# salute-developers/GigaAM

Measured on AMD Instinct MI355X. Metric: RTFx v2_ctc batch32x20s (log-mel + encoder + greedy decode), higher is better.
Workload: dtype f32 (GEMMs: 3-term split on fp16 MFMA, fp32 accumulate)

## Files before the change

### gigaam_amd/_lib.py

```python
from __future__ import annotations

import ctypes as C
import os
from typing import Optional

_HERE = os.path.dirname(os.path.abspath(__file__))
LIB_NAME = "libgigaam_hip.so"
LIB_PATH = os.path.join(_HERE, LIB_NAME)

SUBS_CONV2D, SUBS_CONV1D = 0, 1
ATT_ROTARY, ATT_REL_POS = 0, 1
NORM_BATCH, NORM_LAYER = 0, 1
HEAD_NONE, HEAD_CTC, HEAD_RNNT, HEAD_EMO = 0, 1, 2, 3
DTYPE_F32, DTYPE_F16, DTYPE_BF16, DTYPE_F64, DTYPE_I64 = 0, 1, 2, 3, 4
GEMM_F32, GEMM_F16X3, GEMM_F16 = 0, 1, 2
RS_U8, RS_I16, RS_I24, RS_I32, RS_F32, RS_MULAW, RS_ALAW = range(7)
RS_FORM_SINGLE, RS_FORM_TABLE, RS_FORM_ROWS = 0, 1, 2
PF_CLASSES = ["gemm", "conv2", "attn", "norm", "convmod", "stem", "frontend", "decode", "misc", "align_bt", "align_out"]


class GamConfig(C.Structure):
    _fields_ = [(n, C.c_int32) for n in (
        "sample_rate", "n_mels", "hop_length", "win_length", "n_fft", "center",
        "feat_in", "n_layers", "d_model", "subsampling", "subs_kernel_size", "subsampling_factor",
        "ff_expansion_factor", "self_attention_model", "n_heads", "pos_emb_max_len",
        "conv_norm_type", "conv_kernel_size",
        "head_type", "num_classes", "pred_hidden", "pred_rnn_layers", "joint_hidden",
    )]


_P = C.c_void_p


class GamLnOp(C.Structure):
    _fields_ = ([(n, _P) for n in ("x", "out1", "out2", "w1", "b1", "w2", "b2", "rcos", "rsin", "row_t", "rs", "part", "pbias", "presid",
                                   "xstore")]
                + [(n, C.c_int32) for n in ("mode", "rows", "d", "split1", "split2", "dk", "ta", "rope_rows", "nsplit")]
                + [("eps", C.c_float), ("palpha", C.c_float)])


SIGNATURES = {
    "gam_abi_version": (C.c_int, []),
    "gam_create": (C.c_int, [C.POINTER(GamConfig), C.c_int, C.POINTER(_P)]),
    "gam_destroy": (None, [_P]),
    "gam_set_weight": (C.c_int, [_P, C.c_char_p, _P, C.c_int, C.POINTER(C.c_int64), C.c_int]),
    "gam_finalize": (C.c_int, [_P]),
    "gam_feat_frames": (C.c_int64, [_P, C.c_int64]),
    "gam_enc_frames": (C.c_int64, [_P, C.c_int64]),
    "gam_frontend": (C.c_int, [_P, _P, _P, C.c_int, C.c_int64, _P, _P, _P]),
    "gam_encode": (C.c_int, [_P, _P, _P, C.c_int, C.c_int64, _P, _P, _P]),
    "gam_encode_ex": (C.c_int, [_P, _P, _P, C.c_int, C.c_int64, _P, _P, C.c_int, _P, _P]),
    "gam_encode_varlen": (C.c_int, [_P, _P, _P, C.POINTER(C.c_int64), C.c_int, C.c_int64, _P, _P, C.c_int, _P, _P]),
    "gam_last_encode_rows": (C.c_int, [_P, C.POINTER(C.c_int)]),
    "gam_ctc_head": (C.c_int, [_P, _P, C.c_int, C.c_int64, _P, _P]),
    "gam_ctc_greedy": (C.c_int, [_P, _P, _P, C.c_int, C.c_int64, _P, _P, _P, _P]),
    "gam_ctc_align": (C.c_int, [_P, _P, _P, C.c_int, C.c_int64, _P, _P, C.c_int, _P, _P, _P, _P, _P, _P, _P]),
    "gam_op_ctc_align": (C.c_int, [_P, _P, _P, C.c_int, C.c_int64, C.c_int, _P, _P, C.c_int, _P, _P, _P, _P, _P, _P, _P]),
    "gam_op_ctc_align_long": (C.c_int, [_P, _P, C.c_int64, C.c_int, _P, C.c_int, _P, _P, _P, _P, _P, _P, _P]),
    "gam_op_ctc_star_row": (C.c_int, [_P, _P, _P, C.c_int, C.c_int64, C.c_int, C.c_float, _P, _P]),
    "gam_ctc_align_star": (C.c_int, [_P, _P, _P, C.c_int, C.c_int64, _P, _P, C.c_int, C.c_float, _P, _P, _P, _P, _P, _P, _P]),
    "gam_op_ctc_align_star": (C.c_int, [_P, _P, _P, C.c_int, C.c_int64, C.c_int, _P, _P, _P, C.c_int, _P, _P, _P, _P, _P, _P, _P]),
    "gam_op_ctc_align_long_star": (C.c_int, [_P, _P, C.c_int64, C.c_int, _P, _P, C.c_int, _P, _P, _P, _P, _P, _P, _P]),
    "gam_op_ctc_stitch": (C.c_int, [_P, _P, _P, C.c_int, C.c_int64, C.c_int, _P, _P, _P, _P, C.c_int64, _P, _P]),
    "gam_op_ctc_greedy_long": (C.c_int, [_P, _P, C.c_int64, C.c_int, _P, _P, _P, _P]),
    "gam_set_ctc_align_workspace": (C.c_int, [_P, C.c_int64]),
    "gam_tune_ctc_align_long": (C.c_int, [C.c_int, C.c_int]),
    "gam_ctc_kws": (C.c_int, [_P, _P, _P, C.c_int, C.c_int64, C.c_int, _P, _P, _P, _P, _P, _P]),
    "gam_op_ctc_kws": (C.c_int, [_P, _P, _P, C.c_int, C.c_int64, C.c_int, C.c_int, _P, _P, _P, _P, _P, _P]),
    "gam_set_keywords": (C.c_int, [_P, _P, _P, C.c_int, _P]),
    "gam_ctc_beam": (C.c_int, [_P, _P, _P, C.c_int, C.c_int64, C.c_int, _P, _P, _P, _P, _P, _P]),
    "gam_op_ctc_beam": (C.c_int, [_P, _P, _P, C.c_int, C.c_int64, C.c_int, C.c_int, _P, _P, _P, _P, _P, _P]),
    "gam_set_hotwords": (C.c_int, [_P, _P, _P, C.c_int, C.c_float]),
    "gam_set_lm": (C.c_int, [_P, _P, C.c_int, _P, C.c_int64, C.c_int, _P, C.c_int64, C.c_int, C.c_int, C.c_int, C.c_int, C.c_int,
                             C.c_float, C.c_float, C.c_float]),
    "gam_rnnt_greedy": (C.c_int, [_P, _P, _P, C.c_int, C.c_int64, C.c_int, _P, _P, _P, _P, _P, C.c_int, _P]),
    "gam_ctc_beam_nbest": (C.c_int, [_P, _P, _P, C.c_int, C.c_int64, C.c_int, C.c_int, _P, _P, _P, _P, _P, _P, _P]),
    "gam_op_ctc_beam_nbest": (C.c_int, [_P, _P, _P, C.c_int, C.c_int64, C.c_int, C.c_int, C.c_int, _P, _P, _P, _P, _P, _P, _P]),
    "gam_rnnt_beam_nbest": (C.c_int, [_P, _P, _P, C.c_int, C.c_int64, C.c_int, C.c_int, C.c_int, _P, _P, _P, _P, _P, _P, _P]),
    "gam_op_rnnt_beam_nbest": (C.c_int, [_P, _P, _P, C.c_int, C.c_int64, C.c_int, C.c_int, C.c_int, _P, _P, _P, _P, _P, _P, _P]),
    "gam_rnnt_beam": (C.c_int, [_P, _P, _P, C.c_int, C.c_int64, C.c_int, C.c_int, _P, _P, _P, _P, _P, _P]),
    "gam_op_rnnt_beam": (C.c_int, [_P, _P, _P, C.c_int, C.c_int64, C.c_int, C.c_int, _P, _P, _P, _P, _P, _P]),
    "gam_rnnt_align": (C.c_int, [_P, _P, _P, C.c_int, C.c_int64, _P, _P, C.c_int, _P, _P, _P, _P, _P]),
    "gam_op_rnnt_align": (C.c_int, [_P, _P, _P, C.c_int, C.c_int64, _P, _P, C.c_int, _P, _P, _P, _P, _P, _P]),
    "gam_op_rnnt_lattice_align": (C.c_int, [_P, _P, _P, C.c_int, C.c_int64, C.c_int, _P, _P, C.c_int, _P, _P, _P, _P, _P]),
    "gam_set_rnnt_align_workspace": (C.c_int, [_P, C.c_int64]),
    "gam_ctc_confidence": (C.c_int, [_P, _P, _P, C.c_int, C.c_int64, _P, _P, _P, C.c_int, C.c_int, C.c_int, _P, _P, _P, _P]),
    "gam_op_ctc_confidence": (C.c_int, [_P, _P, _P, C.c_int, C.c_int64, C.c_int, _P, _P, _P, C.c_int, C.c_int, C.c_int, _P, _P, _P, _P]),
    "gam_rnnt_confidence": (C.c_int, [_P, _P, _P, C.c_int, C.c_int64, _P, _P, _P, C.c_int, C.c_int, _P, _P, _P]),
    "gam_op_rnnt_confidence": (C.c_int, [_P, _P, _P, C.c_int, C.c_int64, _P, _P, _P, C.c_int, C.c_int, _P, _P, _P]),
    "gam_emo_probs": (C.c_int, [_P, _P, _P, C.c_int, C.c_int64, _P, _P]),
    "gam_rnnt_predict": (C.c_int, [_P, _P, _P, _P, C.c_int, _P, _P, _P, _P]),
    "gam_rnnt_joint": (C.c_int, [_P, _P, _P, C.c_int, C.c_int, C.c_int, _P, _P]),
    "gam_set_gemm_mode": (C.c_int, [_P, C.c_int]),
    "gam_get_gemm_mode": (C.c_int, [_P]),
    "gam_set_rnnt_cluster": (C.c_int, [_P, C.c_int]),
    "gam_get_rnnt_cluster": (C.c_int, [_P]),
    "gam_rnnt_cluster_plan_info": (C.c_int, [C.c_int] * 8 + [C.POINTER(C.c_int32)]),
    "gam_rnnt_last_decode": (C.c_int, [_P, C.POINTER(C.c_int32)]),
    "gam_debug_buffer_hash": (C.c_int, [_P, C.c_int, C.POINTER(C.c_uint64), C.POINTER(C.c_int64)]),
    "gam_range_flag": (C.c_int, [_P, C.POINTER(C.c_int), _P]),
    "gam_range_flag_fetch": (C.c_int, [_P, _P, _P]),
    "gam_op_gemm": (C.c_int, [_P, _P, _P, _P, _P, C.c_int, C.c_int, C.c_int, C.c_int, _P]),
    "gam_op_gemm_ex": (C.c_int, [_P, _P, _P, _P, _P, C.c_float, _P, C.c_int, C.c_int, C.c_int, C.c_int, _P]),
    "gam_op_attention": (C.c_int, [_P, _P, _P, _P, _P, _P, C.c_int, C.c_int, C.c_int, _P]),
    "gam_op_attention_ex": (C.c_int, [_P, _P, _P, _P, C.c_int64, _P, _P, _P, C.c_int, C.c_int, C.c_int, C.c_int, _P, _P, _P, _P]),
    "gam_op_layernorm": (C.c_int, [_P, C.POINTER(GamLnOp), _P]),
    "gam_op_convmod": (C.c_int, [_P, _P, _P, _P, _P, _P, _P, _P, _P, C.c_int, C.c_int, C.c_int, C.c_int, C.c_int, C.c_int, C.c_int, _P]),
    "gam_tune_sp": (C.c_int, [C.c_int, C.c_int, C.c_int]),
    "gam_plan_sp": (C.c_int, [C.c_int, C.c_int, C.c_int, C.c_int, C.POINTER(C.c_int), C.POINTER(C.c_int), C.POINTER(C.c_int)]),
    "gam_plan_sp_ex": (C.c_int, [C.c_int, C.c_int, C.c_int, C.c_int, C.POINTER(C.c_int), C.POINTER(C.c_int), C.POINTER(C.c_int), C.POINTER(C.c_int)]),
    "gam_tune_sp_stages": (C.c_int, [C.c_int]),
    "gam_resample_plan": (C.c_int, [C.c_int, C.c_int, C.POINTER(C.c_int), C.POINTER(C.c_int), C.POINTER(C.c_int)]),
    "gam_resample_tile": (C.c_int, [C.c_int, C.c_int, C.POINTER(C.c_int), C.POINTER(C.c_int)]),
    "gam_resample_table": (C.c_int, [C.c_int, C.c_int, _P, _P]),
    "gam_resample_out_len": (C.c_int64, [C.c_int, C.c_int, C.c_int64]),
    "gam_op_resample": (C.c_int, [_P, C.c_int, C.c_int, C.c_int, _P, C.c_int, C.c_int64, C.c_int, C.c_int, _P, _P, _P, C.c_int64, _P, _P]),
    "gam_profile_enable": (C.c_int, [_P, C.c_int]),
    "gam_profile_pause": (C.c_int, [_P, C.c_int]),
    "gam_profile_read": (C.c_int, [_P, C.c_int, C.POINTER(C.c_double), C.POINTER(C.c_int64), C.POINTER(C.c_double)]),
    "gam_profile_read_bytes": (C.c_int, [_P, C.c_int, C.POINTER(C.c_double)]),
    "gam_last_error": (C.c_char_p, [_P]),
    "gam_comm_unique_id": (C.c_int, [C.c_char_p]),
    "gam_comm_create": (C.c_int, [C.c_char_p, C.c_int, C.c_int, C.c_int, C.POINTER(_P)]),
    "gam_comm_world": (C.c_int, [_P]),
    "gam_gather_ids": (C.c_int, [_P, _P, _P, _P, _P, C.c_int, C.c_int, _P, _P, _P, _P, _P]),
    "gam_comm_last_error": (C.c_char_p, [_P]),
    "gam_comm_destroy": (None, [_P]),
}

_lib: Optional[C.CDLL] = None


class GigaAMHipError(RuntimeError):
    pass


def load_library(path: Optional[str] = None) -> C.CDLL:
    global _lib
    if _lib is not None and path is None:
        return _lib
    p = path or os.environ.get("GIGAAM_HIP_LIB", LIB_PATH)
    if not os.path.exists(p):
        raise GigaAMHipError(
            f"{p} not found: the HIP extension is not built. Run `python -c 'import __graft_entry__ as g; g.build()'` "
            "(hipcc --offload-arch=gfx950). There is no CPU fallback.")
    lib = C.CDLL(p)
    for name, (res, args) in SIGNATURES.items():
        fn = getattr(lib, name)
        fn.restype = res
        fn.argtypes = args
    if lib.gam_abi_version() != 1:
        raise GigaAMHipError("libgigaam_hip.so ABI version mismatch")
    if path is None:
        _lib = lib
    return lib
```

### gigaam_amd/csrc/gam_api.hip

```cpp
#include <hip/hip_runtime.h>

#include <algorithm>
#include <cmath>
#include <cstdarg>
#include <cstdio>
#include <cstring>
#include <map>
#include <string>
#include <vector>

#include "../../include/gigaam_hip.h"
#include "gam_align.h"
#include "gam_align_long.h"
#include "gam_kws.h"
#include "gam_attn.h"
#include "gam_beam.h"
#include "gam_rnnt_beam.h"
#include "gam_attn16.h"
#include "gam_comm.h"
#include "gam_common.h"
#include "gam_convmod.h"
#include "gam_decode.h"
#include "gam_rnnt_align.h"
#include "gam_confidence.h"
#include "gam_decode_cluster.h"
#include "gam_frontend.h"
#include "gam_gemm.h"
#include "gam_gemm_sp.h"
#include "gam_norm.h"
#include "gam_pack.h"
#include "gam_resample.h"
#include "gam_stem.h"
#include "gam_stitch.h"

namespace {

struct HostTensor {
  std::vector<float> data;
  std::vector<int64_t> shape;
  int64_t numel() const {
    int64_t n = 1;
    for (auto s : shape) n *= s;
    return n;
  }
};

struct DevBuf {
  float* p = nullptr;
  size_t cap = 0;
  DevBuf() = default;
  DevBuf(DevBuf&& o) noexcept : p(o.p), cap(o.cap) { o.p = nullptr; o.cap = 0; }
  DevBuf& operator=(DevBuf&& o) noexcept { std::swap(p, o.p); std::swap(cap, o.cap); return *this; }
  ~DevBuf() { (void)release(); }
  hipError_t release() {
    const hipError_t e = p ? hipFree(p) : hipSuccess;
    p = nullptr; cap = 0;
    return e;
  }
  hipError_t alloc(size_t floats) {
    hipError_t e = release();
    if (e == hipSuccess) e = hipMalloc(&p, floats * sizeof(float));
    if (e == hipSuccess) cap = floats; else p = nullptr;
    return e;
  }
  template <class T> T* as() const { return reinterpret_cast<T*>(p); }
};

struct W16 {
  _Float16* sp = nullptr;
  _Float16* h16 = nullptr;
  float inv = 1.0f;
};

struct LayerW {
  float *ln_ff1_w, *ln_ff1_b, *ff1_w1, *ff1_b1, *ff1_w2, *ff1_b2;
  float *ln_att_w, *ln_att_b, *wqkv, *bqkv, *wo, *bo;
  float *wpos, *pos_u, *pos_v;
  float *ln_conv_w, *ln_conv_b, *pw1_w, *pw1_b, *dw_w, *dw_b, *cn_scale, *cn_shift, *pw2_w, *pw2_b;
  float *ln_ff2_w, *ln_ff2_b, *ff2_w1, *ff2_b1, *ff2_w2, *ff2_b2;
  float *ln_out_w, *ln_out_b;
  W16 s_ff1_w1, s_ff1_w2, s_wqkv, s_wo, s_wpos, s_pw1, s_pw2, s_ff2_w1, s_ff2_w2;
};

struct ProfEvent {
  hipEvent_t a, b;
  int cls;
};

}

struct gam_handle {
  gam_config cfg;
  int device = 0;
  bool finalized = false;
  bool has_encoder = false, has_head = false;
  std::map<std::string, HostTensor> staged;
  std::vector<DevBuf> owned;
  std::string err;

  float* dft_basis = nullptr;
  int* mel_band = nullptr;
  float* mel_wts = nullptr;
  int mel_nw = 0;
  int nf = 0, kpad = 0;
  float *c1_w = nullptr, *c1_b = nullptr, *c2_w = nullptr, *c2_b = nullptr, *lin_w = nullptr, *lin_b = nullptr;
  W16 s_c1, s_c2, s_lin;
  int gemm_mode = 1;
  int f1 = 0, f2 = 0;
  std::vector<LayerW> layers;
  float *rot_cos = nullptr, *rot_sin = nullptr;
  float* rel_pe = nullptr;
  float* rel_pe_sp = nullptr;
  float *ctc_w = nullptr, *ctc_b = nullptr;
  float *emo_w = nullptr, *emo_b = nullptr;
  float *jn_enc_w = nullptr, *jn_enc_b = nullptr, *jn_pred_t = nullptr, *jn_pred_b = nullptr;
  float *jn_out_w = nullptr, *jn_out_b = nullptr, *lstm_whh_t = nullptr, *lstm_tab = nullptr;
  float *lstm_whh_q = nullptr, *jn_pred_q = nullptr;
  float* jn_pred_w = nullptr;
  DevBuf jz, jp, jl;
  float *lstm_wih_x = nullptr, *lstm_whh_x = nullptr, *lstm_bias_x = nullptr;
  int use_rowscale = 1;
  int use_range = 1;
  int ncu = 256;
  int rnnt_cluster = -1;
  int rnnt_coop = 1;
  int rnnt_force_timeout = 0;
  int rnnt_no_repair = 0;
  int rnnt_exclusive = 0;
  int last_rnnt_c = 0, last_rnnt_kern = -1, last_rnnt_refused = 0;
  DevBuf rnnt_x;
  DevBuf rnnt_audit;
  bool audit_pending = false; int audit_last_c = 0; long audit_decodes = 0, audit_hit_decodes = 0;
  hipEvent_t dec_evt = nullptr;
  hipStream_t dec_stream = nullptr;
  bool dec_evt_set = false;

  DevBuf wavp, spec, img, c2, xin, y1, x, y, yr, hbuf, qkv, ctx, ubuf, zbuf, tok, logits, encp, pbuf, aplanes;
  DevBuf op_planes, op_sp, splitk_ws;
  DevBuf align_star;
  DevBuf align_bp;
  DevBuf align_long_ws;
  DevBuf greedy_long_ws;
  size_t al_ws_limit = GAM_AL_WS_DEFAULT;
  DevBuf beam_nodes;
  DevBuf rb_ws, rb_nodes;
  DevBuf ra_g, ra_pp, ra_lat, ra_bp;
  DevBuf cf_stats;
  size_t ra_ws_limit = GAM_RA_WS_DEFAULT;
  DevBuf hw_trie;
  int hw_nodes = 0, hw_words = 0, hw_max_tok = -1;
  float hw_boost = 0.f;
  DevBuf kw_dev;
  int kw_K = 0, kw_ntok = 0, kw_max_tok = -1;
  DevBuf kws_mb;
  DevBuf lm_cls, lm_wt, lm_ng;
  int lm_V = 0, lm_wslots = 0, lm_wprobe = 0, lm_nslots = 0, lm_nprobe = 0, lm_order = 0, lm_bos = 0, lm_eos = 0, lm_unk = 0;
  float lm_unk_logp = 0.f, lm_alpha = 0.f, lm_beta = 0.f;
  DevBuf dec_splitk_ws;
  int last_rows = 0, last_rows_padded = 0;
  DevBuf pack_idx;
  int use_pack = 1;
  int use_splitk = 1;
  int fuse_reduce = 1;
  int use_graph = 1;
  int graph_max_rows = 2048;
  uint64_t ws_generation = 0;
  struct GraphEntry {
    enum Seen { UNSEEN, SEEN_ONCE, PLAIN_ONLY };
    uint64_t gen = 0; Seen seen = UNSEEN; hipGraphExec_t exec = nullptr;
  };
  std::map<std::vector<int>, GraphEntry> graphs;
  long graph_replays = 0, graph_captures_failed = 0;
  int graph_count = 0;
  hipStream_t cap_stream = nullptr;
  DevBuf lens;
  DevBuf rsbuf, op_rs;
  int* range_flag = nullptr;

  int prof_on = 0;
  std::vector<ProfEvent> prof_events;
  size_t prof_used = 0;
  double prof_work[GAM_PF_NCLASS] = {0};
  double prof_bytes[GAM_PF_NCLASS] = {0};
  int64_t prof_launches[GAM_PF_NCLASS] = {0};
};

namespace {

int fail(gam_handle* h, int code, const char* fmt, ...) {
  char buf[512];
  va_list ap;
  va_start(ap, fmt);
  vsnprintf(buf, sizeof buf, fmt, ap);
  va_end(ap);
  if (h) h->err = buf;
  return code;
}

#define HIPCHK(h, expr)                                                                        \
  do {                                                                                         \
    hipError_t e_ = (expr);                                                                    \
    if (e_ != hipSuccess) return fail(h, -2, "%s failed: %s (%s:%d)", #expr, hipGetErrorString(e_), __FILE__, __LINE__); \
  } while (0)

void* dev_upload(gam_handle* h, const void* src, size_t bytes, size_t alloc_bytes) {
  h->owned.emplace_back();
  DevBuf& b = h->owned.back();
  if (b.alloc((alloc_bytes + 3) / 4) != hipSuccess) return nullptr;
  if (src && bytes && hipMemcpy(b.p, src, bytes, hipMemcpyHostToDevice) != hipSuccess) return nullptr;
  return b.p;
}

float* upload(gam_handle* h, const std::vector<float>& v) {
  return (float*)dev_upload(h, v.data(), v.size() * sizeof(float), std::max<size_t>(v.size(), 4) * sizeof(float));
}

int ensure_table(gam_handle* h, DevBuf& b, size_t floats) {
  if (floats <= b.cap) return 0;
  HIPCHK(h, b.alloc(floats));
  return 0;
}
// ... 59 lines not shown
    hi[i] = hb;
    lo[i] = float_to_half_bits(v - half_to_float(hb));
  }
  out.inv = ldexpf(1.0f, -shift);
  std::vector<uint16_t> hp(hi);
  if (conv_taps > 0 && K > 0 && (K / conv_taps) % 64 == 0 && w.size() % (size_t)K == 0) {
    const size_t C = (size_t)K / conv_taps, cb64 = C / 64;
    for (size_t n = 0; n < w.size() / K; ++n)
      for (size_t cb = 0; cb < cb64; ++cb)
        for (size_t t = 0; t < (size_t)conv_taps; ++t)
          for (size_t j = 0; j < 64; ++j)
            hp[n * K + (cb * conv_taps + t) * 64 + j] = hi[n * K + t * C + cb * 64 + j];
  }
  out.h16 = (_Float16*)dev_upload(h, hp.data(), w.size() * 2, std::max<size_t>(w.size(), 8) * 2 + 64);
  if (!out.h16) return -2;
  if (K > 0 && K % 32 == 0 && w.size() % (size_t)K == 0) {
    std::vector<uint16_t> sp(w.size() * 2);
    for (size_t i = 0; i < w.size(); ++i) {
      const size_t n = i / K, k = i % K;
      size_t kb = k / 32;
      if (conv_taps > 0) {
        const size_t cblocks = (size_t)K / conv_taps / 32, t = kb / cblocks, cb = kb % cblocks;
        kb = cb * conv_taps + t;
      }
      const size_t o = n * 2 * (size_t)K + kb * 64 + (k % 32);
      sp[o] = hi[i];
      sp[o + 32] = lo[i];
    }
    out.sp = (_Float16*)dev_upload(h, sp.data(), sp.size() * 2, sp.size() * 2 + 64);
    if (!out.sp) return -2;
  }
  return 0;
}

const HostTensor* find(gam_handle* h, const std::string& key) {
  auto it = h->staged.find(key);
  return it == h->staged.end() ? nullptr : &it->second;
}

struct ProfScope {
  gam_handle* h;
  hipStream_t s;
  ProfEvent* ev = nullptr;
  ProfScope(gam_handle* h_, hipStream_t s_, int cls, double work) : h(h_), s(s_) {
    if (!h->prof_on || (h->prof_on == 2 && cls != GAM_PF_GEMM && cls != GAM_PF_CONV2)) return;
    if (h->prof_used == h->prof_events.size()) {
      ProfEvent e;
      if (hipEventCreate(&e.a) != hipSuccess || hipEventCreate(&e.b) != hipSuccess) return;
      h->prof_events.push_back(e);
    }
    ev = &h->prof_events[h->prof_used++];
    ev->cls = cls;
    h->prof_work[cls] += work;
    h->prof_launches[cls] += 1;
    hipEventRecord(ev->a, s);
  }
  ~ProfScope() {
    if (ev) hipEventRecord(ev->b, s);
  }
};

struct PendingReduce {
  const float* part = nullptr;
  int nsplit = 0;
  const float* bias = nullptr;
  const float* resid = nullptr;
  float alpha = 1.0f;
  GamGemmArgs full;
  int act = 0;
  void clear() { part = nullptr; nsplit = 0; }
};

int flush_pending(gam_handle* h, hipStream_t s, PendingReduce* p) {
  if (p == nullptr || p->part == nullptr) return 0;
  const hipError_t e = gam_launch_splitk_reduce(p->full, p->act, p->nsplit, s);
  const int M = p->full.M, N = p->full.N;
  p->clear();
  if (e != hipSuccess) return fail(h, -2, "split-K reduce launch (M=%d N=%d): %s", M, N, hipGetErrorString(e));
  return 0;
}

static inline bool split_mode(const gam_handle* h) { return h->gemm_mode != GAM_GEMM_F32; }

int gemm(gam_handle* h, hipStream_t s, const GamGemmArgs& a_in, int act, int cls = GAM_PF_GEMM, const W16* w16 = nullptr,
         PendingReduce* defer = nullptr) {
  GamGemmArgs a = a_in;
  if (int r = flush_pending(h, s, defer)) return r;
  a.range_flag = h->use_range ? h->range_flag : nullptr;
  if (!split_mode(h)) a.c_guard = 0;
  ProfScope ps(h, s, cls, 2.0 * (double)a.M * (double)a.N * (double)a.K);
  if (ps.ev) {
    const double abytes = a.a_mode == 0 ? ((double)(a.M - 1) * (double)std::min<long>(a.lda, a.K) + a.K) * 4.0
                                        : (double)a.M / a.conv_f2 * 2.0 * a.conv_fp * a.conv_c * 4.0;
    h->prof_bytes[cls] += abytes * (a.n_switch > 0 ? 2.0 : 1.0) + 4.0 * a.N * a.K + 4.0 * a.M * a.N * (a.R ? 2.0 : 1.0);
  }
  hipError_t e;
  if (a.Asp != nullptr) {
    if (!split_mode(h)) return fail(h, -2, "sp32 A operand outside the split-fp16 GEMM mode");
    if (w16 == nullptr || w16->sp == nullptr) return fail(h, -2, "sp32 A without sp32 W planes");
    a.wscale_inv = w16->inv;
    a.Wsp = w16->sp;
    a.h16 = 0;
    if (a.a_fmt == 2) {
      if (a.K % 64 != 0 || (a.a_mode == 0 ? a.lda % 64 != 0 : a.conv_c % 64 != 0) || w16->h16 == nullptr)
        return fail(h, -2, "GAM_GEMM_F16: K / row pitch of a GEMM operand is not a multiple of 64 (M=%d N=%d K=%d)", a.M, a.N, a.K);
      a.h16 = 1; a.K /= 2; a.lda /= 2; a.conv_c /= 2;
      a.Wsp = w16->h16;
    }
    GamSpPlan plan = gam_gemm_sp_plan(a.M, a.N, a.K, a.a_mode, h->ncu);
    if (!h->use_splitk) plan.s = 1;
    a.sp_mt = plan.mt; a.sp_nw = plan.nw; a.sp_ns = plan.ns;
    GamGemmArgs full = a;
    if (plan.s > 1) {
      if (int r = ensure(h, h->splitk_ws, (size_t)plan.s * a.M * a.N + 64)) return r;
      a.splitk = plan.s; a.partial = h->splitk_ws.p;
    }
    e = gam_launch_gemm_sp(a, act, s);
    if (e != hipSuccess) return fail(h, -2, "sp gemm launch (M=%d N=%d K=%d): %s", a.M, a.N, a.K, hipGetErrorString(e));
    if (plan.s > 1 && defer != nullptr && h->fuse_reduce && act == GAM_ACT_NONE && !a.c_split && !a.c_guard && a.lens == nullptr &&
        !a.remap && a.ldc == a.N && a.bias != nullptr && a.R != nullptr && a.ldr == a.N) {
      defer->part = a.partial; defer->nsplit = plan.s; defer->bias = a.bias; defer->resid = a.R; defer->alpha = a.alpha;
      defer->full = full; defer->full.partial = a.partial; defer->act = act;
    } else if (plan.s > 1) {
      full.partial = a.partial;
      e = gam_launch_splitk_reduce(full, act, plan.s, s);
      if (e != hipSuccess) return fail(h, -2, "split-K reduce launch (M=%d N=%d): %s", a.M, a.N, hipGetErrorString(e));
    }
    return 0;
  }
  if (a.a_rs != nullptr || a.c_split) return fail(h, -2, "row-scaled A or split C without sp32 operands (M=%d N=%d K=%d)", a.M, a.N, a.K);
  int S = 1;
  if (h->use_splitk && a.a_mode == 0 && a.K % 32 == 0) {
    const int tiles = gam_cdiv(a.M, 128) * gam_cdiv(a.N, 128), nk = a.K / 32, ncu = 256;
    if (tiles * 2 <= ncu && nk >= 4) {
      S = std::min(16, std::min(ncu / tiles, nk / 2));
      while (S > 1 && nk % S != 0) --S;
    }
  }
  GamGemmArgs full = a;
  if (S > 1) {
    DevBuf& ws = cls == GAM_PF_DECODE ? h->dec_splitk_ws : h->splitk_ws;
    if (int r = ensure(h, ws, (size_t)S * a.M * a.N + 64)) return r;
    a.splitk = S; a.ldw = a.K; a.K = a.K / S; a.partial = ws.p;
  }
  e = gam_launch_gemm(a, act, s);
  if (e != hipSuccess) return fail(h, -2, "gemm launch (M=%d N=%d K=%d): %s", a.M, a.N, a.K, hipGetErrorString(e));
  if (S > 1) {
    full.partial = a.partial;
    e = gam_launch_splitk_reduce(full, act, S, s);
    if (e != hipSuccess) return fail(h, -2, "split-K reduce launch (M=%d N=%d): %s", a.M, a.N, hipGetErrorString(e));
  }
  return 0;
}

GamGemmArgs gemm_args(const float* A, long lda, const float* W, const float* bias, float* C, long ldc, int M, int N, int K) {
  GamGemmArgs g;
  memset(&g, 0, sizeof g);
  g.A = A; g.W = W; g.bias = bias; g.C = C; g.R = nullptr;
  g.M = M; g.N = N; g.K = K; g.lda = lda; g.ldc = ldc; g.ldr = ldc; g.alpha = 1.0f;
  g.rpb = 1; g.fdiv = 1;
  return g;
}

int layernorm(gam_handle* h, hipStream_t s, GamLnArgs a, int mode, PendingReduce* pend = nullptr) {
  if (pend != nullptr && pend->part != nullptr) {
    const GamGemmArgs& g = pend->full;
    if (a.x == g.C && a.rows == g.M && a.d == g.N && g.ldc == g.N) {
      a.part = pend->part; a.nsplit = pend->nsplit; a.pbias = pend->bias; a.presid = pend->resid; a.palpha = pend->alpha;
      a.xstore = const_cast<float*>(a.x);
      pend->clear();
    } else if (int r = flush_pending(h, s, pend)) {
      return r;
    }
  }
  const double bytes = (double)a.rows * a.d * 4.0 * (mode == 0 ? 2.0 : 3.0);
  ProfScope ps(h, s, GAM_PF_NORM, bytes);
  hipError_t e = gam_launch_layernorm(a, mode, s);
  if (e != hipSuccess) return fail(h, -2, "layernorm launch: %s", hipGetErrorString(e));
  return 0;
}

int64_t half_up(int64_t l) { return l <= 0 ? 0 : (l + 1) / 2; }

struct DecodeScope {
  gam_handle* h;
  hipStream_t s;
  DecodeScope(gam_handle* h_, hipStream_t s_) : h(h_), s(s_) {
    if (h->dec_evt == nullptr && hipEventCreateWithFlags(&h->dec_evt, hipEventDisableTiming) != hipSuccess) { h->dec_evt = nullptr; (void)hipGetLastError(); }
    if (h->dec_evt != nullptr && h->dec_evt_set && h->dec_stream != s) (void)hipStreamWaitEvent(s, h->dec_evt, 0);
  }
  ~DecodeScope() {
    if (h->dec_evt != nullptr && hipEventRecord(h->dec_evt, s) == hipSuccess) { h->dec_stream = s; h->dec_evt_set = true; }
  }
};

#define GAM_DECODE_ENTRY(h, stream)      \
  hipStream_t s = (hipStream_t)(stream); \
  if (!(h)) return -1;                   \
  HIPCHK(h, hipSetDevice((h)->device));  \
  DecodeScope ds(h, s)

int head_check(gam_handle* h, int want, const char* who) {
  if (!h) return -1;
  if (who && !h->finalized) return fail(h, -1, "%s before gam_finalize", who);
  if (h->cfg.head_type != want || !h->has_head)
    return fail(h, -1, "model has no %s head", want == GAM_HEAD_CTC ? "CTC" : want == GAM_HEAD_RNNT ? "RNN-T" : "emotion");
  return 0;
}

template <class Args> void rnnt_pred_weights(const gam_handle* h, Args& a) {
  a.gate_tab = h->lstm_tab; a.whh_t = h->lstm_whh_t; a.wih_x = h->lstm_wih_x; a.whh_x = h->lstm_whh_x; a.bias_x = h->lstm_bias_x;
}
template <class Args> void rnnt_joint_weights(const gam_handle* h, Args& a) {
  a.wpred_t = h->jn_pred_t; a.bpred = h->jn_pred_b; a.wout = h->jn_out_w; a.bout = h->jn_out_b;
}

}

extern "C" {

int gam_abi_version(void) { return GAM_ABI_VERSION; }

const char* gam_last_error(const gam_handle* h) { return h ? h->err.c_str() : "null handle"; }

int gam_create(const gam_config* cfg, int device_id, gam_handle** out) {
  if (!cfg || !out) return -1;
  gam_handle* h = new gam_handle();
  h->cfg = *cfg;
  h->device = device_id;
  *out = h;
  if (const char* e = getenv("GAM_SPLITK")) h->use_splitk = atoi(e);
  if (const char* e = getenv("GAM_PACK")) h->use_pack = atoi(e);
  if (const char* e = getenv("GAM_FUSE_REDUCE")) h->fuse_reduce = atoi(e);
  if (const char* e = getenv("GAM_GRAPH")) h->use_graph = atoi(e);
  if (const char* e = getenv("GAM_GRAPH_MAX_ROWS")) h->graph_max_rows = atoi(e);
  if (const char* e = getenv("GAM_RNNT_CLUSTER")) h->rnnt_cluster = std::max(-1, std::min(8, atoi(e)));
  if (const char* e = getenv("GAM_RNNT_ALIGN_WS")) h->ra_ws_limit = (size_t)std::max(1ll, atoll(e));
  if (const char* e = getenv("GAM_CTC_ALIGN_WS")) h->al_ws_limit = (size_t)std::max(1ll, atoll(e));
  if (const char* e = getenv("GAM_RNNT_EXCLUSIVE")) h->rnnt_exclusive = atoi(e);
  if (const char* e = getenv("GAM_RNNT_COOP")) h->rnnt_coop = atoi(e);
  if (const char* e = getenv("GAM_RNNT_FORCE_TIMEOUT")) h->rnnt_force_timeout = atoi(e);
  if (const char* e = getenv("GAM_RNNT_NO_REPAIR")) h->rnnt_no_repair = atoi(e);
  {
    int n = 0;
    if (hipDeviceGetAttribute(&n, hipDeviceAttributeMultiprocessorCount, device_id) == hipSuccess && n > 0) h->ncu = n;
    int co = 0;
    if (hipDeviceGetAttribute(&co, hipDeviceAttributeCooperativeLaunch, device_id) != hipSuccess || co == 0) h->rnnt_coop = 0;
  }
  if (const char* e = getenv("GAM_ROWSCALE")) h->use_rowscale = atoi(e);
  if (const char* e = getenv("GAM_RANGE")) h->use_range = atoi(e);
  if (const char* e = getenv("GAM_GEMM_MODE"))
    h->gemm_mode = strcmp(e, "f32") == 0 ? GAM_GEMM_F32 : (strcmp(e, "f16") == 0 ? GAM_GEMM_F16 : GAM_GEMM_F16X3);
  const gam_config& c = h->cfg;
  if (c.d_model <= 0 || c.n_heads <= 0 || c.d_model % c.n_heads != 0)
    return fail(h, -1, "bad d_model/n_heads %d/%d", c.d_model, c.n_heads);
  if (c.d_model / c.n_heads != GAM_ATT_DK) return fail(h, -1, "head dim %d unsupported (kernels are built for %d)", c.d_model / c.n_heads, GAM_ATT_DK);
  if (c.d_model % 64 != 0 || c.d_model > 1024) return fail(h, -1, "d_model %d unsupported", c.d_model);
  if (c.subsampling_factor != 4) return fail(h, -1, "subsampling_factor %d unsupported", c.subsampling_factor);
  if (c.subsampling == GAM_SUBS_CONV2D && c.subs_kernel_size != 3) return fail(h, -1, "conv2d stem needs kernel 3");
  if (c.subsampling == GAM_SUBS_CONV1D && c.subs_kernel_size != 5) return fail(h, -1, "conv1d stem needs kernel 5");
  if (c.win_length != c.n_fft) return fail(h, -1, "win_length != n_fft unsupported");
  if (c.n_mels > 64 || c.n_mels != c.feat_in) return fail(h, -1, "n_mels %d / feat_in %d unsupported", c.n_mels, c.feat_in);
  if (c.head_type == GAM_HEAD_RNNT && (c.pred_rnn_layers < 1 || c.pred_rnn_layers > 4 || c.pred_hidden > GAM_RNNT_MAXH || c.joint_hidden > GAM_RNNT_MAXH || c.num_classes > GAM_RNNT_MAXV || c.joint_hidden % 16 != 0 || c.pred_hidden % 16 != 0))
    return fail(h, -1, "RNN-T head shape unsupported");
  if (hipSetDevice(device_id) != hipSuccess) return fail(h, -2, "hipSetDevice(%d) failed", device_id);
  return 0;
}

#if GAM_RC_AUDIT
static int audit_dump(gam_handle* h);
#endif
void gam_destroy(gam_handle* h) {
  if (!h) return;
  hipSetDevice(h->device);
#if GAM_RC_AUDIT
  audit_dump(h);
  fprintf(stderr, "[gam-audit] total: %ld of %ld cluster decodes logged at least one entry\n", h->audit_hit_decodes, h->audit_decodes);
#endif
  for (auto& e : h->prof_events) { hipEventDestroy(e.a); hipEventDestroy(e.b); }
  for (auto& g : h->graphs)
    if (g.second.exec) hipGraphExecDestroy(g.second.exec);
  if (h->cap_stream) hipStreamDestroy(h->cap_stream);
  if (h->dec_evt) hipEventDestroy(h->dec_evt);
  if (getenv("GAM_GRAPH_DEBUG")) fprintf(stderr, "[gam] graph replays %ld, failed captures %ld\n", h->graph_replays, h->graph_captures_failed);
  delete h;
}

int gam_set_weight(gam_handle* h, const char* key, const void* host_ptr, int dtype, const int64_t* shape, int ndim) {
  if (!h || !key || !host_ptr) return -1;
  if (h->finalized) return fail(h, -1, "gam_set_weight after gam_finalize");
  HostTensor t;
  for (int i = 0; i < ndim; ++i) t.shape.push_back(shape[i]);
  const int64_t n = t.numel();
  t.data.resize((size_t)n);
  switch (dtype) {
    case GAM_DTYPE_F32: memcpy(t.data.data(), host_ptr, (size_t)n * 4); break;
    case GAM_DTYPE_F16: for (int64_t i = 0; i < n; ++i) t.data[i] = half_to_float(((const uint16_t*)host_ptr)[i]); break;
    case GAM_DTYPE_BF16: for (int64_t i = 0; i < n; ++i) { uint32_t u = (uint32_t)((const uint16_t*)host_ptr)[i] << 16; memcpy(&t.data[i], &u, 4); } break;
    case GAM_DTYPE_F64: for (int64_t i = 0; i < n; ++i) t.data[i] = (float)((const double*)host_ptr)[i]; break;
    case GAM_DTYPE_I64: for (int64_t i = 0; i < n; ++i) t.data[i] = (float)((const int64_t*)host_ptr)[i]; break;
    default: return fail(h, -1, "unknown dtype %d for %s", dtype, key);
  }
  h->staged[key] = std::move(t);
  return 0;
}

struct Dst {
  float** p;
  const char* name;
};
#define DST(member) Dst{&(member), #member}

static int need(gam_handle* h, const std::string& key, int64_t n, const HostTensor** t) {
  *t = find(h, key);
  if (!*t) return fail(h, -3, "missing weight %s", key.c_str());
  if ((*t)->numel() != n) return fail(h, -3, "weight %s has %lld elements, expected %lld", key.c_str(), (long long)(*t)->numel(), (long long)n);
  return 0;
}

static int upload_to(gam_handle* h, Dst dst, const std::vector<float>& v) {
  *dst.p = upload(h, v);
  return *dst.p ? 0 : fail(h, -2, "device upload failed (%s)", dst.name);
}

static int up_split(gam_handle* h, const std::vector<float>& w, W16* out, int K, int conv_taps = 0) {
  return make_split(h, w, *out, K, conv_taps) ? fail(h, -2, "split upload failed") : 0;
}

static int upload_linear(gam_handle* h, const std::string& prefix, int64_t nout, int64_t nin, Dst w, Dst b, W16* split) {
  const HostTensor *wt, *bt;
  if (int r = need(h, prefix + ".weight", nout * nin, &wt)) return r;
  if (int r = need(h, prefix + ".bias", nout, &bt)) return r;
// ... 79 lines not shown

static int fin_stem_conv2d(gam_handle* h) {
  const int C = h->cfg.d_model, D = h->cfg.d_model, F = h->cfg.feat_in;
  const std::string pe = "encoder.pre_encode.";
  h->f1 = (F + 1) / 2;
  h->f2 = (h->f1 + 1) / 2;
  const HostTensor *w0, *b0, *w2, *b2, *wl, *bl;
  if (int r = need(h, pe + "conv.0.weight", (int64_t)C * 9, &w0)) return r;
  if (int r = need(h, pe + "conv.0.bias", C, &b0)) return r;
  if (int r = need(h, pe + "conv.2.weight", (int64_t)C * C * 9, &w2)) return r;
  if (int r = need(h, pe + "conv.2.bias", C, &b2)) return r;
  if (int r = need(h, pe + "out.weight", (int64_t)D * C * h->f2, &wl)) return r;
  if (int r = need(h, pe + "out.bias", D, &bl)) return r;
  if (int r = upload_to(h, DST(h->c1_w), w0->data)) return r;
  if (int r = upload_to(h, DST(h->c1_b), b0->data)) return r;
  const std::vector<float> t2 = swap_inner(w2->data, C, C, 9);
  if (int r = upload_to(h, DST(h->c2_w), t2)) return r;
  if (int r = up_split(h, t2, &h->s_c2, 9 * C, C % 32 == 0 ? 9 : 0)) return r;
  if (int r = upload_to(h, DST(h->c2_b), b2->data)) return r;
  const std::vector<float> l = swap_inner(wl->data, D, C, h->f2);
  if (int r = upload_to(h, DST(h->lin_w), l)) return r;
  if (int r = up_split(h, l, &h->s_lin, C * h->f2)) return r;
  return upload_to(h, DST(h->lin_b), bl->data);
}

static int fin_stem_conv1d(gam_handle* h) {
  const int C = h->cfg.d_model, F = h->cfg.feat_in, ks = h->cfg.subs_kernel_size;
  const std::string pe = "encoder.pre_encode.";
  const HostTensor *w0, *b0, *w2, *b2;
  if (int r = need(h, pe + "conv.0.weight", (int64_t)C * F * ks, &w0)) return r;
  if (int r = need(h, pe + "conv.0.bias", C, &b0)) return r;
  if (int r = need(h, pe + "conv.2.weight", (int64_t)C * C * ks, &w2)) return r;
  if (int r = need(h, pe + "conv.2.bias", C, &b2)) return r;
  const std::vector<float> r0 = swap_inner(w0->data, C, F, ks), r2 = swap_inner(w2->data, C, C, ks);
  if (int r = upload_to(h, DST(h->c1_w), r0)) return r;
  if (int r = up_split(h, r0, &h->s_c1, ks * F)) return r;
  if (int r = upload_to(h, DST(h->c1_b), b0->data)) return r;
  if (int r = upload_to(h, DST(h->c2_w), r2)) return r;
  if (int r = up_split(h, r2, &h->s_c2, ks * C)) return r;
  return upload_to(h, DST(h->c2_b), b2->data);
}

static int fin_qkv(gam_handle* h, const std::string& p, LayerW& L) {
  const int D = h->cfg.d_model;
  const HostTensor *wq, *bq, *wk, *bk, *wv, *bv;
  if (int r = need(h, p + "self_attn.linear_q.weight", (int64_t)D * D, &wq)) return r;
  if (int r = need(h, p + "self_attn.linear_q.bias", D, &bq)) return r;
  if (int r = need(h, p + "self_attn.linear_k.weight", (int64_t)D * D, &wk)) return r;
  if (int r = need(h, p + "self_attn.linear_k.bias", D, &bk)) return r;
  if (int r = need(h, p + "self_attn.linear_v.weight", (int64_t)D * D, &wv)) return r;
  if (int r = need(h, p + "self_attn.linear_v.bias", D, &bv)) return r;
  std::vector<float> w(wq->data), b(bq->data);
  w.insert(w.end(), wk->data.begin(), wk->data.end());
  w.insert(w.end(), wv->data.begin(), wv->data.end());
  b.insert(b.end(), bk->data.begin(), bk->data.end());
  b.insert(b.end(), bv->data.begin(), bv->data.end());
  if (int r = upload_to(h, DST(L.wqkv), w)) return r;
  if (int r = upload_to(h, DST(L.bqkv), b)) return r;
  return up_split(h, w, &L.s_wqkv, D);
}

static int fin_conv_norm(gam_handle* h, const std::string& p, LayerW& L) {
  const int D = h->cfg.d_model;
  const HostTensor *g, *be;
  if (int r = need(h, p + "conv.batch_norm.weight", D, &g)) return r;
  if (int r = need(h, p + "conv.batch_norm.bias", D, &be)) return r;
  if (h->cfg.conv_norm_type != GAM_NORM_BATCH) {
    if (int r = upload_to(h, DST(L.cn_scale), g->data)) return r;
    return upload_to(h, DST(L.cn_shift), be->data);
  }
  const HostTensor *rm, *rv;
  if (int r = need(h, p + "conv.batch_norm.running_mean", D, &rm)) return r;
  if (int r = need(h, p + "conv.batch_norm.running_var", D, &rv)) return r;
  std::vector<float> sc(D), sh(D);
  for (int i = 0; i < D; ++i) {
    const float inv = 1.0f / sqrtf(rv->data[i] + 1e-5f);
    sc[i] = g->data[i] * inv;
    sh[i] = be->data[i] - rm->data[i] * sc[i];
  }
  if (int r = upload_to(h, DST(L.cn_scale), sc)) return r;
  return upload_to(h, DST(L.cn_shift), sh);
}

static int fin_layer(gam_handle* h, int li, LayerW& L) {
  const gam_config& c = h->cfg;
  const int D = c.d_model, DFF = D * c.ff_expansion_factor;
  const std::string p = "encoder.layers." + std::to_string(li) + ".";
  memset(&L, 0, sizeof L);
  if (int r = upload_ln(h, p + "norm_feed_forward1", D, DST(L.ln_ff1_w), DST(L.ln_ff1_b))) return r;
  if (int r = upload_linear(h, p + "feed_forward1.linear1", DFF, D, DST(L.ff1_w1), DST(L.ff1_b1), &L.s_ff1_w1)) return r;
  if (int r = upload_linear(h, p + "feed_forward1.linear2", D, DFF, DST(L.ff1_w2), DST(L.ff1_b2), &L.s_ff1_w2)) return r;
  if (int r = upload_ln(h, p + "norm_self_att", D, DST(L.ln_att_w), DST(L.ln_att_b))) return r;
  if (int r = fin_qkv(h, p, L)) return r;
  if (int r = upload_linear(h, p + "self_attn.linear_out", D, D, DST(L.wo), DST(L.bo), &L.s_wo)) return r;
  if (c.self_attention_model == GAM_ATT_REL_POS) {
    const HostTensor *wp, *pu, *pv;
    if (int r = need(h, p + "self_attn.linear_pos.weight", (int64_t)D * D, &wp)) return r;
    if (int r = need(h, p + "self_attn.pos_bias_u", D, &pu)) return r;
    if (int r = need(h, p + "self_attn.pos_bias_v", D, &pv)) return r;
    if (int r = upload_to(h, DST(L.wpos), wp->data)) return r;
    if (int r = up_split(h, wp->data, &L.s_wpos, D)) return r;
    if (int r = upload_to(h, DST(L.pos_u), pu->data)) return r;
    if (int r = upload_to(h, DST(L.pos_v), pv->data)) return r;
  }
  if (int r = upload_ln(h, p + "norm_conv", D, DST(L.ln_conv_w), DST(L.ln_conv_b))) return r;
  if (int r = upload_linear(h, p + "conv.pointwise_conv1", 2 * D, D, DST(L.pw1_w), DST(L.pw1_b), &L.s_pw1)) return r;
  if (int r = upload_linear(h, p + "conv.depthwise_conv", D, c.conv_kernel_size, DST(L.dw_w), DST(L.dw_b), nullptr)) return r;
  if (int r = fin_conv_norm(h, p, L)) return r;
  if (int r = upload_linear(h, p + "conv.pointwise_conv2", D, D, DST(L.pw2_w), DST(L.pw2_b), &L.s_pw2)) return r;
  if (int r = upload_ln(h, p + "norm_feed_forward2", D, DST(L.ln_ff2_w), DST(L.ln_ff2_b))) return r;
  if (int r = upload_linear(h, p + "feed_forward2.linear1", DFF, D, DST(L.ff2_w1), DST(L.ff2_b1), &L.s_ff2_w1)) return r;
  if (int r = upload_linear(h, p + "feed_forward2.linear2", D, DFF, DST(L.ff2_w2), DST(L.ff2_b2), &L.s_ff2_w2)) return r;
  return upload_ln(h, p + "norm_out", D, DST(L.ln_out_w), DST(L.ln_out_b));
}

static int fin_rotary(gam_handle* h) {
  const int dk = h->cfg.d_model / h->cfg.n_heads, half = dk / 2, n = h->cfg.pos_emb_max_len;
  std::vector<float> cs((size_t)n * half), sn((size_t)n * half);
  for (int i = 0; i < half; ++i) {
    const float inv_freq = 1.0f / powf((float)n, (float)(2 * i) / (float)dk);
    for (int t = 0; t < n; ++t) {
      const float fr = (float)t * inv_freq;
      cs[(size_t)t * half + i] = (float)cos((double)fr);
      sn[(size_t)t * half + i] = (float)sin((double)fr);
    }
  }
  if (int r = upload_to(h, DST(h->rot_cos), cs)) return r;
  return upload_to(h, DST(h->rot_sin), sn);
}

static int fin_rel_pos(gam_handle* h) {
  const int D = h->cfg.d_model, n = h->cfg.pos_emb_max_len;
  std::vector<float> pe((size_t)(2 * n - 1) * D);
  for (int i = 0; i < D / 2; ++i) {
    const float w = expf((float)(2 * i) * (float)(-(log(10000.0) / D)));
    for (int r = -(n - 1); r <= n - 1; ++r) {
      const float ang = (float)r * w;
      pe[(size_t)(r + n - 1) * D + 2 * i] = (float)sin((double)ang);
      pe[(size_t)(r + n - 1) * D + 2 * i + 1] = (float)cos((double)ang);
    }
  }
  if (int r = upload_to(h, DST(h->rel_pe), pe)) return r;
  h->rel_pe_sp = (float*)dev_upload(h, nullptr, 0, pe.size() * sizeof(float));
  if (!h->rel_pe_sp) return fail(h, -2, "device upload failed (h->rel_pe_sp)");
  hipLaunchKernelGGL(gam_to_sp32_kernel, dim3((int)std::min<size_t>((pe.size() / 4 + 255) / 256, 4096)), dim3(256), 0, nullptr, h->rel_pe,
                     reinterpret_cast<_Float16*>(h->rel_pe_sp), pe.size() / 4, (const float*)nullptr, D);
  HIPCHK(h, hipGetLastError());
  HIPCHK(h, hipStreamSynchronize(nullptr));
  return 0;
}

static int fin_rnnt_upper(gam_handle* h) {
  const int PH = h->cfg.pred_hidden, LX = h->cfg.pred_rnn_layers - 1;
  const size_t G = (size_t)4 * PH;
  std::vector<float> wih_x(LX * PH * G), whh_x(LX * PH * G), bias_x(LX * G);
  for (int l = 1; l <= LX; ++l) {
    const std::string sfx = "_l" + std::to_string(l);
    const HostTensor *wi, *wh, *bi, *bh;
    if (int r = need(h, "head.decoder.lstm.weight_ih" + sfx, (int64_t)4 * PH * PH, &wi)) return r;
    if (int r = need(h, "head.decoder.lstm.weight_hh" + sfx, (int64_t)4 * PH * PH, &wh)) return r;
    if (int r = need(h, "head.decoder.lstm.bias_ih" + sfx, 4 * PH, &bi)) return r;
    if (int r = need(h, "head.decoder.lstm.bias_hh" + sfx, 4 * PH, &bh)) return r;
    transpose_rk(wi->data.data(), G, PH, &wih_x[(l - 1) * PH * G]);
    transpose_rk(wh->data.data(), G, PH, &whh_x[(l - 1) * PH * G]);
    for (size_t r = 0; r < G; ++r) bias_x[(l - 1) * G + r] = bi->data[r] + bh->data[r];
  }
  if (int r = upload_to(h, DST(h->lstm_wih_x), wih_x)) return r;
  if (int r = upload_to(h, DST(h->lstm_whh_x), whh_x)) return r;
  return upload_to(h, DST(h->lstm_bias_x), bias_x);
}

static std::vector<float> lstm_input_table(const HostTensor* emb, const HostTensor* wih, const HostTensor* bih, const HostTensor* bhh, int V, int PH) {
  std::vector<float> tab((size_t)(V + 1) * 4 * PH);
  for (int v = 0; v <= V; ++v)
    for (int r = 0; r < 4 * PH; ++r) {
      float acc = 0.f;
      if (v < V) {
        const float* wr = &wih->data[(size_t)r * PH];
        const float* e = &emb->data[(size_t)v * PH];
        for (int k = 0; k < PH; ++k) acc = fmaf(wr[k], e[k], acc);
      }
      tab[(size_t)v * 4 * PH + r] = (acc + bih->data[r]) + bhh->data[r];
    }
  return tab;
}

static int fin_rnnt_head(gam_handle* h) {
  const gam_config& c = h->cfg;
  const int D = c.d_model, V = c.num_classes, PH = c.pred_hidden, JH = c.joint_hidden;
  const HostTensor *emb, *wih, *whh, *bih, *bhh, *wp, *bp, *we, *bee, *wo, *bo;
  if (int r = need(h, "head.decoder.embed.weight", (int64_t)V * PH, &emb)) return r;
  if (int r = need(h, "head.decoder.lstm.weight_ih_l0", (int64_t)4 * PH * PH, &wih)) return r;
  if (int r = need(h, "head.decoder.lstm.weight_hh_l0", (int64_t)4 * PH * PH, &whh)) return r;
  if (int r = need(h, "head.decoder.lstm.bias_ih_l0", 4 * PH, &bih)) return r;
  if (int r = need(h, "head.decoder.lstm.bias_hh_l0", 4 * PH, &bhh)) return r;
  if (int r = need(h, "head.joint.pred.weight", (int64_t)JH * PH, &wp)) return r;
  if (int r = need(h, "head.joint.pred.bias", JH, &bp)) return r;
  if (int r = need(h, "head.joint.enc.weight", (int64_t)JH * D, &we)) return r;
  if (int r = need(h, "head.joint.enc.bias", JH, &bee)) return r;
  if (int r = need(h, "head.joint.joint_net.1.weight", (int64_t)V * JH, &wo)) return r;
  if (int r = need(h, "head.joint.joint_net.1.bias", V, &bo)) return r;
  if (c.pred_rnn_layers > 1)
    if (int r = fin_rnnt_upper(h)) return r;
  if (int r = upload_to(h, DST(h->lstm_whh_q), quad_rk(whh->data, 4 * PH, PH))) return r;
  if (int r = upload_to(h, DST(h->jn_pred_q), quad_rk(wp->data, JH, PH))) return r;
  if (int r = upload_to(h, DST(h->lstm_tab), lstm_input_table(emb, wih, bih, bhh, V, PH))) return r;
  if (int r = upload_to(h, DST(h->lstm_whh_t), swap_inner(whh->data, 1, 4 * PH, PH))) return r;
  if (int r = upload_to(h, DST(h->jn_pred_t), swap_inner(wp->data, 1, JH, PH))) return r;
  if (int r = upload_to(h, DST(h->jn_pred_b), bp->data)) return r;
  if (int r = upload_to(h, DST(h->jn_pred_w), wp->data)) return r;
  if (int r = upload_to(h, DST(h->jn_enc_w), we->data)) return r;
  if (int r = upload_to(h, DST(h->jn_enc_b), bee->data)) return r;
  if (int r = upload_to(h, DST(h->jn_out_w), wo->data)) return r;
  return upload_to(h, DST(h->jn_out_b), bo->data);
}

static int fin_head(gam_handle* h) {
  const gam_config& c = h->cfg;
  if (c.head_type == GAM_HEAD_CTC) return upload_linear(h, "head.decoder_layers.0", c.num_classes, c.d_model, DST(h->ctc_w), DST(h->ctc_b), nullptr);
  if (c.head_type == GAM_HEAD_EMO) return upload_linear(h, "head", c.num_classes, c.d_model, DST(h->emo_w), DST(h->emo_b), nullptr);
  return c.head_type == GAM_HEAD_RNNT ? fin_rnnt_head(h) : 0;
}

int gam_finalize(gam_handle* h) {
  if (!h) return -1;
  if (h->finalized) return 0;
  HIPCHK(h, hipSetDevice(h->device));
  const gam_config& c = h->cfg;
  if (int r = fin_frontend(h)) return r;
  const bool build_encoder = find(h, "encoder.pre_encode.conv.0.weight") != nullptr;
  if (build_encoder) {
    if (int r = c.subsampling == GAM_SUBS_CONV2D ? fin_stem_conv2d(h) : fin_stem_conv1d(h)) return r;
    h->layers.resize(c.n_layers);
    for (int li = 0; li < c.n_layers; ++li)
      if (int r = fin_layer(h, li, h->layers[li])) return r;
    if (int r = c.self_attention_model == GAM_ATT_ROTARY ? fin_rotary(h) : fin_rel_pos(h)) return r;
  }
  h->has_encoder = build_encoder;
  h->has_head = find(h, "head.decoder_layers.0.weight") != nullptr || find(h, "head.joint.enc.weight") != nullptr ||
                (c.head_type == GAM_HEAD_EMO && find(h, "head.weight") != nullptr);
  if (h->has_head)
    if (int r = fin_head(h)) return r;
  const std::vector<int> zeros(16, 0);
  h->range_flag = (int*)dev_upload(h, zeros.data(), 64, 64);
  if (!h->range_flag) return fail(h, -2, "device upload failed (h->range_flag)");
  h->staged.clear();
  h->finalized = true;
  return 0;
}

int64_t gam_feat_frames(const gam_handle* h, int64_t n) {
  const gam_config& c = h->cfg;
  if (c.center) return n / c.hop_length + 1;
  return n < c.win_length ? 0 : (n - c.win_length) / c.hop_length + 1;
}

int64_t gam_enc_frames(const gam_handle* h, int64_t t) {
  (void)h;
  return half_up(half_up(t));
}

int gam_frontend(gam_handle* h, const float* wav, const int64_t* wav_len, int B, int64_t L, float* feat,
                 int64_t* feat_len, void* stream) {
  if (!h || !h->finalized) return fail(h, -1, "gam_frontend before gam_finalize");
  if (B <= 0 || L <= 0) return fail(h, -1, "bad shape B=%d L=%lld", B, (long long)L);
  const gam_config& c = h->cfg;
  hipStream_t s = (hipStream_t)stream;
  HIPCHK(h, hipSetDevice(h->device));
  const int hop = c.hop_length, n = c.n_fft, half = n / 2;
  if (c.center && L <= half) return fail(h, -1, "input of %lld samples is too short for reflect padding (%d)", (long long)L, half);
  const int64_t Tf = gam_feat_frames(h, L);
  if (Tf <= 0) return fail(h, -1, "input of %lld samples yields no frames", (long long)L);
  const int64_t need = (Tf - 1) * hop + h->kpad;
  const int64_t Tfa = (need + hop - 1) / hop;
  const int64_t Lp = Tfa * hop;
  const int lds = (2 * h->nf + 3) / 4 * 4;
  if (int r = ensure(h, h->wavp, (size_t)B * Lp + h->kpad + 64)) return r;
  if (int r = ensure(h, h->spec, (size_t)B * Tfa * lds)) return r;
  {
    ProfScope ps(h, s, GAM_PF_FRONTEND, (double)B * (L + Lp) * 4.0);
    dim3 grid(gam_cdiv(Lp, 256), B);
    hipLaunchKernelGGL(gam_pad_wav_kernel, grid, dim3(256), 0, s, wav, h->wavp.p, B, (long)L, (long)Lp, half, c.center);
    HIPCHK(h, hipGetLastError());
    HIPCHK(h, hipMemsetAsync(h->wavp.p + (size_t)B * Lp, 0, (h->kpad + 64) * sizeof(float), s));
  }
  GamGemmArgs g = gemm_args(h->wavp.p, hop, h->dft_basis, nullptr, h->spec.p, lds, (int)(B * Tfa), 2 * h->nf, h->kpad);
  if (int r = gemm(h, s, g, GAM_ACT_NONE, GAM_PF_FRONTEND, nullptr)) return r;
  {
    GamPowMelArgs a;
    a.spec = h->spec.p; a.wts = h->mel_wts; a.nw = h->mel_nw; a.band = h->mel_band; a.feat = feat; a.wav_len = (const long long*)wav_len; a.feat_len = (long long*)feat_len;
    a.B = B; a.Tfa = (int)Tfa; a.Tf = (int)Tf; a.nf = h->nf; a.n_mels = c.n_mels; a.lds = lds;
    a.hop = hop; a.win = c.win_length; a.center = c.center;
    ProfScope ps(h, s, GAM_PF_FRONTEND, (double)B * Tf * (2.0 * h->nf + c.n_mels) * 4.0);
    dim3 grid(gam_cdiv(Tf, 64), B);
    const size_t pm_lds = (size_t)(64 * (h->nf + 1) + h->mel_nw) * sizeof(float);
    if (pm_lds > 160 * 1024) return fail(h, -1, "n_fft %d: the power / mel kernel's LDS image (%zu bytes) does not fit", c.n_fft, pm_lds);
    if (pm_lds > 64 * 1024) {
      static std::atomic<unsigned long long> attr_devs{0};
      HIPCHK(h, gam_set_max_lds(reinterpret_cast<const void*>(gam_powmel_kernel), (int)pm_lds, attr_devs));
    }
    hipLaunchKernelGGL(gam_powmel_kernel, grid, dim3(256), pm_lds, s, a);
    HIPCHK(h, hipGetLastError());
  }
  return 0;
}

struct EncPlan {
  int B;
  int64_t T;
  int T1, Tv;
  int Ta, N;
  int NR, Tmax;
  int T1a;
  int D, DFF, F, H, dk, nl;
  bool conv2d, rel, packed;
  bool sp;
  int spf;
  bool sp_stem;
  bool graph;
};

struct EncBufs {
  int *len0, *len1, *len2, *elen;
  int *cu, *row_t, *row_src;
  float* rs;
};

struct EncCtx {
  EncPlan p;
  EncBufs w;
  GamLnArgs ln;
};

static int enc_plan(gam_handle* h, int B, int64_t T, int n_layers_run, const int64_t* feat_len_host, EncPlan& p) {
  const gam_config& c = h->cfg;
  if (B <= 0 || T <= 0) return fail(h, -1, "bad shape B=%d T=%lld", B, (long long)T);
  p.B = B; p.T = T;
  p.D = c.d_model; p.F = c.feat_in; p.H = c.n_heads; p.dk = p.D / p.H; p.DFF = p.D * c.ff_expansion_factor;
  p.T1 = (int)half_up(T); p.Tv = (int)half_up(p.T1);
  if (p.Tv > c.pos_emb_max_len) return fail(h, -1, "%d encoder frames exceed pos_emb_max_len %d", p.Tv, c.pos_emb_max_len);
  if (p.Tv <= 0) return fail(h, -1, "no encoder frames");
  p.conv2d = c.subsampling == GAM_SUBS_CONV2D;
  p.rel = c.self_attention_model == GAM_ATT_REL_POS;
  p.nl = n_layers_run < 0 ? c.n_layers : std::min(n_layers_run, c.n_layers);
  p.Ta = p.conv2d ? std::max(p.Tv + 1, (p.T1 + 3) / 2) : std::max(p.Tv, (p.T1 + 5) / 2);
  p.N = B * p.Ta;
  const int pad = (c.subs_kernel_size - 1) / 2;
  p.T1a = p.conv2d ? 0 : std::max(p.T1, (int)((T + 2 * pad + 1) / 2));
  p.packed = false;
  p.NR = p.N; p.Tmax = p.Ta;
  const bool pack_regime = h->use_pack >= 2 || !h->use_graph || p.N >= h->graph_max_rows;
  if (feat_len_host != nullptr && h->use_pack && pack_regime && B > 1 && B <= 1024) {
    long long sum = 0;
    int mx = 0;
    for (int b = 0; b < B; ++b) {
      const int64_t l = std::min<int64_t>(std::max<int64_t>(feat_len_host[b], 0), T);
      const int l2 = (int)half_up(half_up(l));
      sum += l2;
      mx = std::max(mx, l2);
    }
    if (sum > 0 && sum * 100 <= (long long)p.N * 97) { p.packed = true; p.NR = (int)sum; p.Tmax = mx; }
  }
  p.sp = split_mode(h) && p.D % 32 == 0 && p.DFF % 32 == 0;
  const bool f16_fmt_ok = p.D % 64 == 0 && p.DFF % 64 == 0;
  p.spf = p.sp ? (h->gemm_mode == GAM_GEMM_F16 && f16_fmt_ok ? 2 : 1) : 0;
  p.sp_stem = p.sp && p.F % 32 == 0;
  p.graph = h->use_graph && !h->prof_on && p.nl > 0 && p.N < h->graph_max_rows && !p.packed;
  return 0;
}

static int enc_workspace(gam_handle* h, const EncPlan& p, EncBufs& w) {
  const size_t B = p.B, N = p.N, D = p.D, Ta = p.Ta;
  if (int r = ensure(h, h->lens, 4 * B)) return r;
  const size_t maxB = h->lens.cap / 4;
  w.len0 = h->lens.as<int>(); w.len1 = w.len0 + maxB; w.len2 = w.len0 + 2 * maxB; w.elen = w.len0 + 3 * maxB;
  if (int r = ensure(h, h->x, N * D)) return r;
  if (int r = ensure(h, h->y, N * D)) return r;
  if (int r = ensure(h, h->yr, N * D)) return r;
  if (int r = ensure(h, h->hbuf, N * p.DFF)) return r;
  if (int r = ensure(h, h->qkv, N * 3 * D)) return r;
  if (int r = ensure(h, h->ctx, N * D)) return r;
  if (int r = ensure(h, h->ubuf, N * 2 * D)) return r;
  if (int r = ensure(h, h->zbuf, N * D)) return r;
  if (int r = ensure(h, h->rsbuf, N + 64)) return r;
  if (p.packed)
    if (int r = ensure(h, h->pack_idx, (size_t)1032 + 2 * N)) return r;
  w.cu = p.packed ? reinterpret_cast<int*>(h->pack_idx.p) : nullptr;
  w.row_t = p.packed ? w.cu + 1032 : nullptr;
  w.row_src = p.packed ? w.row_t + N : nullptr;
  w.rs = p.sp && h->use_rowscale ? h->rsbuf.p : nullptr;
  if (p.conv2d) {
    if (int r = ensure(h, h->img, (B * 2 * Ta + 2) * (h->f1 + 1) * D)) return r;
    if (int r = ensure(h, h->c2, N * h->f2 * D)) return r;
  } else {
    if (int r = ensure(h, h->xin, (B * 2 * p.T1a + 8) * p.F)) return r;
    if (int r = ensure(h, h->y1, (B * 2 * Ta + 8) * D)) return r;
  }
  if (p.rel)
    if (int r = ensure(h, h->pbuf, (size_t)(2 * p.Tv - 1) * D)) return r;
  if (p.graph)
    if (int r = ensure(h, h->splitk_ws, (size_t)16 * N * std::max(p.DFF, 2 * p.D) + 64)) return r;
  return 0;
}

static GamLnArgs enc_ln_args(const gam_handle* h, const EncPlan& p, const EncBufs& w) {
  GamLnArgs ln;
  memset(&ln, 0, sizeof ln);
  ln.rows = p.NR; ln.d = p.D; ln.ta = p.Ta; ln.row_t = w.row_t; ln.dk = p.dk; ln.eps = 1e-5f; ln.rcos = h->rot_cos; ln.rsin = h->rot_sin;
  ln.rope_rows = h->cfg.pos_emb_max_len;
  ln.rs = w.rs;
  return ln;
}

static int enc_lengths(gam_handle* h, hipStream_t s, const EncPlan& p, const EncBufs& w, const int64_t* feat_len) {
  ProfScope ps(h, s, GAM_PF_MISC, 0.0);
  hipLaunchKernelGGL(gam_lengths_kernel, dim3(gam_cdiv(p.B, 64)), dim3(64), 0, s, (const long long*)feat_len, p.B, (int)p.T, 2,
                     w.len0, w.len1, w.len2, w.elen);
  HIPCHK(h, hipGetLastError());
  if (p.packed) {
    hipLaunchKernelGGL(gam_pack_index_kernel, dim3(1), dim3(256), 0, s, w.len2, p.B, p.Ta, p.NR, w.cu, w.row_t, w.row_src, h->range_flag);
    HIPCHK(h, hipGetLastError());
  }
  return 0;
}

static inline void gemm_formats(GamGemmArgs& g, int a_fmt, const float* a_rs, int c_split, int c_guard) {
  if (a_fmt) { g.Asp = reinterpret_cast<const _Float16*>(g.A); g.a_fmt = a_fmt; }
  g.a_rs = a_rs; g.c_split = c_split; g.c_guard = c_guard;
}

static int stem_conv2d(gam_handle* h, hipStream_t s, const EncPlan& p, const EncBufs& w, const float* feat) {
  const int B = p.B, Ta = p.Ta, N = p.N, C = p.D, D = p.D, FP = h->f1 + 1, F2 = h->f2;
  {
    GamConv1Args a;
    a.feat = feat; a.img = h->img.p; a.w = h->c1_w; a.bias = h->c1_b; a.len0 = w.len0; a.len1 = w.len1;
    a.B = B; a.T = (int)p.T; a.F = p.F; a.Ta = Ta; a.FP = FP; a.C = C; a.T1 = p.T1;
    a.img_split = p.spf;
    a.range_flag = h->use_range ? h->range_flag : nullptr;
    ProfScope ps(h, s, GAM_PF_STEM, (double)B * 2 * Ta * FP * C * 4.0);
    if (a.img_split == 2) hipLaunchKernelGGL(gam_conv2d1_kernel<2>, dim3(2 * Ta, B), dim3(256), 0, s, a);
    else if (a.img_split == 1) hipLaunchKernelGGL(gam_conv2d1_kernel<1>, dim3(2 * Ta, B), dim3(256), 0, s, a);
    else hipLaunchKernelGGL(gam_conv2d1_kernel<0>, dim3(2 * Ta, B), dim3(256), 0, s, a);
    HIPCHK(h, hipGetLastError());
    const size_t img_end = (size_t)B * 2 * Ta * FP * C;
    HIPCHK(h, hipMemsetAsync(a.img_split == 2 ? reinterpret_cast<float*>(reinterpret_cast<_Float16*>(h->img.p) + img_end) : h->img.p + img_end, 0,
                             (size_t)2 * FP * C * sizeof(float), s));
  }
  GamGemmArgs g = gemm_args(h->img.p, 0, h->c2_w, h->c2_b, h->c2.p, C, N * F2, C, 9 * C);
  g.a_mode = 1; g.conv_fp = FP; g.conv_c = C; g.conv_f2 = F2;
  g.lens = w.len2; g.rpb = Ta * F2; g.fdiv = F2;
  g.skip_pad = p.packed ? 1 : 0;
  gemm_formats(g, p.spf, nullptr, p.spf, 1);
  if (int r = gemm(h, s, g, GAM_ACT_RELU, GAM_PF_CONV2, &h->s_c2)) return r;
  GamGemmArgs l = gemm_args(h->c2.p, (long)F2 * C, h->lin_w, h->lin_b, p.packed ? h->y.p : h->x.p, D, N, D, F2 * C);
  gemm_formats(l, p.spf, nullptr, 0, 0);
  return gemm(h, s, l, GAM_ACT_NONE, GAM_PF_GEMM, &h->s_lin);
}

static int stem_conv1d(gam_handle* h, hipStream_t s, const EncPlan& p, const EncBufs& w, const float* feat) {
  const int B = p.B, Ta = p.Ta, T1a = p.T1a, N = p.N, C = p.D, D = p.D, F = p.F;
  const int64_t T = p.T;
  const int ks = h->cfg.subs_kernel_size, pad = (ks - 1) / 2;
  const int fmt = p.sp_stem ? 1 : 0;
  {
    ProfScope ps(h, s, GAM_PF_STEM, (double)B * T * F * 8.0);
    HIPCHK(h, hipMemsetAsync(h->xin.p, 0, ((size_t)B * 2 * T1a + 8) * F * sizeof(float), s));
    HIPCHK(h, hipMemsetAsync(h->y1.p, 0, ((size_t)B * 2 * Ta + 8) * C * sizeof(float), s));
    dim3 grid(gam_cdiv(T, 32), gam_cdiv(F, 32), B);
    int* const rf = h->use_range ? h->range_flag : nullptr;
    if (p.sp_stem) hipLaunchKernelGGL(gam_feat_to_rows_kernel<1>, grid, dim3(256), 0, s, feat, h->xin.p, w.len0, B, F, (int)T, 2 * T1a, pad, rf);
    else hipLaunchKernelGGL(gam_feat_to_rows_kernel<0>, grid, dim3(256), 0, s, feat, h->xin.p, w.len0, B, F, (int)T, 2 * T1a, pad, rf);
    HIPCHK(h, hipGetLastError());
  }
  GamGemmArgs g1 = gemm_args(h->xin.p, 2L * F, h->c1_w, h->c1_b, h->y1.p, C, B * T1a, C, ks * F);
  g1.lens = w.len1; g1.rpb = T1a; g1.fdiv = 1;
  g1.remap = 1; g1.out_rpb = 2 * Ta; g1.out_shift = pad; g1.rows_valid = std::min(T1a, 2 * Ta - pad);
  gemm_formats(g1, fmt, nullptr, fmt, 1);
  if (int r = gemm(h, s, g1, GAM_ACT_RELU, GAM_PF_CONV2, &h->s_c1)) return r;
  GamGemmArgs g2 = gemm_args(h->y1.p, 2L * C, h->c2_w, h->c2_b, p.packed ? h->y.p : h->x.p, D, N, D, ks * C);
  g2.lens = w.len2; g2.rpb = Ta; g2.fdiv = 1;
  gemm_formats(g2, fmt, nullptr, 0, 0);
  return gemm(h, s, g2, GAM_ACT_RELU, GAM_PF_CONV2, &h->s_c2);
}

static int enc_stem(gam_handle* h, hipStream_t s, const EncPlan& p, const EncBufs& w, const float* feat) {
  if (int r = p.conv2d ? stem_conv2d(h, s, p, w, feat) : stem_conv1d(h, s, p, w, feat)) return r;
  if (p.packed) {
    ProfScope ps(h, s, GAM_PF_STEM, (double)p.NR * p.D * 8.0);
    hipLaunchKernelGGL(gam_gather_rows_kernel, dim3(std::min(4096, gam_cdiv(p.NR * (p.D / 4), 256))), dim3(256), 0, s, h->y.p, w.row_src, h->x.p, p.NR, p.D);
    HIPCHK(h, hipGetLastError());
  }
  return 0;
}

static int launch_attention(gam_handle* h, hipStream_t s, const float* q, const float* k, const float* v, long ldq, float* ctx, int ctx_split,
                            const int* lens, const int* cu, int B, int Ta, int Tv, int H, const float* pbuf, const float* pos_u,
                            const float* pos_v) {
  const int D = H * GAM_ATT_DK;
  GamAttnArgs at;
  memset(&at, 0, sizeof at);
  at.q = q; at.k = k; at.v = v; at.ctx = ctx; at.ctx_split = ctx_split; at.lens = lens; at.cu = cu;
  at.B = B; at.Ta = Ta; at.Tv = Tv; at.H = H; at.ldq = ldq; at.ldv = ldq; at.ldo = D;
  at.scale = 1.0f / sqrtf((float)GAM_ATT_DK);
  at.pbuf = pbuf; at.pos_u = pos_u; at.pos_v = pos_v; at.ldp = D;
  hipError_t e = gam_launch_attn_mode(at, GAM_ATT_DK, split_mode(h), s, h->gemm_mode == GAM_GEMM_F16 ? 1 : 3, h->ncu);
  if (e != hipSuccess) return fail(h, -2, "attention launch: %s", hipGetErrorString(e));
  return 0;
}

static hipError_t launch_convmod(gam_handle* h, hipStream_t s, const float* u, float* z, const float* dw_w, const float* dw_b, const float* n_scale,
                                 const float* n_shift, const int* lens, const int* cu, int B, int Ta, int Tv, int d, int ks, bool layer_norm,
                                 int z_split) {
  GamConvModArgs cm;
  memset(&cm, 0, sizeof cm);
  cm.u = u; cm.z = z; cm.dw_w = dw_w; cm.dw_b = dw_b; cm.n_scale = n_scale; cm.n_shift = n_shift;
  cm.lens = lens; cm.cu = cu; cm.B = B; cm.Ta = Ta; cm.Tv = Tv; cm.d = d; cm.ks = ks; cm.eps = 1e-5f;
  cm.z_split = z_split; cm.range_flag = h->use_range ? h->range_flag : nullptr;
  return gam_launch_convmod(cm, layer_norm, s);
}

static int norm_to_y(gam_handle* h, hipStream_t s, const EncCtx& c, const float* w, const float* b, PendingReduce* pend) {
  GamLnArgs a = c.ln;
  a.x = h->x.p; a.out1 = h->y.p; a.w1 = w; a.b1 = b;
  a.split1 = c.p.spf;
  return layernorm(h, s, a, 0, pend);
}

static int ffn_block(gam_handle* h, hipStream_t s, const EncCtx& c, const float* w1, const float* b1, const W16& s_w1, const float* w2,
                     const float* b2, const W16& s_w2, PendingReduce* pend) {
  const int D = c.p.D, DFF = c.p.DFF, NR = c.p.NR, spf = c.p.spf;
  GamGemmArgs g = gemm_args(h->y.p, D, w1, b1, h->hbuf.p, DFF, NR, DFF, D);
  gemm_formats(g, spf, c.w.rs, spf, 1);
  if (int r = gemm(h, s, g, GAM_ACT_SILU, GAM_PF_GEMM, &s_w1)) return r;
  GamGemmArgs g2 = gemm_args(h->hbuf.p, DFF, w2, b2, h->x.p, D, NR, D, DFF);
  g2.R = h->x.p; g2.ldr = D; g2.alpha = 0.5f;
  gemm_formats(g2, spf, nullptr, 0, 0);
  return gemm(h, s, g2, GAM_ACT_NONE, GAM_PF_GEMM, &s_w2, pend);
}

static int attn_block(gam_handle* h, hipStream_t s, const EncCtx& c, const LayerW& L, PendingReduce* pend) {
  const EncPlan& p = c.p;
  const int D = p.D, NR = p.NR, Tv = p.Tv, spf = p.spf;
  float* const rs = c.w.rs;
  GamLnArgs a = c.ln;
  a.x = h->x.p; a.out1 = h->y.p; a.out2 = h->yr.p; a.w1 = L.ln_att_w; a.b1 = L.ln_att_b;
  a.split1 = spf; a.split2 = spf;
  if (int r = layernorm(h, s, a, p.rel ? 0 : 1, pend)) return r;
  const bool one_launch = p.rel || (p.sp && (2 * D) % 256 == 0);
  if (one_launch) {
    GamGemmArgs gq = gemm_args(p.rel ? h->y.p : h->yr.p, D, L.wqkv, L.bqkv, h->qkv.p, 3 * D, NR, 3 * D, D);
    gemm_formats(gq, spf, rs, 0, 1);
    if (!p.rel) { gq.Asp2 = reinterpret_cast<const _Float16*>(h->y.p); gq.n_switch = 2 * D; }
    if (int r = gemm(h, s, gq, GAM_ACT_NONE, GAM_PF_GEMM, &L.s_wqkv)) return r;
  } else {
    GamGemmArgs gq = gemm_args(h->yr.p, D, L.wqkv, L.bqkv, h->qkv.p, 3 * D, NR, 2 * D, D);
    gemm_formats(gq, spf, rs, 0, 1);
    if (int r = gemm(h, s, gq, GAM_ACT_NONE, GAM_PF_GEMM, &L.s_wqkv)) return r;
    W16 wv16 = L.s_wqkv;
    const size_t off = (size_t)2 * D * D;
    wv16.h16 += off;
    if (wv16.sp) wv16.sp += 2 * off;
    GamGemmArgs gv = gemm_args(h->y.p, D, L.wqkv + off, L.bqkv + 2 * D, h->qkv.p + 2 * D, 3 * D, NR, D, D);
    gemm_formats(gv, spf, rs, 0, 1);
    if (int r = gemm(h, s, gv, GAM_ACT_NONE, GAM_PF_GEMM, &wv16)) return r;
  }
  if (p.rel) {
    const size_t pe0 = (size_t)(h->cfg.pos_emb_max_len - 1 - (Tv - 1)) * D;
    GamGemmArgs gp = gemm_args(h->rel_pe + pe0, D, L.wpos, nullptr, h->pbuf.p, D, 2 * Tv - 1, D, D);
    if (p.sp) { gp.Asp = reinterpret_cast<const _Float16*>(h->rel_pe_sp + pe0); gp.a_fmt = 1; }
    if (int r = gemm(h, s, gp, GAM_ACT_NONE, GAM_PF_GEMM, &L.s_wpos)) return r;
  }
  {
    ProfScope ps(h, s, GAM_PF_ATTN, 4.0 * (double)p.B * p.H * (double)Tv * Tv * p.dk);
    if (int r = launch_attention(h, s, h->qkv.p, h->qkv.p + D, h->qkv.p + 2 * D, 3 * D, h->ctx.p, spf, p.B > 1 ? c.w.len2 : nullptr, c.w.cu, p.B,
                                 p.packed ? p.Tmax : p.Ta, Tv, p.H, p.rel ? h->pbuf.p : nullptr, L.pos_u, L.pos_v))
      return r;
  }
  GamGemmArgs go = gemm_args(h->ctx.p, D, L.wo, L.bo, h->x.p, D, NR, D, D);
  go.R = h->x.p; go.ldr = D;
  gemm_formats(go, spf, nullptr, 0, 0);
  return gemm(h, s, go, GAM_ACT_NONE, GAM_PF_GEMM, &L.s_wo, pend);
}

static int conv_block(gam_handle* h, hipStream_t s, const EncCtx& c, const LayerW& L, PendingReduce* pend) {
  const EncPlan& p = c.p;
  const int D = p.D, NR = p.NR, ks = h->cfg.conv_kernel_size;
  if (int r = norm_to_y(h, s, c, L.ln_conv_w, L.ln_conv_b, pend)) return r;
  GamGemmArgs g1 = gemm_args(h->y.p, D, L.pw1_w, L.pw1_b, h->ubuf.p, 2 * D, NR, 2 * D, D);
  gemm_formats(g1, p.spf, c.w.rs, 0, 0);
  if (int r = gemm(h, s, g1, GAM_ACT_NONE, GAM_PF_GEMM, &L.s_pw1)) return r;
  {
    ProfScope ps(h, s, GAM_PF_CONVMOD, (double)NR * D * 3 * 4.0);
    hipError_t e = launch_convmod(h, s, h->ubuf.p, h->zbuf.p, L.dw_w, L.dw_b, L.cn_scale, L.cn_shift, c.w.len2, c.w.cu, p.B,
                                  p.packed ? p.Tmax : p.Ta, p.Tv, D, ks, h->cfg.conv_norm_type == GAM_NORM_LAYER, p.spf);
    if (e != hipSuccess) return fail(h, -2, "conv-module launch (k=%d): %s", ks, hipGetErrorString(e));
  }
  GamGemmArgs g2 = gemm_args(h->zbuf.p, D, L.pw2_w, L.pw2_b, h->x.p, D, NR, D, D);
  g2.R = h->x.p; g2.ldr = D;
  gemm_formats(g2, p.spf, nullptr, 0, 0);
  return gemm(h, s, g2, GAM_ACT_NONE, GAM_PF_GEMM, &L.s_pw2, pend);
}

static int norm_out_block(gam_handle* h, hipStream_t s, const EncCtx& c, const LayerW& L, const LayerW* next, PendingReduce* pend) {
  GamLnArgs a = c.ln;
  a.x = h->x.p; a.out1 = h->x.p; a.w1 = L.ln_out_w; a.b1 = L.ln_out_b;
  if (next != nullptr) {
    a.out2 = h->y.p; a.w2 = next->ln_ff1_w; a.b2 = next->ln_ff1_b;
    a.split2 = c.p.spf;
    return layernorm(h, s, a, 2, pend);
  }
  a.rs = nullptr;
  return layernorm(h, s, a, 0, pend);
}

static int run_layers(gam_handle* h, hipStream_t s, const EncCtx& c) {
  const int nl = c.p.nl;
  if (nl > 0)
    if (int r = norm_to_y(h, s, c, h->layers[0].ln_ff1_w, h->layers[0].ln_ff1_b, nullptr)) return r;
  PendingReduce pend;
  for (int li = 0; li < nl; ++li) {
    const LayerW& L = h->layers[li];
    if (int r = ffn_block(h, s, c, L.ff1_w1, L.ff1_b1, L.s_ff1_w1, L.ff1_w2, L.ff1_b2, L.s_ff1_w2, &pend)) return r;
    if (int r = attn_block(h, s, c, L, &pend)) return r;
    if (int r = conv_block(h, s, c, L, &pend)) return r;
    if (int r = norm_to_y(h, s, c, L.ln_ff2_w, L.ln_ff2_b, &pend)) return r;
    if (int r = ffn_block(h, s, c, L.ff2_w1, L.ff2_b1, L.s_ff2_w1, L.ff2_w2, L.ff2_b2, L.s_ff2_w2, &pend)) return r;
    if (int r = norm_out_block(h, s, c, L, li + 1 < nl ? &h->layers[li + 1] : nullptr, &pend)) return r;
  }
  return flush_pending(h, s, &pend);
}

static int replay_layers(gam_handle* h, hipStream_t s, const EncCtx& c, bool* replayed) {
  typedef gam_handle::GraphEntry Entry;
  const EncPlan& p = c.p;
  *replayed = false;
  if (!p.graph) return 0;
  const GamSpForce& frc = gam_sp_force();
  const std::vector<int> key = {p.B, p.Ta, p.Tv, p.nl, h->gemm_mode, (int)p.sp, h->use_splitk, h->fuse_reduce, frc.mt.load(), frc.nw.load(), frc.s.load(), frc.ns.load()};
  Entry& ge = h->graphs[key];
  if (ge.gen != h->ws_generation) {
    if (ge.exec) { hipGraphExecDestroy(ge.exec); --h->graph_count; }
    ge = Entry();
    ge.gen = h->ws_generation;
  }
  if (ge.exec == nullptr && ge.seen == Entry::SEEN_ONCE && h->graph_count >= 32) ge.seen = Entry::PLAIN_ONLY;
  if (ge.exec == nullptr && ge.seen == Entry::SEEN_ONCE) {
    hipGraph_t graph = nullptr;
    if (h->cap_stream == nullptr && hipStreamCreateWithFlags(&h->cap_stream, hipStreamNonBlocking) != hipSuccess)
      h->cap_stream = nullptr;
    if (h->cap_stream != nullptr && hipStreamBeginCapture(h->cap_stream, hipStreamCaptureModeRelaxed) == hipSuccess) {
      const int r = run_layers(h, h->cap_stream, c);
      const hipError_t e = hipStreamEndCapture(h->cap_stream, &graph);
      if (r == 0 && e == hipSuccess && graph != nullptr && h->ws_generation == ge.gen &&
          hipGraphInstantiate(&ge.exec, graph, nullptr, nullptr, 0) != hipSuccess)
        ge.exec = nullptr;
      if (graph) hipGraphDestroy(graph);
    }
    (void)hipGetLastError();
    if (ge.exec == nullptr) { ge.seen = Entry::PLAIN_ONLY; ++h->graph_captures_failed; }
    else ++h->graph_count;
  }
  if (ge.exec != nullptr) {
    HIPCHK(h, hipGraphLaunch(ge.exec, s));
    *replayed = true;
    ++h->graph_replays;
  } else if (ge.seen == Entry::UNSEEN) {
    ge.seen = Entry::SEEN_ONCE;
  }
  return 0;
}

static int enc_outputs(gam_handle* h, hipStream_t s, const EncPlan& p, const EncBufs& w, float* encoded, float* tokens_out, int32_t* enc_len) {
  const int B = p.B, Ta = p.Ta, Tv = p.Tv, D = p.D;
  ProfScope ps(h, s, GAM_PF_MISC, (double)B * Tv * D * 8.0);
  if (encoded && p.packed) {
    hipLaunchKernelGGL(gam_unpack_transpose_kernel, dim3(gam_cdiv(D, 32), gam_cdiv(Tv, 32), B), dim3(256), 0, s, h->x.p, w.cu, w.len2, encoded, Tv, D);
    HIPCHK(h, hipGetLastError());
  } else if (encoded) {
    hipError_t e = gam_launch_transpose(h->x.p, encoded, B, Tv, D, (size_t)Ta * D, D, (size_t)D * Tv, Tv, s);
    if (e != hipSuccess) return fail(h, -2, "transpose launch: %s", hipGetErrorString(e));
  }
  if (tokens_out && p.packed) {
    hipLaunchKernelGGL(gam_unpack_rows_kernel, dim3(std::min(4096, gam_cdiv(B * Tv * (D / 4), 256))), dim3(256), 0, s, h->x.p, w.cu, w.len2, tokens_out, B, Tv, D);
    HIPCHK(h, hipGetLastError());
  } else if (tokens_out)
    HIPCHK(h, hipMemcpy2DAsync(tokens_out, (size_t)Tv * D * 4, h->x.p, (size_t)Ta * D * 4, (size_t)Tv * D * 4, B, hipMemcpyDeviceToDevice, s));
  if (enc_len) HIPCHK(h, hipMemcpyAsync(enc_len, w.elen, (size_t)B * sizeof(int), hipMemcpyDeviceToDevice, s));
  return 0;
}

static int encode_impl(gam_handle* h, const float* feat, const int64_t* feat_len, int B, int64_t T, float* encoded,
                       int32_t* enc_len, int n_layers_run, float* tokens_out, hipStream_t s, const int64_t* feat_len_host = nullptr) {
  if (!h || !h->finalized) return fail(h, -1, "gam_encode before gam_finalize");
  if (!h->has_encoder) return fail(h, -1, "this handle was finalized without encoder weights");
  EncCtx c;
  if (int r = enc_plan(h, B, T, n_layers_run, feat_len_host, c.p)) return r;
  HIPCHK(h, hipSetDevice(h->device));
  h->last_rows = c.p.NR;
  h->last_rows_padded = c.p.N;
  if (int r = enc_workspace(h, c.p, c.w)) return r;
  c.ln = enc_ln_args(h, c.p, c.w);
  if (int r = enc_lengths(h, s, c.p, c.w, feat_len)) return r;
  if (int r = enc_stem(h, s, c.p, c.w, feat)) return r;
  bool replayed = false;
  if (int r = replay_layers(h, s, c, &replayed)) return r;
  if (!replayed)
    if (int r = run_layers(h, s, c)) return r;
  return enc_outputs(h, s, c.p, c.w, encoded, tokens_out, enc_len);
}

int gam_encode(gam_handle* h, const float* feat, const int64_t* feat_len, int B, int64_t T, float* encoded, int32_t* enc_len,
               void* stream) {
  return encode_impl(h, feat, feat_len, B, T, encoded, enc_len, -1, nullptr, (hipStream_t)stream);
}

int gam_encode_ex(gam_handle* h, const float* feat, const int64_t* feat_len, int B, int64_t T, float* encoded, int32_t* enc_len,
                  int n_layers_run, float* tokens_out, void* stream) {
  return encode_impl(h, feat, feat_len, B, T, encoded, enc_len, n_layers_run, tokens_out, (hipStream_t)stream);
}

int gam_encode_varlen(gam_handle* h, const float* feat, const int64_t* feat_len, const int64_t* feat_len_host, int B, int64_t T,
// ... 1106 lines not shown

int gam_op_rnnt_confidence(gam_handle* h, const float* encp, const int32_t* enc_len, int B, int64_t Tp, const int32_t* ids,
                           const int32_t* frames, const int32_t* counts, int cap, int measure, float* conf, int32_t* status, void* stream) {
  if (int r = head_check(h, GAM_HEAD_RNNT, "RNN-T head")) return r;
  GAM_DECODE_ENTRY(h, stream);
  return rnnt_conf_launch(h, encp, enc_len, B, Tp, ids, frames, counts, cap, measure, conf, status, s);
}

int gam_rnnt_predict(gam_handle* h, const int32_t* labels, const float* h_in, const float* c_in, int B, float* g_out,
                     float* h_out, float* c_out, void* stream) {
  if (int r = head_check(h, GAM_HEAD_RNNT, "gam_rnnt_predict")) return r;
  if (B <= 0 || !g_out || !h_out || !c_out || (h_in == nullptr) != (c_in == nullptr)) return fail(h, -1, "bad gam_rnnt_predict arguments");
  HIPCHK(h, hipSetDevice(h->device));
  const gam_config& c = h->cfg;
  GamPredictArgs a;
  rnnt_pred_weights(h, a);
  a.label = labels; a.h_in = h_in; a.c_in = c_in; a.g_out = g_out; a.h_out = h_out; a.c_out = c_out;
  a.B = B; a.PH = c.pred_hidden; a.V = c.num_classes; a.L = c.pred_rnn_layers;
  hipStream_t s = (hipStream_t)stream;
  ProfScope ps(h, s, GAM_PF_DECODE, 0.0);
  hipLaunchKernelGGL(gam_rnnt_predict_kernel, dim3(B), dim3(256), (size_t)6 * c.pred_hidden * sizeof(float), s, a);
  HIPCHK(h, hipGetLastError());
  return 0;
}

int gam_rnnt_joint(gam_handle* h, const float* enc, const float* dec, int B, int T, int U, float* log_probs, void* stream) {
  if (int r = head_check(h, GAM_HEAD_RNNT, "gam_rnnt_joint")) return r;
  if (B <= 0 || T <= 0 || U <= 0 || !enc || !dec || !log_probs) return fail(h, -1, "bad gam_rnnt_joint arguments");
  HIPCHK(h, hipSetDevice(h->device));
  const gam_config& c = h->cfg;
  const int D = c.d_model, PH = c.pred_hidden, JH = c.joint_hidden, V = c.num_classes;
  const size_t rows = (size_t)B * T * U;
  if (rows * std::max(JH, V) > ((size_t)1 << 31)) return fail(h, -1, "gam_rnnt_joint: B x T x U = %zu rows is too large for one call", rows);
  hipStream_t s = (hipStream_t)stream;
  DecodeScope ds(h, s);
  if (int r = ensure(h, h->encp, (size_t)B * T * JH)) return r;
  if (int r = ensure(h, h->jp, (size_t)B * U * JH)) return r;
  if (int r = ensure(h, h->jz, rows * JH)) return r;
  if (int r = ensure(h, h->jl, rows * V)) return r;
  GamGemmArgs ge = gemm_args(enc, D, h->jn_enc_w, h->jn_enc_b, h->encp.p, JH, B * T, JH, D);
  if (int r = gemm(h, s, ge, GAM_ACT_NONE, GAM_PF_DECODE)) return r;
  GamGemmArgs gp = gemm_args(dec, PH, h->jn_pred_w, h->jn_pred_b, h->jp.p, JH, B * U, JH, PH);
  if (int r = gemm(h, s, gp, GAM_ACT_NONE, GAM_PF_DECODE)) return r;
  {
    ProfScope ps(h, s, GAM_PF_DECODE, (double)rows * JH * 4.0);
    const int grid = (int)std::min<size_t>((rows * JH + 255) / 256, 8192);
    hipLaunchKernelGGL(gam_joint_hidden_kernel, dim3(grid), dim3(256), 0, s, h->encp.p, h->jp.p, h->jz.p, B, T, U, JH);
    HIPCHK(h, hipGetLastError());
  }
  GamGemmArgs go = gemm_args(h->jz.p, JH, h->jn_out_w, h->jn_out_b, h->jl.p, V, (int)rows, V, JH);
  if (int r = gemm(h, s, go, GAM_ACT_NONE, GAM_PF_DECODE)) return r;
  ProfScope ps(h, s, GAM_PF_DECODE, (double)rows * V * 8.0);
  hipLaunchKernelGGL(gam_log_softmax_kernel, dim3(gam_cdiv((long)rows, 4)), dim3(256), 0, s, h->jl.p, log_probs, (int)rows, V);
  HIPCHK(h, hipGetLastError());
  return 0;
}

int gam_emo_probs(gam_handle* h, const float* encoded, const int32_t* enc_len, int B, int64_t Tp, float* probs,
                  void* stream) {
  if (int r = head_check(h, GAM_HEAD_EMO, nullptr)) return r;
  if (B <= 0 || Tp <= 0 || !encoded || !probs) return fail(h, -1, "bad emotion-head arguments");
  HIPCHK(h, hipSetDevice(h->device));
  hipStream_t s = (hipStream_t)stream;
  const int D = h->cfg.d_model, NC = h->cfg.num_classes;
  ProfScope ps(h, s, GAM_PF_DECODE, (double)B * D * Tp * 4.0);
  hipLaunchKernelGGL(gam_emo_head_kernel, dim3(B), dim3(256), (size_t)(D + NC) * sizeof(float), s, encoded, enc_len,
                     h->emo_w, h->emo_b, probs, D, (int)Tp, NC);
  HIPCHK(h, hipGetLastError());
  return 0;
}

int gam_op_gemm(gam_handle* h, const float* A, const float* W, const float* bias, float* C, int M, int N, int K, int act,
                void* stream) {
  return gam_op_gemm_ex(h, A, W, bias, nullptr, 1.0f, C, M, N, K, act, stream);
}

int gam_op_gemm_ex(gam_handle* h, const float* A, const float* W, const float* bias, const float* R, float alpha, float* C, int M,
                   int N, int K, int act, void* stream) {
  if (!h) return -1;
  HIPCHK(h, hipSetDevice(h->device));
  GamGemmArgs g = gemm_args(A, K, W, bias, C, N, M, N, K);
  g.R = R; g.ldr = N; g.alpha = alpha;
  hipStream_t s = (hipStream_t)stream;
  if (!split_mode(h) || K % 32 != 0 || N % 4 != 0) return gemm(h, s, g, act);
  const size_t wn = (size_t)N * K, an = (size_t)M * K;
  W16 w16;
  if (int r = ensure(h, h->op_sp, wn + 64)) return r;
  hipLaunchKernelGGL(gam_to_sp32_kernel, dim3((int)std::min<size_t>((wn / 4 + 255) / 256, 4096)), dim3(256), 0, s, W,
                     (_Float16*)h->op_sp.p, wn / 4, (const float*)nullptr, K);
  w16.sp = (_Float16*)h->op_sp.p;
  if (int r = ensure(h, h->op_rs, (size_t)M + 64)) return r;
  hipLaunchKernelGGL(gam_rowscale_kernel, dim3(gam_cdiv(M, 4)), dim3(256), 0, s, A, h->op_rs.p, M, K, (long)K);
  g.a_rs = h->op_rs.p;
  if (int r = ensure(h, h->aplanes, an + 64)) return r;
  g.Asp = (const _Float16*)h->aplanes.p;
  g.a_fmt = (h->gemm_mode == GAM_GEMM_F16 && K % 64 == 0) ? 2 : 1;
  if (g.a_fmt == 2) {
    if (int r = ensure(h, h->op_planes, wn / 2 + 64)) return r;
    w16.h16 = (_Float16*)h->op_planes.p;
    hipLaunchKernelGGL(gam_to_h16_kernel, dim3((int)std::min<size_t>((wn / 4 + 255) / 256, 4096)), dim3(256), 0, s, W, w16.h16,
                       wn / 4, (const float*)nullptr, K);
    hipLaunchKernelGGL(gam_to_h16_kernel, dim3((int)std::min<size_t>((an / 4 + 255) / 256, 8192)), dim3(256), 0, s, A,
                       (_Float16*)h->aplanes.p, an / 4, (const float*)h->op_rs.p, K);
  } else {
    hipLaunchKernelGGL(gam_to_sp32_kernel, dim3((int)std::min<size_t>((an / 4 + 255) / 256, 8192)), dim3(256), 0, s, A,
                       (_Float16*)h->aplanes.p, an / 4, (const float*)h->op_rs.p, K);
  }
  return gemm(h, s, g, act, GAM_PF_GEMM, &w16);
}

int gam_op_attention(gam_handle* h, const float* q, const float* k, const float* v, float* ctx, const int32_t* lens, int B,
                     int T, int H, void* stream) {
  if (!h) return -1;
  if (B <= 0 || T <= 0 || H <= 0) return fail(h, -1, "bad attention shape");
  HIPCHK(h, hipSetDevice(h->device));
  return launch_attention(h, (hipStream_t)stream, q, k, v, H * GAM_ATT_DK, ctx, 0, lens, nullptr, B, T, T, H, nullptr, nullptr, nullptr);
}

int gam_op_attention_ex(gam_handle* h, const float* q, const float* k, const float* v, int64_t ldq, float* ctx, const int32_t* lens,
                        const int32_t* cu, int B, int Ta, int Tv, int H, const float* pbuf, const float* pos_u, const float* pos_v,
                        void* stream) {
  if (!h) return -1;
  const int D = H * GAM_ATT_DK;
  if (B <= 0 || Ta <= 0 || Tv <= 0 || H <= 0) return fail(h, -1, "bad attention shape");
  if (cu == nullptr && Tv > Ta) return fail(h, -1, "attention: Tv %d > Ta %d in the padded layout", Tv, Ta);
  if (ldq < D || ldq % 4 != 0) return fail(h, -1, "attention: row stride %ld (H*48 = %d, multiple of 4)", (long)ldq, D);
  if (pbuf != nullptr && (pos_u == nullptr || pos_v == nullptr)) return fail(h, -1, "attention: pbuf without pos_u / pos_v");
  auto al16 = [](const void* p) { return (reinterpret_cast<uintptr_t>(p) & 15) == 0; };
  if (!al16(q) || !al16(k) || !al16(v) || !al16(ctx) || (pbuf && (!al16(pbuf) || !al16(pos_u) || !al16(pos_v))))
    return fail(h, -1, "attention: operands must be 16-byte aligned");
  HIPCHK(h, hipSetDevice(h->device));
  return launch_attention(h, (hipStream_t)stream, q, k, v, (long)ldq, ctx, 0, lens, cu, B, Ta, Tv, H, pbuf, pos_u, pos_v);
}

int gam_op_layernorm(gam_handle* h, const gam_ln_op* op, void* stream) {
  if (!h) return -1;
  if (!op) return fail(h, -1, "layernorm: null argument block");
  const gam_ln_op& o = *op;
  if (o.mode < 0 || o.mode > 2) return fail(h, -1, "layernorm: mode %d outside 0..2", o.mode);
  if (o.rows <= 0 || o.d <= 0) return fail(h, -1, "layernorm: bad shape rows %d d %d", o.rows, o.d);
  if (o.split1 < 0 || o.split1 > 2 || o.split2 < 0 || o.split2 > 2)
    return fail(h, -1, "layernorm: store format %d / %d outside 0..2", o.split1, o.split2);
  if (!o.out1 || !o.w1 || !o.b1) return fail(h, -1, "layernorm: out1 / w1 / b1 are mandatory");
  if (!o.part && !o.x) return fail(h, -1, "layernorm: x is mandatory without part");
  if (o.part && o.mode != 2 && !o.xstore) return fail(h, -1, "layernorm: part without xstore");
  if (o.mode != 0 && !o.out2) return fail(h, -1, "layernorm: mode %d needs out2", o.mode);
  if (o.mode == 2 && (!o.w2 || !o.b2)) return fail(h, -1, "layernorm: mode 2 needs w2 / b2");
  if (o.mode == 1) {
    if (!o.rcos || !o.rsin || o.rope_rows <= 0) return fail(h, -1, "layernorm: mode 1 needs rcos / rsin of rope_rows > 0 rows");
    if (o.dk <= 0) return fail(h, -1, "layernorm: mode 1 needs dk > 0");
    if (!o.row_t && o.ta <= 0) return fail(h, -1, "layernorm: mode 1 needs row_t or ta > 0");
  }
  auto al16 = [](const void* p) { return (reinterpret_cast<uintptr_t>(p) & 15) == 0; };
  if (!al16(o.x) || !al16(o.out1) || !al16(o.out2) || !al16(o.w1) || !al16(o.b1) || !al16(o.w2) || !al16(o.b2) || !al16(o.rcos) ||
      !al16(o.rsin) || !al16(o.part) || !al16(o.pbias) || !al16(o.presid) || !al16(o.xstore))
    return fail(h, -1, "layernorm: operands must be 16-byte aligned");
  HIPCHK(h, hipSetDevice(h->device));
  GamLnArgs a;
  memset(&a, 0, sizeof a);
  a.x = o.x; a.out1 = o.out1; a.out2 = o.out2; a.w1 = o.w1; a.b1 = o.b1; a.w2 = o.w2; a.b2 = o.b2;
  a.rcos = o.rcos; a.rsin = o.rsin; a.rows = o.rows; a.d = o.d; a.ta = o.ta; a.dk = o.dk; a.eps = o.eps;
  a.split1 = o.split1; a.split2 = o.split2; a.rs = o.rs; a.rope_rows = o.rope_rows;
  a.part = o.part; a.nsplit = o.nsplit; a.pbias = o.pbias; a.presid = o.presid; a.palpha = o.palpha; a.xstore = o.xstore;
  a.row_t = o.row_t;
  hipError_t e = gam_launch_layernorm(a, o.mode, (hipStream_t)stream);
  if (e != hipSuccess)
    return fail(h, -2, "layernorm launch (mode %d, rows %d, d %d, dk %d, split %d/%d, nsplit %d): %s", o.mode, o.rows, o.d, o.dk,
                o.split1, o.split2, o.part ? o.nsplit : 0, hipGetErrorString(e));
  return 0;
}

int gam_op_convmod(gam_handle* h, const float* u, float* z, const float* dw_w, const float* dw_b, const float* n_scale,
                   const float* n_shift, const int32_t* lens, const int32_t* cu, int B, int Ta, int Tv, int d, int ks, int layer_norm,
                   int z_split, void* stream) {
  if (!h) return -1;
  if (!h->finalized) return fail(h, -1, "gam_op_convmod before gam_finalize");
  if (!u || !z || !dw_w || !dw_b || !n_scale || !n_shift || !lens) return fail(h, -1, "conv module: null operand");
  if (B <= 0 || Ta <= 0 || Tv <= 0 || d <= 0) return fail(h, -1, "conv module: bad shape B %d Ta %d Tv %d d %d", B, Ta, Tv, d);
  if (cu == nullptr && Tv > Ta) return fail(h, -1, "conv module: Tv %d > Ta %d in the padded layout", Tv, Ta);
  if (z_split < 0 || z_split > 2) return fail(h, -1, "conv module: store format %d outside 0..2", z_split);
  if (z_split && d % 32 != 0) return fail(h, -1, "conv module: a split-fp16 z needs d %% 32 == 0 (d = %d)", d);
  auto al16 = [](const void* p) { return (reinterpret_cast<uintptr_t>(p) & 15) == 0; };
  if (d % 4 == 0 && (!al16(u) || !al16(z) || !al16(dw_b) || !al16(n_scale) || !al16(n_shift)))
    return fail(h, -1, "conv module: operands must be 16-byte aligned");
  HIPCHK(h, hipSetDevice(h->device));
  hipError_t e = launch_convmod(h, (hipStream_t)stream, u, z, dw_w, dw_b, n_scale, n_shift, lens, cu, B, Ta, Tv, d, ks, layer_norm != 0, z_split);
  if (e != hipSuccess) return fail(h, -2, "conv-module launch (k=%d, d=%d, %s): %s", ks, d, layer_norm ? "LayerNorm" : "BatchNorm", hipGetErrorString(e));
  return 0;
}

int gam_set_gemm_mode(gam_handle* h, int mode) {
  if (!h || (mode != GAM_GEMM_F32 && mode != GAM_GEMM_F16X3 && mode != GAM_GEMM_F16)) return fail(h, -1, "unknown GEMM mode %d", mode);
  h->gemm_mode = mode;
  return 0;
}

int gam_get_gemm_mode(const gam_handle* h) { return h ? h->gemm_mode : -1; }

int gam_debug_buffer_hash(gam_handle* h, int which, uint64_t* hash_out, int64_t* floats_out) {
  if (!h || !hash_out) return -1;
  const DevBuf* b = which == 0 ? &h->tok : which == 1 ? &h->encp : which == 2 ? &h->rnnt_x : which == 3 ? &h->logits : nullptr;
  if (!b) return fail(h, -1, "no such buffer %d", which);
  HIPCHK(h, hipSetDevice(h->device));
  HIPCHK(h, hipDeviceSynchronize());
  std::vector<uint32_t> host(b->cap);
  if (b->cap) HIPCHK(h, hipMemcpy(host.data(), b->p, b->cap * sizeof(float), hipMemcpyDeviceToHost));
  uint64_t x = 1469598103934665603ull;
  for (uint32_t v : host) { x ^= v; x *= 1099511628211ull; }
  *hash_out = x;
  if (floats_out) *floats_out = (int64_t)b->cap;
  return 0;
}

int gam_set_rnnt_cluster(gam_handle* h, int workgroups_per_utterance) {
  if (!h) return -1;
  if (workgroups_per_utterance < -1 || workgroups_per_utterance > 8) return fail(h, -1, "cluster size %d outside -1 (auto) .. 8", workgroups_per_utterance);
  h->rnnt_cluster = workgroups_per_utterance;
  return 0;
}

int gam_get_rnnt_cluster(gam_handle* h) { return h ? h->rnnt_cluster : -2; }

int gam_rnnt_cluster_plan_info(int ncu, int cluster, int exclusive, int B, int H, int JH, int V, int L, int32_t* out) {
  if (!out || B <= 0 || H <= 0 || JH <= 0 || V <= 0 || L <= 0) return -1;
  const RnntClusterPlan p = rnnt_cluster_plan(ncu, cluster, exclusive, B, H, JH, V, L);
  memset(out, 0, 8 * sizeof(int32_t));
  if (p.C == 0) return 0;
  out[0] = p.C; out[1] = p.nr; out[2] = p.kern; out[3] = p.resident ? 1 : 0;
  out[4] = p.wout_slice_in_lds; out[5] = p.wpred_slice_in_lds; out[6] = (int32_t)p.lds; out[7] = (int32_t)p.grid;
  return 0;
}

int gam_rnnt_last_decode(gam_handle* h, int32_t* out) {
  if (!h || !out) return -1;
  out[0] = h->last_rnnt_c; out[1] = h->last_rnnt_kern; out[2] = h->last_rnnt_refused;
  return 0;
}

int gam_last_encode_rows(gam_handle* h, int* rows_padded) {
  if (!h) return -1;
  if (rows_padded) *rows_padded = h->last_rows_padded;
  return h->last_rows;
}

int gam_range_flag(gam_handle* h, int* flag_host, void* stream) {
  if (!h || !flag_host) return -1;
  if (!h->finalized) return fail(h, -1, "gam_range_flag before gam_finalize");
  HIPCHK(h, hipSetDevice(h->device));
  hipStream_t s = (hipStream_t)stream;
  HIPCHK(h, hipMemcpyAsync(flag_host, h->range_flag, sizeof(int), hipMemcpyDeviceToHost, s));
  HIPCHK(h, hipMemsetAsync(h->range_flag, 0, sizeof(int), s));
  HIPCHK(h, hipStreamSynchronize(s));
  return 0;
}

int gam_range_flag_fetch(gam_handle* h, int32_t* flag_dev, void* stream) {
  if (!h || !flag_dev) return -1;
  if (!h->finalized) return fail(h, -1, "gam_range_flag_fetch before gam_finalize");
  HIPCHK(h, hipSetDevice(h->device));
  hipStream_t s = (hipStream_t)stream;
  HIPCHK(h, hipMemcpyAsync(flag_dev, h->range_flag, sizeof(int), hipMemcpyDeviceToDevice, s));
  HIPCHK(h, hipMemsetAsync(h->range_flag, 0, sizeof(int), s));
  return 0;
}

int gam_plan_sp(int M, int N, int K, int n_cu, int* mt, int* nw, int* splitk) {
  if (M <= 0 || N <= 0 || K <= 0 || K % 32 != 0 || !mt || !nw || !splitk) return -1;
  const GamSpPlan p = gam_gemm_sp_plan(M, N, K, 0, n_cu > 0 ? n_cu : 256);
  *mt = p.mt; *nw = p.nw; *splitk = p.s;
// ... 100 lines not shown
```

### gigaam_amd/csrc/gam_common.h

```cpp
#pragma once
#include <hip/hip_runtime.h>
#include <stdint.h>
#include <math.h>

#define GAM_WAVE 64

typedef float f32x4 __attribute__((ext_vector_type(4)));
typedef float f32x2 __attribute__((ext_vector_type(2)));
typedef float f32x16 __attribute__((ext_vector_type(16)));

static inline int gam_cdiv(long a, long b) { return (int)((a + b - 1) / b); }

#include <atomic>
static inline hipError_t gam_set_max_lds(const void* kern, int bytes, std::atomic<unsigned long long>& mask) {
  int dev = 0;
  hipError_t e = hipGetDevice(&dev);
  if (e != hipSuccess) return e;
  const unsigned long long bit = 1ull << (dev & 63);
  if (mask.load(std::memory_order_acquire) & bit) return hipSuccess;
  e = hipFuncSetAttribute(kern, hipFuncAttributeMaxDynamicSharedMemorySize, bytes);
  if (e == hipSuccess) mask.fetch_or(bit, std::memory_order_release);
  return e;
}

// ... 97 lines not shown
    e = e < -40 ? -40 : (e > 40 ? 40 : e);
  }
  s = __builtin_ldexpf(1.0f, e);
  inv = __builtin_ldexpf(1.0f, -e);
}

#define GAM_F16_SAFE_MAX 60000.0f
__device__ __forceinline__ void gam_range_note(int* flag, float a, float b, float c, float d) {
  if (flag != nullptr && fmaxf(fmaxf(fabsf(a), fabsf(b)), fmaxf(fabsf(c), fabsf(d))) > GAM_F16_SAFE_MAX) atomicOr(flag, 1);
}

__device__ __forceinline__ void gam_store4(float* base, size_t row_off, int c, float x0, float x1, float x2, float x3,
                                           int split) {
  if (!split) {
    *reinterpret_cast<f32x4*>(base + row_off + c) = (f32x4){x0, x1, x2, x3};
  } else if (split == 2) {
    *reinterpret_cast<gam_half4*>(reinterpret_cast<_Float16*>(base) + row_off + c) = __builtin_convertvector((f32x4){x0, x1, x2, x3}, gam_half4);
  } else {
    _Float16* p = reinterpret_cast<_Float16*>(base) + row_off * 2 + (c >> 5) * 64 + (c & 31);
    gam_half4 hi, lo;
    gam_split4((f32x4){x0, x1, x2, x3}, hi, lo);
    *reinterpret_cast<gam_half4*>(p) = hi;
    *reinterpret_cast<gam_half4*>(p + 32) = lo;
  }
}
__device__ __forceinline__ void gam_store2(float* base, size_t row_off, int c, float x0, float x1, int split) {
  if (!split) {
    *reinterpret_cast<float2*>(base + row_off + c) = make_float2(x0, x1);
  } else if (split == 2) {
    *reinterpret_cast<gam_half2*>(reinterpret_cast<_Float16*>(base) + row_off + c) = __builtin_convertvector((f32x2){x0, x1}, gam_half2);
  } else {
    _Float16* p = reinterpret_cast<_Float16*>(base) + row_off * 2 + (c >> 5) * 64 + (c & 31);
    unsigned h, l;
    gam_split2(x0, x1, h, l);
    *reinterpret_cast<unsigned*>(p) = h;
    *reinterpret_cast<unsigned*>(p + 32) = l;
  }
}
__device__ __forceinline__ void gam_store1(float* base, size_t row_off, int c, float x, int split) {
  if (!split) {
    base[row_off + c] = x;
  } else if (split == 2) {
    reinterpret_cast<_Float16*>(base)[row_off + c] = (_Float16)x;
  } else {
    _Float16* p = reinterpret_cast<_Float16*>(base) + row_off * 2 + (c >> 5) * 64 + (c & 31);
    const _Float16 h = (_Float16)x;
    p[0] = h;
    p[32] = (_Float16)(x - (float)h);
  }
}

template <int NS>
__device__ __forceinline__ f32x4 gam_sum_slices_n(const float* __restrict__ p, size_t slice) {
  f32x4 t[NS];
#pragma unroll
  for (int s_ = 0; s_ < NS; ++s_) t[s_] = *reinterpret_cast<const f32x4*>(p + s_ * slice);
  f32x4 acc = (f32x4){0.f, 0.f, 0.f, 0.f};
#pragma unroll
  for (int s_ = 0; s_ < NS; ++s_) acc += t[s_];
  return acc;
}
template <int SMAX = 16>
__device__ __forceinline__ f32x4 gam_sum_slices(const float* __restrict__ p, size_t slice, int ns) {
  switch (ns) {
    case 1: return gam_sum_slices_n<1>(p, slice);
    case 2: return gam_sum_slices_n<2>(p, slice);
    case 3: return gam_sum_slices_n<3>(p, slice);
    case 4: return gam_sum_slices_n<4>(p, slice);
    default: break;
  }
  if (SMAX >= 8) {
    if (ns == 6) return gam_sum_slices_n<6>(p, slice);
    if (ns == 8) return gam_sum_slices_n<8>(p, slice);
  }
  if (SMAX >= 16) {
    if (ns == 12) return gam_sum_slices_n<12>(p, slice);
    if (ns == 16) return gam_sum_slices_n<16>(p, slice);
  }
  f32x4 acc = (f32x4){0.f, 0.f, 0.f, 0.f};
  for (int s_ = 0; s_ < ns; ++s_) acc += *reinterpret_cast<const f32x4*>(p + s_ * slice);
  return acc;
}

enum { GAM_ACT_NONE = 0, GAM_ACT_SILU = 1, GAM_ACT_RELU = 2 };
```

### gigaam_amd/csrc/gam_convmod.h

```cpp
#pragma once
#include "gam_common.h"
#include "gam_pack.h"
#include <type_traits>

struct GamConvModArgs {
  const float* u;
  float* z;
  const float* dw_w;
  const float* dw_b;
  const float* n_scale;
  const float* n_shift;
  const int* lens;
  const int* cu;
  int B, Ta, Tv, d, ks;
  float eps;
  int z_split;
  int* range_flag;
};

template <int KS>
__global__ __launch_bounds__(512, 4) void gam_convmod_bn_kernel(GamConvModArgs a) {
  constexpr int NRG = 32, TT = 128, PAD = (KS - 1) / 2, ROWS = (TT + KS - 1 + NRG - 1) / NRG * NRG, OUT = TT / NRG;
  __shared__ f32x4 tile[ROWS * 16];
  __shared__ f32x4 wl[KS * 16];
  const int tid = threadIdx.x;
  const int q = tid & 15, rg = tid >> 4;
  const int b = blockIdx.z, c = blockIdx.y * 64 + q * 4, t0 = blockIdx.x * TT;
  int klen = a.lens[b];
  klen = klen < a.Tv ? klen : a.Tv;
  const GamRows ur = gam_rows(a.cu, b, a.Ta, klen);
  if (t0 >= ur.lim) return;
  const size_t rowbase = ur.base;
  const int rlim = ur.lim;
  constexpr int NLD = ROWS / NRG;
  f32x4 ua[NLD], ub[NLD];
#pragma unroll
  for (int u = 0; u < NLD; ++u) {
    const int t = t0 - PAD + rg + NRG * u;
    const int tc = t < 0 ? 0 : (t < rlim ? t : rlim - 1);
    const float* up = a.u + (rowbase + tc) * (size_t)(2 * a.d);
    ua[u] = *reinterpret_cast<const f32x4*>(up + c);
    ub[u] = *reinterpret_cast<const f32x4*>(up + a.d + c);
  }
  {
#pragma unroll
    for (int i = 0; i < (KS + NRG - 1) / NRG; ++i) {
      const int k = rg + NRG * i;
      if (k < KS) wl[k * 16 + q] = (f32x4){a.dw_w[(size_t)c * KS + k], a.dw_w[(size_t)(c + 1) * KS + k],
                                           a.dw_w[(size_t)(c + 2) * KS + k], a.dw_w[(size_t)(c + 3) * KS + k]};
    }
  }
#pragma unroll
  for (int u = 0; u < NLD; ++u) {
    const int rr = rg + NRG * u;
    const int t = t0 - PAD + rr;
    const bool live = t >= 0 && t < klen;
    const f32x4 glu = (f32x4){ua[u].x * gam_sigmoid(ub[u].x), ua[u].y * gam_sigmoid(ub[u].y),
                              ua[u].z * gam_sigmoid(ub[u].z), ua[u].w * gam_sigmoid(ub[u].w)};
    tile[rr * 16 + q] = live ? glu : (f32x4){0.f, 0.f, 0.f, 0.f};
  }
  __syncthreads();
  const f32x4* trow = tile + (rg * OUT) * 16 + q;
  const f32x4* wq = wl + q;
  int lofs = 0;
  f32x4 win[OUT + KS - 1];
#pragma unroll
  for (int r = 0; r < OUT + 1; ++r) win[r] = trow[r * 16];
  f32x4 acc[OUT];
#pragma unroll
  for (int i = 0; i < OUT; ++i) acc[i] = (f32x4){0.f, 0.f, 0.f, 0.f};
  f32x4 w_cur = wq[0], w_nxt = wq[16];
#pragma unroll
  for (int k = 0; k < KS; ++k) {
    const f32x4 w = w_cur;
    w_cur = w_nxt;
#pragma unroll
    for (int i = 0; i < OUT; ++i) {
      acc[i].x = fmaf(w.x, win[i + k].x, acc[i].x);
      acc[i].y = fmaf(w.y, win[i + k].y, acc[i].y);
      acc[i].z = fmaf(w.z, win[i + k].z, acc[i].z);
      acc[i].w = fmaf(w.w, win[i + k].w, acc[i].w);
    }
    static_assert(OUT == 4, "the pin below names the 16 accumulator components of a tap");
    asm volatile("" : "+v"(lofs), "+v"(acc[0].x), "+v"(acc[0].y), "+v"(acc[0].z), "+v"(acc[0].w), "+v"(acc[1].x), "+v"(acc[1].y),
                 "+v"(acc[1].z), "+v"(acc[1].w), "+v"(acc[2].x), "+v"(acc[2].y), "+v"(acc[2].z), "+v"(acc[2].w), "+v"(acc[3].x),
                 "+v"(acc[3].y), "+v"(acc[3].z), "+v"(acc[3].w));
    if (k + 2 < KS) w_nxt = wq[(k + 2) * 16 + lofs];
    if (k + OUT + 1 < OUT + KS - 1) win[k + OUT + 1] = trow[(k + OUT + 1) * 16 + lofs];
  }
  const f32x4 bias = *reinterpret_cast<const f32x4*>(a.dw_b + c);
  const f32x4 sc = *reinterpret_cast<const f32x4*>(a.n_scale + c);
  const f32x4 sh = *reinterpret_cast<const f32x4*>(a.n_shift + c);
#pragma unroll
  for (int i = 0; i < OUT; ++i) {
    const int t = t0 + rg * OUT + i;
    const f32x4 y = (acc[i] + bias) * sc + sh;
    const float v0 = gam_silu(y.x), v1 = gam_silu(y.y), v2 = gam_silu(y.z), v3 = gam_silu(y.w);
    if (t < rlim) {
      gam_range_note(a.range_flag, v0, v1, v2, v3);
      gam_store4(a.z, (rowbase + t) * (size_t)a.d, c, v0, v1, v2, v3, a.z_split);
    }
  }
}

template <int KS>
__global__ __launch_bounds__(256) void gam_convmod_ln_kernel(GamConvModArgs a) {
  constexpr int TT = 8, PAD = (KS - 1) / 2, ROWS = TT + KS - 1, MAXC = 4;
  extern __shared__ __attribute__((aligned(16))) float gam_smem_cm[];
  float* tile = gam_smem_cm;
  float* red = gam_smem_cm + ROWS * a.d;
  const int tid = threadIdx.x, lane = tid & 63, wave = tid >> 6;
  const int b = blockIdx.y, t0 = blockIdx.x * TT;
  int klen = a.lens[b];
  klen = klen < a.Tv ? klen : a.Tv;
  const GamRows ur = gam_rows(a.cu, b, a.Ta, klen);
  if (t0 >= ur.lim) return;
  const size_t rowbase = ur.base;
  const int rlim = ur.lim;
  for (int r0 = 0; r0 < ROWS; r0 += 4) {
    float ua[4][MAXC], ub[4][MAXC];
#pragma unroll
    for (int q = 0; q < 4; ++q) {
      const int t = t0 - PAD + r0 + q;
      const int tc = t < 0 ? 0 : (t < rlim ? t : rlim - 1);
      const float* up = a.u + (rowbase + tc) * (size_t)(2 * a.d);
#pragma unroll
      for (int ci = 0; ci < MAXC; ++ci) {
        const int c = tid + ci * 256 < a.d ? tid + ci * 256 : a.d - 1;
        ua[q][ci] = up[c];
        ub[q][ci] = up[a.d + c];
      }
    }
#pragma unroll
    for (int q = 0; q < 4; ++q) {
      const int rr = r0 + q, t = t0 - PAD + rr;
      const bool ok = t >= 0 && t < klen;
#pragma unroll
      for (int ci = 0; ci < MAXC; ++ci) {
        const int c = tid + ci * 256;
        if (rr < ROWS && c < a.d) tile[rr * a.d + c] = ok ? ua[q][ci] * gam_sigmoid(ub[q][ci]) : 0.f;
      }
// ... 77 lines not shown
  const int c = live ? tid * 4 : 0;
  int klen = a.lens[b];
  klen = klen < a.Tv ? klen : a.Tv;
  const GamRows ur = gam_rows(a.cu, b, a.Ta, klen);
  if (t0 >= ur.lim) return;
  const size_t rowbase = ur.base;
  const int rlim = ur.lim;
  f32x4 ua[ROWS], ub[ROWS];
#pragma unroll
  for (int r = 0; r < ROWS; ++r) {
    const int t = t0 - PAD + r;
    const int tc = t < 0 ? 0 : (t < rlim ? t : rlim - 1);
    const float* up = a.u + (rowbase + tc) * (size_t)(2 * a.d);
    ua[r] = *reinterpret_cast<const f32x4*>(up + c);
    ub[r] = *reinterpret_cast<const f32x4*>(up + a.d + c);
  }
  f32x4 w[KS];
#pragma unroll
  for (int k = 0; k < KS; ++k)
    w[k] = (f32x4){a.dw_w[(size_t)c * KS + k], a.dw_w[(size_t)(c + 1) * KS + k], a.dw_w[(size_t)(c + 2) * KS + k],
                   a.dw_w[(size_t)(c + 3) * KS + k]};
  const f32x4 bias = *reinterpret_cast<const f32x4*>(a.dw_b + c);
#pragma unroll
  for (int r = 0; r < ROWS; ++r) {
    const int t = t0 - PAD + r;
    const bool live = t >= 0 && t < klen;
    const f32x4 glu = (f32x4){ua[r].x * gam_sigmoid(ub[r].x), ua[r].y * gam_sigmoid(ub[r].y), ua[r].z * gam_sigmoid(ub[r].z),
                              ua[r].w * gam_sigmoid(ub[r].w)};
    ua[r] = live ? glu : (f32x4){0.f, 0.f, 0.f, 0.f};
  }
  f32x4 y[TT];
#pragma unroll
  for (int i = 0; i < TT; ++i) {
    f32x4 acc = (f32x4){0.f, 0.f, 0.f, 0.f};
#pragma unroll
    for (int k = 0; k < KS; ++k) {
      acc.x = fmaf(w[k].x, ua[i + k].x, acc.x);
      acc.y = fmaf(w[k].y, ua[i + k].y, acc.y);
      acc.z = fmaf(w[k].z, ua[i + k].z, acc.z);
      acc.w = fmaf(w[k].w, ua[i + k].w, acc.w);
    }
    y[i] = acc + bias;
  }
  float mean[TT], rstd[TT];
#pragma unroll
  for (int i = 0; i < TT; ++i) {
    float s = live ? (y[i].x + y[i].y) + (y[i].z + y[i].w) : 0.f;
    s = gam_wave_sum(s);
    if (lane == 0) red[wave][i] = s;
  }
  __syncthreads();
#pragma unroll
  for (int i = 0; i < TT; ++i) mean[i] = (red[0][i] + red[1][i] + red[2][i] + red[3][i]) / (float)a.d;
  __syncthreads();
#pragma unroll
  for (int i = 0; i < TT; ++i) {
    const float d0 = y[i].x - mean[i], d1 = y[i].y - mean[i], d2 = y[i].z - mean[i], d3 = y[i].w - mean[i];
    float s = live ? (d0 * d0 + d1 * d1) + (d2 * d2 + d3 * d3) : 0.f;
    s = gam_wave_sum(s);
    if (lane == 0) red[wave][i] = s;
  }
  __syncthreads();
#pragma unroll
  for (int i = 0; i < TT; ++i) rstd[i] = 1.0f / sqrtf((red[0][i] + red[1][i] + red[2][i] + red[3][i]) / (float)a.d + a.eps);
  if (!live) return;
  const f32x4 gm = *reinterpret_cast<const f32x4*>(a.n_scale + c);
  const f32x4 be = *reinterpret_cast<const f32x4*>(a.n_shift + c);
#pragma unroll
  for (int i = 0; i < TT; ++i) {
    const int t = t0 + i;
    if (t < rlim) {
      const float v0 = gam_silu((y[i].x - mean[i]) * rstd[i] * gm.x + be.x), v1 = gam_silu((y[i].y - mean[i]) * rstd[i] * gm.y + be.y);
      const float v2 = gam_silu((y[i].z - mean[i]) * rstd[i] * gm.z + be.z), v3 = gam_silu((y[i].w - mean[i]) * rstd[i] * gm.w + be.w);
      gam_range_note(a.range_flag, v0, v1, v2, v3);
      gam_store4(a.z, (rowbase + t) * (size_t)a.d, c, v0, v1, v2, v3, a.z_split);
    }
  }
}

static inline hipError_t gam_launch_convmod(const GamConvModArgs& a, int layer_norm, hipStream_t s) {
  if (!layer_norm) {
    if (a.d % 64 != 0) return hipErrorInvalidValue;
    dim3 grid(gam_cdiv(a.Ta, 128), a.d / 64, a.B);
    if (a.ks == 31) hipLaunchKernelGGL(gam_convmod_bn_kernel<31>, grid, dim3(512), 0, s, a);
    else if (a.ks == 5) hipLaunchKernelGGL(gam_convmod_bn_kernel<5>, grid, dim3(512), 0, s, a);
    else if (a.ks == 9) hipLaunchKernelGGL(gam_convmod_bn_kernel<9>, grid, dim3(512), 0, s, a);
    else return hipErrorInvalidValue;
  } else {
    if (a.d > 1024) return hipErrorInvalidValue;
    dim3 grid(gam_cdiv(a.Ta, 8), a.B);
    if ((a.ks == 5 || a.ks == 9) && a.d % 4 == 0) {
      dim3 g4(gam_cdiv(a.Ta, 16), a.B);
      if (a.ks == 5) hipLaunchKernelGGL(gam_convmod_ln4_kernel<5>, g4, dim3(256), 0, s, a);
      else hipLaunchKernelGGL(gam_convmod_ln4_kernel<9>, g4, dim3(256), 0, s, a);
    } else if (a.ks == 5) {
      const size_t sm = ((8 + 4) * a.d + 32) * sizeof(float);
      hipLaunchKernelGGL(gam_convmod_ln_kernel<5>, grid, dim3(256), sm, s, a);
    } else if (a.ks == 31) {
      const size_t sm = ((8 + 30) * a.d + 32) * sizeof(float);
      static std::atomic<unsigned long long> attr_devs{0};
      if (hipError_t e = gam_set_max_lds(reinterpret_cast<const void*>(gam_convmod_ln_kernel<31>), 160 * 1024, attr_devs)) return e;
      hipLaunchKernelGGL(gam_convmod_ln_kernel<31>, grid, dim3(256), sm, s, a);
    } else if (a.ks == 9) {
      const size_t sm = ((8 + 8) * a.d + 32) * sizeof(float);
      if (sm > 64 * 1024) {
        static std::atomic<unsigned long long> attr_devs9{0};
        if (hipError_t e = gam_set_max_lds(reinterpret_cast<const void*>(gam_convmod_ln_kernel<9>), 160 * 1024, attr_devs9)) return e;
      }
      hipLaunchKernelGGL(gam_convmod_ln_kernel<9>, grid, dim3(256), sm, s, a);
    } else return hipErrorInvalidValue;
  }
  return hipGetLastError();
}
```

### gigaam_amd/csrc/gam_gemm_sp.h

```cpp
#pragma once
#include "gam_gemm.h"
#include <type_traits>
#if defined(GAM_SP_INSTRUMENT) && GAM_SP_INSTRUMENT
#include <algorithm>
#include <vector>
#endif

#ifndef GAM_SP_INSTRUMENT
#define GAM_SP_INSTRUMENT 0
#endif
#define GAM_SP_DBG(g) (GAM_SP_INSTRUMENT ? (g).dbg : 0)
#if GAM_SP_INSTRUMENT
#define GAM_SP_TL(i)                                                                  \
  if ((GAM_SP_DBG(g) & 16) && g.tlog != nullptr && threadIdx.x == 0) {                        \
    g.tlog[(size_t)lid * 8 + (i)] = wall_clock64();                                   \
    if ((i) == 1 || (i) == 2) g.tlog[(size_t)lid * 8 + 4 + (i)] = clock64();          \
    if ((i) == 0) g.tlog[(size_t)lid * 8 + 7] = blockIdx.x;                            \
  }
#else
#define GAM_SP_TL(i)
#endif

template <int MT, int NW, int NS = 2>
struct GamGemmSpCfg {
// ... 251 lines not shown
  const int mw = m0 + wm * (BM / 2), nw = n0 + wn * 64;
  if ((GAM_SP_DBG(g) & 1) && acc[0][0][0] != 123.456f) return;

  const int lrow = lane & 15, lq8 = (lane >> 4) * 8;
  const float accscale = g.wscale_inv;
  f32x4 bv[2][2];
#pragma unroll
  for (int pp = 0; pp < 2; ++pp)
#pragma unroll
    for (int hf = 0; hf < 2; ++hf) {
      const int col = nw + 32 * pp + lq8 + 4 * hf;
      bv[pp][hf] = (g.bias != nullptr && col < g.N) ? *reinterpret_cast<const f32x4*>(g.bias + col) : (f32x4){0.f, 0.f, 0.f, 0.f};
    }
  const bool part = g.partial != nullptr;
  const bool need_bt = !part && (g.lens != nullptr || g.remap);
  bool r_ok[2 * MT], r_masked[2 * MT];
  long r_orow[2 * MT];
  float r_rsc[2 * MT];
  int bb = 0, tt = 0;
  if (need_bt) { bb = (mw + lrow) / g.rpb; tt = (mw + lrow) - bb * g.rpb; }
#pragma unroll
  for (int i = 0; i < 2 * MT; ++i) {
    const int row = mw + 16 * i + lrow;
    bool ok = row < g.M, masked = false;
    long orow = row;
    if (need_bt) {
      if (i > 0) {
        tt += 16;
        if (g.rpb < 16) { bb = row / g.rpb; tt = row - bb * g.rpb; }
        else if (tt >= g.rpb) { tt -= g.rpb; ++bb; }
      }
      if (ok) {
        if (g.lens != nullptr) masked = tt >= g.lens[bb] * g.fdiv;
        if (g.remap) {
          if (tt >= g.rows_valid) ok = false;
          orow = (long)bb * g.out_rpb + tt + g.out_shift;
        }
      }
    }
    r_rsc[i] = accscale * ((ok && g.a_rs != nullptr) ? g.a_rs[row] : 1.0f);
    r_ok[i] = ok; r_masked[i] = masked; r_orow[i] = orow;
  }
  if (part) {
#pragma unroll
    for (int i = 0; i < 2 * MT; ++i) {
      if (!r_ok[i]) continue;
      float* P = g.partial + ((size_t)blockIdx.y * (size_t)g.M + (size_t)(mw + 16 * i + lrow)) * (size_t)g.N;
#pragma unroll
      for (int pp = 0; pp < 2; ++pp)
#pragma unroll
        for (int hf = 0; hf < 2; ++hf) {
          const int ecol = nw + 32 * pp + lq8 + 4 * hf;
          if (ecol < g.N) *reinterpret_cast<f32x4*>(P + ecol) = acc[i][2 * pp + hf] * r_rsc[i];
        }
    }
  }
#define GAM_SP_LDR(I, D)                                                                          \
  _Pragma("unroll") for (int pp = 0; pp < 2; ++pp) _Pragma("unroll") for (int hf = 0; hf < 2; ++hf) { \
    const int col = nw + 32 * pp + lq8 + 4 * hf;                                                  \
    D[pp][hf] = (r_ok[I] && col < g.N) ? *reinterpret_cast<const f32x4*>(g.R + r_orow[I] * g.ldr + col) : (f32x4){0.f, 0.f, 0.f, 0.f}; \
  }
  f32x4 rv[2][2], rn[2][2];
  const bool resid = g.R != nullptr && !part;
  if (resid) GAM_SP_LDR(0, rv);
#pragma unroll
  for (int i = 0; i < 2 * MT; ++i) {
    if (resid && i + 1 < 2 * MT) GAM_SP_LDR(i + 1, rn);
    const bool masked = r_masked[i];
    const long orow = r_orow[i];
    const float rsc = r_rsc[i];
    if (r_ok[i] && !part) {
#pragma unroll
      for (int pp = 0; pp < 2; ++pp) {
        const int ecol = nw + 32 * pp + lq8;
        if (ecol >= g.N) continue;
        const bool both = ecol + 4 < g.N;
        f32x4 v[2];
#pragma unroll
        for (int hf = 0; hf < 2; ++hf) {
          f32x4 t = acc[i][2 * pp + hf];
          t = t * rsc + bv[pp][hf];
          if (ACT == GAM_ACT_SILU) { t.x = gam_silu(t.x); t.y = gam_silu(t.y); t.z = gam_silu(t.z); t.w = gam_silu(t.w); }
          if (ACT == GAM_ACT_RELU) { t.x = fmaxf(t.x, 0.f); t.y = fmaxf(t.y, 0.f); t.z = fmaxf(t.z, 0.f); t.w = fmaxf(t.w, 0.f); }
          if (masked) t = (f32x4){0.f, 0.f, 0.f, 0.f};
          t = t * g.alpha;
          if (resid) t += rv[pp][hf];
          if (!both && hf == 1) t = (f32x4){0.f, 0.f, 0.f, 0.f};
          v[hf] = t;
        }
        if (g.c_guard) { gam_range_note(g.range_flag, v[0].x, v[0].y, v[0].z, v[0].w); gam_range_note(g.range_flag, v[1].x, v[1].y, v[1].z, v[1].w); }
        if ((GAM_SP_DBG(g) & 32) && v[0].x != 123.456f) continue;
        if (g.c_split == 2) {
          _Float16* cp = reinterpret_cast<_Float16*>(g.C) + orow * g.ldc + ecol;
          const gam_half4 h0 = __builtin_convertvector(v[0], gam_half4), h1 = __builtin_convertvector(v[1], gam_half4);
          if (both) *reinterpret_cast<gam_half8*>(cp) = (gam_half8){h0[0], h0[1], h0[2], h0[3], h1[0], h1[1], h1[2], h1[3]};
          else *reinterpret_cast<gam_half4*>(cp) = h0;
        } else if (g.c_split) {
          _Float16* cp = reinterpret_cast<_Float16*>(g.C) + orow * (2 * g.ldc) + (ecol >> 5) * 64 + (ecol & 31);
          gam_half4 hi0, lo0, hi1, lo1;
          gam_split4(v[0], hi0, lo0);
          gam_split4(v[1], hi1, lo1);
          if (both) {
            *reinterpret_cast<gam_half8*>(cp) = (gam_half8){hi0[0], hi0[1], hi0[2], hi0[3], hi1[0], hi1[1], hi1[2], hi1[3]};
            *reinterpret_cast<gam_half8*>(cp + 32) = (gam_half8){lo0[0], lo0[1], lo0[2], lo0[3], lo1[0], lo1[1], lo1[2], lo1[3]};
          } else {
            *reinterpret_cast<gam_half4*>(cp) = hi0;
            *reinterpret_cast<gam_half4*>(cp + 32) = lo0;
          }
        } else {
          *reinterpret_cast<f32x4*>(g.C + orow * g.ldc + ecol) = v[0];
          if (both) *reinterpret_cast<f32x4*>(g.C + orow * g.ldc + ecol + 4) = v[1];
        }
      }
    }
    if (resid && i + 1 < 2 * MT) {
#pragma unroll
      for (int pp = 0; pp < 2; ++pp)
#pragma unroll
        for (int hf = 0; hf < 2; ++hf) rv[pp][hf] = rn[pp][hf];
    }
  }
#undef GAM_SP_LDR
#if GAM_SP_INSTRUMENT
  if (GAM_SP_DBG(g) & 16) { __builtin_amdgcn_s_waitcnt(0x0070); __syncthreads(); }
  GAM_SP_TL(3);
#endif
}

static inline bool gam_gemm_sp_epilogue_ok(const GamGemmArgs& a) {
  auto al16 = [](const void* p) { return (reinterpret_cast<uintptr_t>(p) & 15) == 0; };
  return a.N % 4 == 0 && a.ldc % 4 == 0 && al16(a.C) && (a.bias == nullptr || al16(a.bias)) &&
         (a.R == nullptr || (a.ldr % 4 == 0 && al16(a.R)));
}

template <int ACT, int MT, int NW, int NS = 2, bool H16 = false>
static inline void gam_launch_gemm_sp_t(const GamGemmArgs& a, int grid, hipStream_t stream) {
  static std::atomic<unsigned long long> attr_devs{0};
  constexpr int smem = GamGemmSpCfg<MT, NW, NS>::SMEM;
  static_assert(smem <= 160 * 1024, "LDS stages do not fit a CU");
  auto kern = gam_gemm_sp_kernel<ACT, MT, NW, NS, H16>;
  if (gam_set_max_lds(reinterpret_cast<const void*>(kern), smem, attr_devs) != hipSuccess) return;
  hipLaunchKernelGGL(kern, dim3(grid, a.splitk > 1 ? a.splitk : 1), dim3(128 * NW), smem, stream, a);
}

struct GamSpPlan { int mt, nw, s, ns; };
struct GamSpForce {
  std::atomic<int> mt{0}, nw{0}, s{0}, ns{0};
  GamSpForce() {
    const char* e0 = getenv("GAM_SP_MT"); const char* e1 = getenv("GAM_SP_NW"); const char* e2 = getenv("GAM_SP_SPLITK");
    const char* e3 = getenv("GAM_SP_STAGES");
    mt = e0 ? atoi(e0) : 0; nw = e1 ? atoi(e1) : 0; s = e2 ? atoi(e2) : 0; ns = e3 ? atoi(e3) : 0;
  }
};
static inline bool gam_sp_has_ns3(int mt, int nw) { return (nw == 2 && (mt == 2 || mt == 3)) || (nw == 4 && mt == 2); }
static inline GamSpForce& gam_sp_force() { static GamSpForce f; return f; }
static inline int gam_env_int_once(const char* name) { const char* e = getenv(name); return e ? atoi(e) : 0; }
static inline double gam_gemm_sp_model(int M, int N, int K, int a_mode, int t, int w, int S, int ncu, int ns = 2) {
  const long wgs = (long)gam_cdiv(M, 64 * t) * gam_cdiv(N, 64 * w) * S;
  const int nkt = K / 32 / S;
  double t_kt, t_fix, rounds;
  if (ns == 3) {
    if (w == 4) { t_kt = 0.953; t_fix = S > 1 ? 6.62 : 12.8; }
    else { t_kt = 0.229 * t + 0.115; t_fix = S > 1 ? 4.76 : 12.0; }
    rounds = (double)((wgs + ncu - 1) / ncu);
  } else if (w == 4) {
    t_kt = 0.335 * t + 0.425;
    t_fix = S > 1 ? 6.2 : 13.2;
    rounds = (double)((wgs + ncu - 1) / ncu);
  } else {
    const bool shared = wgs > ncu;
    const double tk_u = 0.256 * t + 0.142, tf_u = S > 1 ? 4.9 : 14.1;
    t_kt = tk_u * (shared ? 1.82 : 1.0);
    t_fix = tf_u * (shared ? 0.73 : 1.0);
    rounds = (double)((wgs + (shared ? 2 : 1) * ncu - 1) / ((shared ? 2 : 1) * ncu));
    const long cap2 = 2L * ncu, rem = wgs % cap2;
    if (shared && wgs > cap2 && rem != 0 && rem <= ncu) {
      (void)a_mode;
      double us2 = (double)(wgs / cap2) * (nkt * t_kt + t_fix) + (nkt * tk_u + tf_u);
      if (S > 1) us2 += 7.1 + (double)(S + 2) * M * N * 4.0 / 3.87e6;
      return us2;
    }
  }
  (void)a_mode;
  double us = rounds * (nkt * t_kt + t_fix);
  if (S > 1) us += 7.1 + (double)(S + 2) * M * N * 4.0 / 3.87e6;
  return us;
}
static inline GamSpPlan gam_gemm_sp_plan(int M, int N, int K, int a_mode = 0, int ncu = 256) {
  GamSpForce& frc = gam_sp_force();
  const int f_mt = frc.mt.load(std::memory_order_relaxed), f_nw = frc.nw.load(std::memory_order_relaxed);
  int f_s = frc.s.load(std::memory_order_relaxed), f_ns = frc.ns.load(std::memory_order_relaxed);
  GamSpPlan best = {3, 4, 1, 2};
  double bt = 1e30;
  const int nk = K / 32;
  if (f_s > 1 && (f_s > 8 || nk % f_s != 0 || nk / f_s < 4)) f_s = 1;
  if (f_ns == 3 && a_mode != 0) f_ns = 2;
  for (int w = 4; w >= 2; w -= 2) {
    if ((f_nw == 2 || f_nw == 4) && w != f_nw) continue;
    for (int t = (w == 2 ? 3 : 4); t >= 2; --t) {
      if (f_mt >= 2 && f_mt <= 4 && t != f_mt && !(w == 2 && f_mt == 4)) continue;
      for (int S = 1; S <= 8; ++S) {
        if (f_s >= 1 && S != f_s) continue;
        if (S > 1 && (nk % S != 0 || nk / S < 4)) continue;
        if (f_s < 1 && S > 1 && (long)gam_cdiv(M, 64 * t) * gam_cdiv(N, 64 * w) * 2 > ncu) continue;
        for (int ns = 2; ns <= 3; ++ns) {
          if (ns == 3 && (!gam_sp_has_ns3(t, w) || a_mode != 0)) continue;
          if ((f_ns == 2 || f_ns == 3) && ns != f_ns && !(f_ns == 3 && !gam_sp_has_ns3(t, w))) continue;
          const double us = gam_gemm_sp_model(M, N, K, a_mode, t, w, S, ncu, ns);
          if (us < bt - 1e-9) { bt = us; best = {t, w, S, ns}; }
        }
      }
    }
  }
  return best;
}

static inline hipError_t gam_launch_gemm_sp(const GamGemmArgs& a_in, int act, hipStream_t stream) {
  GamGemmArgs a = a_in;
  if (a.M <= 0 || a.N <= 0) return hipSuccess;
  if (a.K <= 0 || a.K % 32 != 0 || a.Asp == nullptr || a.Wsp == nullptr) return hipErrorInvalidValue;
  if (a.a_mode == 0 ? (a.lda % 32 != 0) : (a.conv_c % 32 != 0)) return hipErrorInvalidValue;
  if (!gam_gemm_sp_epilogue_ok(a)) return hipErrorInvalidValue;
  int mt = a.sp_mt, nw = a.sp_nw, ns = a.sp_ns;
  if (mt < 2 || mt > 4 || (nw != 2 && nw != 4) || (nw == 2 && mt == 4)) {
    const GamSpPlan p = gam_gemm_sp_plan(a.M, a.N, a.K, a.a_mode);
    mt = p.mt; nw = p.nw; ns = p.ns;
    if (a.splitk > 1 && a.partial == nullptr) return hipErrorInvalidValue;
  }
  if (ns != 3 || !gam_sp_has_ns3(mt, nw)) ns = 2;
  if (a.splitk > 1 && (a.partial == nullptr || (a.K / 32) % a.splitk != 0)) return hipErrorInvalidValue;
  if (a.n_switch > 0 && (a.Asp2 == nullptr || a.a_mode != 0 || a.n_switch % (64 * nw) != 0)) return hipErrorInvalidValue;
  if (a.splitk <= 1) { a.splitk = 0; a.partial = nullptr; }
  const int grid = gam_cdiv(a.M, 64 * mt) * gam_cdiv(a.N, 64 * nw);
  a.ntiles = grid;
#if GAM_SP_INSTRUMENT
  static const int dbg = gam_env_int_once("GAM_SP_DBG"), prio = gam_env_int_once("GAM_SP_PRIO"), order = gam_env_int_once("GAM_SP_ORDER");
#else
  constexpr int dbg = 0, prio = 0, order = 0;
#endif
  a.dbg = dbg;
  a.prio = prio;
  a.tile_order = order;
#if GAM_SP_INSTRUMENT
  static long long* tl_dev = nullptr;
  static int tl_cap = 0;
  if (dbg & 16) {
    if (grid > tl_cap) { if (tl_dev) (void)hipFree(tl_dev); (void)hipMalloc(&tl_dev, (size_t)grid * 64); tl_cap = grid; }
    (void)hipMemsetAsync(tl_dev, 0, (size_t)grid * 64, stream);
    a.tlog = tl_dev;
  }
#endif
#define GAM_LSP(ACTV)                                                            \
  if (a.h16) {           \
    if (ns == 3) {                                                               \
      if (nw == 4) gam_launch_gemm_sp_t<ACTV, 2, 4, 3, true>(a, grid, stream);   \
      else if (mt == 2) gam_launch_gemm_sp_t<ACTV, 2, 2, 3, true>(a, grid, stream); \
      else gam_launch_gemm_sp_t<ACTV, 3, 2, 3, true>(a, grid, stream);           \
    } else if (nw == 2) {                                                        \
      if (mt == 2) gam_launch_gemm_sp_t<ACTV, 2, 2, 2, true>(a, grid, stream);   \
      else gam_launch_gemm_sp_t<ACTV, 3, 2, 2, true>(a, grid, stream);           \
    } else switch (mt) {                                                         \
      case 2: gam_launch_gemm_sp_t<ACTV, 2, 4, 2, true>(a, grid, stream); break; \
      case 3: gam_launch_gemm_sp_t<ACTV, 3, 4, 2, true>(a, grid, stream); break; \
      default: gam_launch_gemm_sp_t<ACTV, 4, 4, 2, true>(a, grid, stream); break; \
    }                                                                            \
  } else if (ns == 3) {                                                          \
    if (nw == 4) gam_launch_gemm_sp_t<ACTV, 2, 4, 3>(a, grid, stream);           \
    else if (mt == 2) gam_launch_gemm_sp_t<ACTV, 2, 2, 3>(a, grid, stream);      \
    else gam_launch_gemm_sp_t<ACTV, 3, 2, 3>(a, grid, stream);                   \
  } else if (nw == 2) switch (mt) {                                              \
    case 2: gam_launch_gemm_sp_t<ACTV, 2, 2>(a, grid, stream); break;            \
    default: gam_launch_gemm_sp_t<ACTV, 3, 2>(a, grid, stream); break;           \
  } else switch (mt) {                                                           \
    case 2: gam_launch_gemm_sp_t<ACTV, 2, 4>(a, grid, stream); break;            \
    case 3: gam_launch_gemm_sp_t<ACTV, 3, 4>(a, grid, stream); break;            \
    default: gam_launch_gemm_sp_t<ACTV, 4, 4>(a, grid, stream); break;           \
  }
  switch (act) {
    case GAM_ACT_SILU: GAM_LSP(GAM_ACT_SILU); break;
    case GAM_ACT_RELU: GAM_LSP(GAM_ACT_RELU); break;
    default: GAM_LSP(GAM_ACT_NONE); break;
  }
#undef GAM_LSP
#if GAM_SP_INSTRUMENT
  if ((dbg & 16) && getenv("GAM_SP_TLOG")) {
    std::vector<long long> t((size_t)grid * 8);
    (void)hipStreamSynchronize(stream);
    (void)hipMemcpy(t.data(), tl_dev, t.size() * 8, hipMemcpyDeviceToHost);
    long long t_first = t[0], t_last = 0;
    for (int i = 0; i < grid; ++i) { t_first = std::min(t_first, t[i * 8]); t_last = std::max(t_last, t[i * 8 + 3]); }
    auto stat = [&](auto f, const char* name) {
      std::vector<double> v(grid);
      for (int i = 0; i < grid; ++i) v[i] = f(i);
      std::sort(v.begin(), v.end());
      fprintf(stderr, "    %-26s min %7.2f  p50 %7.2f  p90 %7.2f  max %7.2f us\n", name, v[0], v[grid / 2], v[(size_t)(grid * 0.9)], v[grid - 1]);
    };
    fprintf(stderr, "[tlog] M=%d N=%d K=%d MT=%d NW=%d tiles=%d: first entry -> last exit %.2f us\n", a.M, a.N, a.K, mt, nw, grid, (t_last - t_first) * 0.01);
    stat([&](int i) { return (t[i * 8] - t_first) * 0.01; }, "entry after first entry");
    stat([&](int i) { return (t[i * 8 + 1] - t[i * 8]) * 0.01; }, "prologue (2 k-tiles land)");
    stat([&](int i) { return (t[i * 8 + 2] - t[i * 8 + 1]) * 0.01; }, "main loop");
    stat([&](int i) { return (t[i * 8 + 2] - t[i * 8 + 1]) * 0.01 / (a.K / 32); }, "  per k-tile");
    stat([&](int i) { return (double)(t[i * 8 + 6] - t[i * 8 + 5]) / std::max<long long>(1, t[i * 8 + 2] - t[i * 8 + 1]) * 100.0; }, "  shader MHz in loop");
    stat([&](int i) { return (t[i * 8 + 3] - t[i * 8 + 2]) * 0.01; }, "epilogue");
    stat([&](int i) { return (t_last - t[i * 8 + 3]) * 0.01; }, "idle after exit");
    double x_loop[8] = {0}; int x_n[8] = {0};
    for (int i = 0; i < grid; ++i) { const int x = (int)(t[i * 8 + 7] & 7); x_loop[x] += (t[i * 8 + 2] - t[i * 8 + 1]) * 0.01; ++x_n[x]; }
    fprintf(stderr, "    mean loop us by XCD:");
    for (int x = 0; x < 8; ++x) fprintf(stderr, " %.1f", x_n[x] ? x_loop[x] / x_n[x] : 0.0);
    fprintf(stderr, "\n");
  }
#endif
  return hipGetLastError();
}

__global__ __launch_bounds__(256) void gam_to_sp32_kernel(const float* __restrict__ x, _Float16* __restrict__ y,
                                                          size_t n4, const float* __restrict__ rs, int K) {
  const size_t stride = (size_t)gridDim.x * 256;
  for (size_t i = (size_t)blockIdx.x * 256 + threadIdx.x; i < n4; i += stride) {
    f32x4 v = reinterpret_cast<const f32x4*>(x)[i];
    const size_t e = i * 4;
    if (rs != nullptr) v = v * (1.0f / rs[e / (size_t)K]);
    gam_half4 h, l;
    gam_split4(v, h, l);
    _Float16* p = y + (e >> 5) * 64 + (e & 31);
    *reinterpret_cast<gam_half4*>(p) = h;
    *reinterpret_cast<gam_half4*>(p + 32) = l;
  }
}

__global__ __launch_bounds__(256) void gam_to_h16_kernel(const float* __restrict__ x, _Float16* __restrict__ y, size_t n4,
                                                         const float* __restrict__ rs, int K) {
  const size_t stride = (size_t)gridDim.x * 256;
  for (size_t i = (size_t)blockIdx.x * 256 + threadIdx.x; i < n4; i += stride) {
    f32x4 v = reinterpret_cast<const f32x4*>(x)[i];
    if (rs != nullptr) v = v * (1.0f / rs[(i * 4) / (size_t)K]);
    reinterpret_cast<gam_half4*>(y)[i] = __builtin_convertvector(v, gam_half4);
  }
}

__global__ __launch_bounds__(256) void gam_rowscale_kernel(const float* __restrict__ x, float* __restrict__ rs, int rows,
                                                           int K, long lda) {
  const int row = blockIdx.x * 4 + (threadIdx.x >> 6), lane = threadIdx.x & 63;
  if (row >= rows) return;
  const float* xr = x + (size_t)row * lda;
  float m = 0.f;
  for (int k = lane; k < K; k += 64) m = fmaxf(m, fabsf(xr[k]));
  m = gam_wave_max(m);
  float s_, inv_;
  gam_row_scale(m, s_, inv_);
  if (lane == 0) rs[row] = inv_;
}
```

### gigaam_amd/engine.py

```python
from __future__ import annotations

import contextlib
import ctypes as C
import functools
import math
import os
import threading
from typing import Any, Callable, Dict, List, Mapping, Optional, Sequence, Tuple

import numpy as np
import torch
from torch import Tensor

from . import _lib
from ._lib import GamConfig, GigaAMHipError


def _get(cfg: Any, key: str, default: Any = None) -> Any:
    if cfg is None:
        return default
    if isinstance(cfg, Mapping):
        return cfg.get(key, default)
    return getattr(cfg, key, default)

# ... 978 lines not shown

    @staticmethod
    def side_cluster(b: int, side_cus: int) -> int:
        if "GAM_DEBUG_SIDE_CLUSTER" in os.environ:
            return int(os.environ["GAM_DEBUG_SIDE_CLUSTER"])
        return max(1, min(8, side_cus // (8 * ((b + 7) // 8))))

    def rnnt_greedy(self, encoded: Tensor, enc_len: Tensor, max_symbols: int, dump_cap: int = 0, overlap: bool = False,
                    side_cus: int = 0) -> Decoded:
        encoded, enc_len, b, tp = self._in_encoded(encoded, enc_len)
        cap = tp * max_symbols
        main = torch.cuda.current_stream(self.device)
        side = self._decode_side_stream() if overlap else None
        ids, frames, counts = out = Decoded.packed(self.device, b, cap)
        whole, word = out.whole, out.flag_word()
        if overlap:
            with torch.cuda.device(self.device):
                self._fetch_flag(word)
            side.wait_stream(main)
            c_side = self.side_cluster(b, side_cus if side_cus > 0 else (96 if self.cfg.num_classes <= 64 else 160))
            self._check(self.lib.gam_set_rnnt_cluster(self._h, c_side), "gam_set_rnnt_cluster")
        try:
            with torch.cuda.stream(side) if overlap else torch.cuda.device(self.device):
                dump = dcount = None
                if dump_cap > 0:
                    dump = torch.zeros((b, dump_cap, self.cfg.num_classes), dtype=torch.float32, device=self.device)
                    dcount = torch.zeros((b,), dtype=torch.int32, device=self.device)
                rc = self.lib.gam_rnnt_greedy(self._h, _ptr(encoded), _ptr(enc_len), b, tp, max_symbols, _ptr(ids),
                                              _ptr(frames), _ptr(counts), _ptr(dump), _ptr(dcount), dump_cap, self._stream())
                self._check(rc, "gam_rnnt_greedy")
                if overlap:
                    st = torch.cuda.current_stream(self.device)
                    evt = torch.cuda.Event()
                    evt.record(st)
                    for t in (encoded, enc_len, whole):
                        t.record_stream(st)
                else:
                    evt, st = self._fetch_flag(word)
        finally:
            if overlap:
                self._check(self.lib.gam_set_rnnt_cluster(self._h, self._rnnt_cluster_user), "gam_set_rnnt_cluster")
        return Decoded(ids, frames, counts, out.ext, evt, st, dump, dcount, whole=whole)

    def rnnt_predict(self, labels: Optional[Tensor], state: Optional[Tuple[Tensor, Tensor]], batch_size: int = 1):
        ph, nl = self.cfg.pred_hidden, self.cfg.pred_rnn_layers
        if labels is not None:
            labels = self._dev(labels.reshape(-1), torch.int32)
            b = labels.shape[0]
        else:
            b = batch_size if state is None else state[0].shape[1]
        h_in = c_in = None
        if state is not None:
            h_in, c_in = self._dev(state[0], torch.float32), self._dev(state[1], torch.float32)
            if tuple(h_in.shape) != (nl, b, ph) or tuple(c_in.shape) != (nl, b, ph):
                raise GigaAMHipError(f"predictor state must be two [{nl},{b},{ph}] tensors, got {tuple(h_in.shape)} / {tuple(c_in.shape)}")
        g = torch.empty((b, ph), dtype=torch.float32, device=self.device)
        h_out = torch.empty((nl, b, ph), dtype=torch.float32, device=self.device)
        c_out = torch.empty_like(h_out)
        with torch.cuda.device(self.device):
            rc = self.lib.gam_rnnt_predict(self._h, _ptr(labels), _ptr(h_in), _ptr(c_in), b, _ptr(g), _ptr(h_out), _ptr(c_out), self._stream())
        self._check(rc, "gam_rnnt_predict")
        return g, (h_out, c_out)

    def rnnt_joint(self, enc: Tensor, dec: Tensor) -> Tensor:
        enc, dec = self._dev(enc, torch.float32), self._dev(dec, torch.float32)
        b, t, d = enc.shape
        b2, u, ph = dec.shape
        if b != b2 or d != self.cfg.d_model or ph != self.cfg.pred_hidden:
            raise GigaAMHipError(f"joint expects [B,T,{self.cfg.d_model}] and [B,U,{self.cfg.pred_hidden}], got {tuple(enc.shape)} / {tuple(dec.shape)}")
        out = torch.empty((b, t, u, self.cfg.num_classes), dtype=torch.float32, device=self.device)
        with torch.cuda.device(self.device):
            rc = self.lib.gam_rnnt_joint(self._h, _ptr(enc), _ptr(dec), b, t, u, _ptr(out), self._stream())
        self._check(rc, "gam_rnnt_joint")
        return out

    def op_gemm(self, a: Tensor, w: Tensor, bias: Optional[Tensor] = None, act: int = 0, resid: Optional[Tensor] = None,
                alpha: float = 1.0) -> Tensor:
        a = self._dev(a, torch.float32)
        w = self._dev(w, torch.float32)
        bias = None if bias is None else self._dev(bias, torch.float32)
        resid = None if resid is None else self._dev(resid, torch.float32)
        m, k = a.shape
        n = w.shape[0]
        out = torch.empty((m, n), dtype=torch.float32, device=self.device)
        with torch.cuda.device(self.device):
            rc = self.lib.gam_op_gemm_ex(self._h, _ptr(a), _ptr(w), _ptr(bias), _ptr(resid), alpha, _ptr(out), m, n, k, act,
                                         self._stream())
        self._check(rc, "gam_op_gemm_ex")
        return out

    def op_attention(self, q: Tensor, k: Tensor, v: Tensor, lens: Optional[Tensor] = None) -> Tensor:
        q, k, v = (self._dev(t, torch.float32) for t in (q, k, v))
        b, t, d = q.shape
        lens_d = None if lens is None else self._dev(lens, torch.int32)
        out = torch.empty_like(q)
        with torch.cuda.device(self.device):
            rc = self.lib.gam_op_attention(self._h, _ptr(q), _ptr(k), _ptr(v), _ptr(out), _ptr(lens_d), b, t, d // 48, self._stream())
        self._check(rc, "gam_op_attention")
        return out

    def op_attention_ex(self, q: Tensor, k: Tensor, v: Tensor, B: int, Ta: int, Tv: int, H: int, lens: Optional[Tensor] = None,
                        cu: Optional[Tensor] = None, pbuf: Optional[Tensor] = None, pos_u: Optional[Tensor] = None,
                        pos_v: Optional[Tensor] = None) -> Tensor:
        ldq = q.stride(0)
        if not (q.is_cuda and k.is_cuda and v.is_cuda) or k.stride(0) != ldq or v.stride(0) != ldq or any(t.stride(1) != 1 for t in (q, k, v)):
            raise GigaAMHipError("op_attention_ex: q, k, v must be CUDA row views with one row stride")
        lens_d, cu_d = (None if t is None else self._dev(t, torch.int32) for t in (lens, cu))
        pbuf, pos_u, pos_v = (None if t is None else self._dev(t, torch.float32) for t in (pbuf, pos_u, pos_v))
        out = torch.full((q.shape[0], H * 48), float("nan"), dtype=torch.float32, device=self.device)
        with torch.cuda.device(self.device):
            rc = self.lib.gam_op_attention_ex(self._h, _ptr(q), _ptr(k), _ptr(v), ldq, _ptr(out), _ptr(lens_d), _ptr(cu_d), B, Ta, Tv, H,
                                              _ptr(pbuf), _ptr(pos_u), _ptr(pos_v), self._stream())
        self._check(rc, "gam_op_attention_ex")
        return out

    def _op_ptr(self, what: str, name: str, t: Optional[Tensor], dtype: torch.dtype = torch.float32) -> Optional[int]:
        if t is None:
            return None
        if not (t.is_cuda and t.device == self.device and t.dtype == dtype and t.is_contiguous()):
            raise GigaAMHipError(f"{what}: {name} must be a contiguous {dtype} tensor on {self.device}")
        return t.data_ptr()

    def op_layernorm(self, mode: int, rows: int, d: int, x: Optional[Tensor], out1: Tensor, w1: Tensor, b1: Tensor, *,
                     out2: Optional[Tensor] = None, w2: Optional[Tensor] = None, b2: Optional[Tensor] = None, split1: int = 0,
                     split2: int = 0, rs: Optional[Tensor] = None, rcos: Optional[Tensor] = None, rsin: Optional[Tensor] = None,
                     dk: int = 0, ta: int = 0, rope_rows: Optional[int] = None, row_t: Optional[Tensor] = None,
                     part: Optional[Tensor] = None, nsplit: int = 0, pbias: Optional[Tensor] = None, presid: Optional[Tensor] = None,
                     palpha: float = 1.0, xstore: Optional[Tensor] = None, eps: float = 1e-5) -> None:
        what = "op_layernorm"
        op = _lib.GamLnOp()
        for name, t in (("x", x), ("out1", out1), ("out2", out2), ("w1", w1), ("b1", b1), ("w2", w2), ("b2", b2), ("rcos", rcos),
                        ("rsin", rsin), ("rs", rs), ("part", part), ("pbias", pbias), ("presid", presid), ("xstore", xstore)):
            setattr(op, name, self._op_ptr(what, name, t))
        op.row_t = self._op_ptr(what, "row_t", row_t, torch.int32)
        op.mode, op.rows, op.d, op.split1, op.split2, op.dk, op.ta, op.nsplit = mode, rows, d, split1, split2, dk, ta, nsplit
        op.rope_rows = (0 if rcos is None else rcos.shape[0]) if rope_rows is None else rope_rows
        op.eps, op.palpha = eps, palpha
        with torch.cuda.device(self.device):
            rc = self.lib.gam_op_layernorm(self._h, C.byref(op), self._stream())
        self._check(rc, "gam_op_layernorm")

    def op_convmod(self, u: Tensor, z: Tensor, dw_w: Tensor, dw_b: Tensor, n_scale: Tensor, n_shift: Tensor, lens: Tensor, B: int,
                   Ta: int, Tv: int, d: int, ks: int, layer_norm: bool, z_split: int = 0, cu: Optional[Tensor] = None) -> None:
        what = "op_convmod"
        ptrs = [self._op_ptr(what, n, t) for n, t in (("u", u), ("z", z), ("dw_w", dw_w), ("dw_b", dw_b), ("n_scale", n_scale),
                                                      ("n_shift", n_shift))]
        ptrs += [self._op_ptr(what, "lens", lens, torch.int32), self._op_ptr(what, "cu", cu, torch.int32)]
        with torch.cuda.device(self.device):
            rc = self.lib.gam_op_convmod(self._h, *ptrs, B, Ta, Tv, d, ks, int(bool(layer_norm)), z_split, self._stream())
        self._check(rc, "gam_op_convmod")

    def profile_enable(self, on=True) -> None:
        self._check(self.lib.gam_profile_enable(self._h, int(on)), "gam_profile_enable")

    def profile_level(self, on) -> None:
        self._check(self.lib.gam_profile_pause(self._h, int(on)), "gam_profile_pause")

    def profile_read(self) -> Dict[str, Dict[str, float]]:
        out = {}
        for i, name in enumerate(_lib.PF_CLASSES):
            ms, n, work = C.c_double(), C.c_int64(), C.c_double()
            self._check(self.lib.gam_profile_read(self._h, i, C.byref(ms), C.byref(n), C.byref(work)), "gam_profile_read")
            nbytes = C.c_double()
            self._check(self.lib.gam_profile_read_bytes(self._h, i, C.byref(nbytes)), "gam_profile_read_bytes")
            out[name] = {"ms": ms.value, "launches": int(n.value), "work": work.value, "bytes": nbytes.value}
        return out
```

### include/gigaam_hip.h

```cpp
#ifndef GIGAAM_HIP_H
#define GIGAAM_HIP_H

#include <stdint.h>

#ifdef __cplusplus
extern "C" {
#endif

#define GAM_ABI_VERSION 1

typedef struct gam_handle gam_handle;

enum { GAM_SUBS_CONV2D = 0, GAM_SUBS_CONV1D = 1 };
enum { GAM_ATT_ROTARY = 0, GAM_ATT_REL_POS = 1 };
enum { GAM_NORM_BATCH = 0, GAM_NORM_LAYER = 1 };
enum { GAM_HEAD_NONE = 0, GAM_HEAD_CTC = 1, GAM_HEAD_RNNT = 2, GAM_HEAD_EMO = 3 };
enum { GAM_DTYPE_F32 = 0, GAM_DTYPE_F16 = 1, GAM_DTYPE_BF16 = 2, GAM_DTYPE_F64 = 3, GAM_DTYPE_I64 = 4 };

typedef struct gam_config {
  int32_t sample_rate, n_mels, hop_length, win_length, n_fft, center;
  int32_t feat_in, n_layers, d_model, subsampling, subs_kernel_size, subsampling_factor;
  int32_t ff_expansion_factor, self_attention_model, n_heads, pos_emb_max_len;
  int32_t conv_norm_type, conv_kernel_size;
  int32_t head_type, num_classes, pred_hidden, pred_rnn_layers, joint_hidden;
// ... 89 lines not shown
                     int32_t* frames, int32_t* counts, float* score, float* logp, void* stream);

int gam_rnnt_beam_nbest(gam_handle* h, const float* encoded, const int32_t* enc_len, int B, int64_t Tp, int W, int max_symbols, int N,
                        int32_t* ids, int32_t* frames, int32_t* counts, float* score, float* logp, int32_t* n_hyp, void* stream);
int gam_op_rnnt_beam_nbest(gam_handle* h, const float* encp, const int32_t* enc_len, int B, int64_t Tp, int W, int max_symbols, int N,
                           int32_t* ids, int32_t* frames, int32_t* counts, float* score, float* logp, int32_t* n_hyp, void* stream);

int gam_rnnt_align(gam_handle* h, const float* encoded, const int32_t* enc_len, int B, int64_t Tp, const int32_t* targets,
                   const int32_t* target_len, int Umax, int32_t* tok_frame, float* score, float* loglik, int32_t* status, void* stream);
int gam_op_rnnt_align(gam_handle* h, const float* encp, const int32_t* enc_len, int B, int64_t Tp, const int32_t* targets,
                      const int32_t* target_len, int Umax, int32_t* tok_frame, float* score, float* loglik, int32_t* status,
                      float* lattice_out, void* stream);
int gam_op_rnnt_lattice_align(gam_handle* h, const float* lattice, const int32_t* enc_len, int B, int64_t Tp, int V, const int32_t* targets,
                              const int32_t* target_len, int Umax, int32_t* tok_frame, float* score, float* loglik, int32_t* status,
                              void* stream);
int gam_set_rnnt_align_workspace(gam_handle* h, int64_t bytes);

int gam_ctc_confidence(gam_handle* h, const float* encoded, const int32_t* enc_len, int B, int64_t Tp, const int32_t* ids,
                       const int32_t* frames, const int32_t* counts, int cap, int measure, int agg, float* conf, int32_t* span,
                       int32_t* status, void* stream);
int gam_op_ctc_confidence(gam_handle* h, const float* log_probs, const int32_t* enc_len, int B, int64_t Tp, int V, const int32_t* ids,
                          const int32_t* frames, const int32_t* counts, int cap, int measure, int agg, float* conf, int32_t* span,
                          int32_t* status, void* stream);
int gam_rnnt_confidence(gam_handle* h, const float* encoded, const int32_t* enc_len, int B, int64_t Tp, const int32_t* ids,
                        const int32_t* frames, const int32_t* counts, int cap, int measure, float* conf, int32_t* status, void* stream);
int gam_op_rnnt_confidence(gam_handle* h, const float* encp, const int32_t* enc_len, int B, int64_t Tp, const int32_t* ids,
                           const int32_t* frames, const int32_t* counts, int cap, int measure, float* conf, int32_t* status, void* stream);

int gam_set_rnnt_cluster(gam_handle* h, int workgroups_per_utterance);
int gam_get_rnnt_cluster(gam_handle* h);
int gam_rnnt_cluster_plan_info(int ncu, int cluster, int exclusive, int B, int H, int JH, int V, int L, int32_t* out);
int gam_rnnt_last_decode(gam_handle* h, int32_t* out);

int gam_debug_buffer_hash(gam_handle* h, int which, uint64_t* hash_out, int64_t* floats_out);

int gam_rnnt_predict(gam_handle* h, const int32_t* labels, const float* h_in, const float* c_in, int B, float* g_out,
                     float* h_out, float* c_out, void* stream);
int gam_rnnt_joint(gam_handle* h, const float* enc, const float* dec, int B, int T, int U, float* log_probs, void* stream);

int gam_emo_probs(gam_handle* h, const float* encoded, const int32_t* enc_len, int B, int64_t Tp, float* probs,
                  void* stream);

enum { GAM_GEMM_F32 = 0, GAM_GEMM_F16X3 = 1, GAM_GEMM_F16 = 2 };
int gam_set_gemm_mode(gam_handle* h, int mode);
int gam_range_flag(gam_handle* h, int* flag_host, void* stream);
int gam_range_flag_fetch(gam_handle* h, int32_t* flag_dev, void* stream);
int gam_get_gemm_mode(const gam_handle* h);

int gam_op_gemm(gam_handle* h, const float* A, const float* W, const float* bias, float* C,
                int M, int N, int K, int act, void* stream);
int gam_op_gemm_ex(gam_handle* h, const float* A, const float* W, const float* bias, const float* R, float alpha,
                   float* C, int M, int N, int K, int act, void* stream);

int gam_op_attention(gam_handle* h, const float* q, const float* k, const float* v, float* ctx,
                     const int32_t* lens, int B, int T, int H, void* stream);
int gam_op_attention_ex(gam_handle* h, const float* q, const float* k, const float* v, int64_t ldq, float* ctx,
                        const int32_t* lens, const int32_t* cu, int B, int Ta, int Tv, int H, const float* pbuf,
                        const float* pos_u, const float* pos_v, void* stream);

typedef struct gam_ln_op {
  const float* x;
  float* out1;
  float* out2;
  const float* w1;
  const float* b1;
  const float* w2;
  const float* b2;
  const float* rcos;
  const float* rsin;
  const int32_t* row_t;
  float* rs;
  const float* part;
  const float* pbias;
  const float* presid;
  float* xstore;
  int32_t mode, rows, d, split1, split2, dk, ta, rope_rows, nsplit;
  float eps, palpha;
} gam_ln_op;
int gam_op_layernorm(gam_handle* h, const gam_ln_op* op, void* stream);

int gam_op_convmod(gam_handle* h, const float* u, float* z, const float* dw_w, const float* dw_b, const float* n_scale,
                   const float* n_shift, const int32_t* lens, const int32_t* cu, int B, int Ta, int Tv, int d, int ks,
                   int layer_norm, int z_split, void* stream);

int gam_tune_sp(int mt, int nw, int splitk);
int gam_plan_sp(int M, int N, int K, int n_cu, int* mt, int* nw, int* splitk);
int gam_plan_sp_ex(int M, int N, int K, int n_cu, int* mt, int* nw, int* splitk, int* stages);
int gam_tune_sp_stages(int stages);

enum { GAM_RS_FMT_U8 = 0, GAM_RS_FMT_I16 = 1, GAM_RS_FMT_I24 = 2, GAM_RS_FMT_I32 = 3, GAM_RS_FMT_F32 = 4, GAM_RS_FMT_MULAW = 5,
       GAM_RS_FMT_ALAW = 6 };
int gam_resample_plan(int rate_in, int rate_out, int* up, int* down, int* taps);
int gam_resample_tile(int rate_in, int rate_out, int* tile, int* form);
int gam_resample_table(int rate_in, int rate_out, float* coeff, int32_t* first);
int64_t gam_resample_out_len(int rate_in, int rate_out, int64_t n_in);
int gam_op_resample(const void* src, int fmt, int channels, int channel, const int64_t* len_in, int B, int64_t frames, int rate_in,
                    int rate_out, const float* coeff, const int32_t* first, float* dst, int64_t L_out, int64_t* len_out, void* stream);

enum { GAM_PF_GEMM = 0, GAM_PF_CONV2 = 1, GAM_PF_ATTN = 2, GAM_PF_NORM = 3, GAM_PF_CONVMOD = 4,
       GAM_PF_STEM = 5, GAM_PF_FRONTEND = 6, GAM_PF_DECODE = 7, GAM_PF_MISC = 8,
       GAM_PF_ALIGN_BT = 9, GAM_PF_ALIGN_OUT = 10,
       GAM_PF_NCLASS = 11 };
int gam_profile_enable(gam_handle* h, int on);
int gam_profile_read(gam_handle* h, int cls, double* ms, int64_t* launches, double* work);
int gam_profile_pause(gam_handle* h, int on);
int gam_profile_read_bytes(gam_handle* h, int cls, double* bytes);

typedef struct gam_comm gam_comm;
#define GAM_COMM_ID_BYTES 128
int gam_comm_unique_id(char id_out[GAM_COMM_ID_BYTES]);
int gam_comm_create(const char id[GAM_COMM_ID_BYTES], int rank, int world, int device_id, gam_comm** out);
int gam_comm_world(const gam_comm* c);
int gam_gather_ids(gam_comm* c, const int32_t* index, const int32_t* counts, const int32_t* ids, const int32_t* frames,
                   int rows, int cap, int32_t* all_index, int32_t* all_counts, int32_t* all_ids, int32_t* all_frames,
                   void* stream);
const char* gam_comm_last_error(const gam_comm* c);
void gam_comm_destroy(gam_comm* c);

const char* gam_last_error(const gam_handle* h);

#ifdef __cplusplus
}
#endif
#endif
```

Before: 20780.

## Fuse GLU into pointwise_conv1 GEMM epilogue via interleaved (dealt) weight rows

Reorders pointwise_conv1 weight and bias rows at load time so that value and gate channels sit in adjacent groups of four within each GEMM output tile. The split-fp16 GEMM epilogue then applies GLU directly and writes a half-width output. When the GEMM plan uses split-K it falls back to a dealt layout that the conv-module kernel de-interleaves itself. This is meant to halve the intermediate u buffer traffic (write and read) and drop the sigmoid from the conv-module kernel. The cost is a new kernel template variant, extra weight copies, and a restriction to the BatchNorm path.

```diff
diff --git a/gigaam_amd/_lib.py b/gigaam_amd/_lib.py
--- a/gigaam_amd/_lib.py
+++ b/gigaam_amd/_lib.py
@@ -106,6 +106,7 @@
     "gam_op_attention_ex": (C.c_int, [_P, _P, _P, _P, C.c_int64, _P, _P, _P, C.c_int, C.c_int, C.c_int, C.c_int, _P, _P, _P, _P]),
     "gam_op_layernorm": (C.c_int, [_P, C.POINTER(GamLnOp), _P]),
     "gam_op_convmod": (C.c_int, [_P, _P, _P, _P, _P, _P, _P, _P, _P, C.c_int, C.c_int, C.c_int, C.c_int, C.c_int, C.c_int, C.c_int, _P]),
+    "gam_op_convmod_ex": (C.c_int, [_P, _P, _P, _P, _P, _P, _P, _P, _P, C.c_int, C.c_int, C.c_int, C.c_int, C.c_int, C.c_int, C.c_int, C.c_int, _P]),
     "gam_tune_sp": (C.c_int, [C.c_int, C.c_int, C.c_int]),
     "gam_plan_sp": (C.c_int, [C.c_int, C.c_int, C.c_int, C.c_int, C.POINTER(C.c_int), C.POINTER(C.c_int), C.POINTER(C.c_int)]),
     "gam_plan_sp_ex": (C.c_int, [C.c_int, C.c_int, C.c_int, C.c_int, C.POINTER(C.c_int), C.POINTER(C.c_int), C.POINTER(C.c_int), C.POINTER(C.c_int)]),
diff --git a/gigaam_amd/csrc/gam_api.hip b/gigaam_amd/csrc/gam_api.hip
--- a/gigaam_amd/csrc/gam_api.hip
+++ b/gigaam_amd/csrc/gam_api.hip
@@ -76,6 +76,7 @@
   float *ln_ff1_w, *ln_ff1_b, *ff1_w1, *ff1_b1, *ff1_w2, *ff1_b2;
   float *ln_att_w, *ln_att_b, *wqkv, *bqkv, *wo, *bo;
   float *wpos, *pos_u, *pos_v;
+  float *pw1_bd;
   float *ln_conv_w, *ln_conv_b, *pw1_w, *pw1_b, *dw_w, *dw_b, *cn_scale, *cn_shift, *pw2_w, *pw2_b;
   float *ln_ff2_w, *ln_ff2_b, *ff2_w1, *ff2_b1, *ff2_w2, *ff2_b2;
   float *ln_out_w, *ln_out_b;
@@ -120,6 +121,8 @@
   DevBuf jz, jp, jl;
   float *lstm_wih_x = nullptr, *lstm_whh_x = nullptr, *lstm_bias_x = nullptr;
   int use_rowscale = 1;
+  int glu_fuse = 1;
+  bool pw1_dealt = false;
   int use_range = 1;
   int ncu = 256;
   int rnnt_cluster = -1;
@@ -137,6 +140,7 @@
 
   DevBuf wavp, spec, img, c2, xin, y1, x, y, yr, hbuf, qkv, ctx, ubuf, zbuf, tok, logits, encp, pbuf, aplanes;
   DevBuf op_planes, op_sp, splitk_ws;
+  DevBuf op_deal;
   DevBuf align_star;
   DevBuf align_bp;
   DevBuf align_long_ws;
@@ -362,6 +366,12 @@
 
 static inline bool split_mode(const gam_handle* h) { return h->gemm_mode != GAM_GEMM_F32; }
 
+static GamSpPlan sp_plan(const gam_handle* h, int M, int N, int K, int a_mode) {
+  GamSpPlan plan = gam_gemm_sp_plan(M, N, K, a_mode, h->ncu);
+  if (!h->use_splitk) plan.s = 1;
+  return plan;
+}
+
 int gemm(gam_handle* h, hipStream_t s, const GamGemmArgs& a_in, int act, int cls = GAM_PF_GEMM, const W16* w16 = nullptr,
          PendingReduce* defer = nullptr) {
   GamGemmArgs a = a_in;
@@ -372,7 +382,7 @@
   if (ps.ev) {
     const double abytes = a.a_mode == 0 ? ((double)(a.M - 1) * (double)std::min<long>(a.lda, a.K) + a.K) * 4.0
                                         : (double)a.M / a.conv_f2 * 2.0 * a.conv_fp * a.conv_c * 4.0;
-    h->prof_bytes[cls] += abytes * (a.n_switch > 0 ? 2.0 : 1.0) + 4.0 * a.N * a.K + 4.0 * a.M * a.N * (a.R ? 2.0 : 1.0);
+    h->prof_bytes[cls] += abytes * (a.n_switch > 0 ? 2.0 : 1.0) + 4.0 * a.N * a.K + 4.0 * a.M * a.N * (a.R ? 2.0 : act == GAM_ACT_GLU ? 0.5 : 1.0);
   }
   hipError_t e;
   if (a.Asp != nullptr) {
@@ -387,8 +397,8 @@
       a.h16 = 1; a.K /= 2; a.lda /= 2; a.conv_c /= 2;
       a.Wsp = w16->h16;
     }
-    GamSpPlan plan = gam_gemm_sp_plan(a.M, a.N, a.K, a.a_mode, h->ncu);
-    if (!h->use_splitk) plan.s = 1;
+    const GamSpPlan plan = sp_plan(h, a.M, a.N, a.K, a.a_mode);
+    if (act == GAM_ACT_GLU && plan.s > 1) return fail(h, -2, "GLU epilogue on a split-K plan (M=%d N=%d K=%d S=%d): nothing launched", a.M, a.N, a.K, plan.s);
     a.sp_mt = plan.mt; a.sp_nw = plan.nw; a.sp_ns = plan.ns;
     GamGemmArgs full = a;
     if (plan.s > 1) {
@@ -408,6 +418,7 @@
     }
     return 0;
   }
+  if (act == GAM_ACT_GLU) return fail(h, -2, "GLU epilogue without sp32 operands (M=%d N=%d K=%d)", a.M, a.N, a.K);
   if (a.a_rs != nullptr || a.c_split) return fail(h, -2, "row-scaled A or split C without sp32 operands (M=%d N=%d K=%d)", a.M, a.N, a.K);
   int S = 1;
   if (h->use_splitk && a.a_mode == 0 && a.K % 32 == 0) {
@@ -528,6 +539,7 @@
     if (hipDeviceGetAttribute(&co, hipDeviceAttributeCooperativeLaunch, device_id) != hipSuccess || co == 0) h->rnnt_coop = 0;
   }
   if (const char* e = getenv("GAM_ROWSCALE")) h->use_rowscale = atoi(e);
+  if (const char* e = getenv("GAM_GLU_FUSE")) h->glu_fuse = atoi(e);
   if (const char* e = getenv("GAM_RANGE")) h->use_range = atoi(e);
   if (const char* e = getenv("GAM_GEMM_MODE"))
     h->gemm_mode = strcmp(e, "f32") == 0 ? GAM_GEMM_F32 : (strcmp(e, "f16") == 0 ? GAM_GEMM_F16 : GAM_GEMM_F16X3);
@@ -773,6 +785,21 @@
   return upload_to(h, DST(L.cn_shift), sh);
 }
 
+static int fin_pw1_dealt(gam_handle* h, const std::string& prefix, LayerW& L) {
+  const int D = h->cfg.d_model;
+  const HostTensor *wt, *bt;
+  if (int r = need(h, prefix + ".weight", (int64_t)2 * D * D, &wt)) return r;
+  if (int r = need(h, prefix + ".bias", 2 * D, &bt)) return r;
+  std::vector<float> w(wt->data.size()), b(bt->data.size());
+  for (int r = 0; r < 2 * D; ++r) {
+    const int ch = gam_glu_dealt_row(r, D);
+    std::copy(wt->data.begin() + (size_t)ch * D, wt->data.begin() + (size_t)(ch + 1) * D, w.begin() + (size_t)r * D);
+    b[r] = bt->data[ch];
+  }
+  if (int r = upload_to(h, DST(L.pw1_bd), b)) return r;
+  return up_split(h, w, &L.s_pw1, D);
+}
+
 static int fin_layer(gam_handle* h, int li, LayerW& L) {
   const gam_config& c = h->cfg;
   const int D = c.d_model, DFF = D * c.ff_expansion_factor;
@@ -795,7 +822,9 @@
     if (int r = upload_to(h, DST(L.pos_v), pv->data)) return r;
   }
   if (int r = upload_ln(h, p + "norm_conv", D, DST(L.ln_conv_w), DST(L.ln_conv_b))) return r;
-  if (int r = upload_linear(h, p + "conv.pointwise_conv1", 2 * D, D, DST(L.pw1_w), DST(L.pw1_b), &L.s_pw1)) return r;
+  if (int r = upload_linear(h, p + "conv.pointwise_conv1", 2 * D, D, DST(L.pw1_w), DST(L.pw1_b), h->pw1_dealt ? nullptr : &L.s_pw1)) return r;
+  if (h->pw1_dealt)
+    if (int r = fin_pw1_dealt(h, p + "conv.pointwise_conv1", L)) return r;
   if (int r = upload_linear(h, p + "conv.depthwise_conv", D, c.conv_kernel_size, DST(L.dw_w), DST(L.dw_b), nullptr)) return r;
   if (int r = fin_conv_norm(h, p, L)) return r;
   if (int r = upload_linear(h, p + "conv.pointwise_conv2", D, D, DST(L.pw2_w), DST(L.pw2_b), &L.s_pw2)) return r;
@@ -923,6 +952,7 @@
   if (build_encoder) {
     if (int r = c.subsampling == GAM_SUBS_CONV2D ? fin_stem_conv2d(h) : fin_stem_conv1d(h)) return r;
     h->layers.resize(c.n_layers);
+    h->pw1_dealt = h->glu_fuse != 0 && c.conv_norm_type == GAM_NORM_BATCH && c.d_model % 4 == 0;
     for (int li = 0; li < c.n_layers; ++li)
       if (int r = fin_layer(h, li, h->layers[li])) return r;
     if (int r = c.self_attention_model == GAM_ATT_ROTARY ? fin_rotary(h) : fin_rel_pos(h)) return r;
@@ -1009,6 +1039,7 @@
   int spf;
   bool sp_stem;
   bool graph;
+  int u_mode;
 };
 
 struct EncBufs {
@@ -1056,6 +1087,8 @@
   const bool f16_fmt_ok = p.D % 64 == 0 && p.DFF % 64 == 0;
   p.spf = p.sp ? (h->gemm_mode == GAM_GEMM_F16 && f16_fmt_ok ? 2 : 1) : 0;
   p.sp_stem = p.sp && p.F % 32 == 0;
+  p.u_mode = GAM_CM_U_NATURAL;
+  if (p.sp && h->pw1_dealt) p.u_mode = sp_plan(h, p.NR, 2 * p.D, p.spf == 2 ? p.D / 2 : p.D, 0).s == 1 ? GAM_CM_U_GLUED : GAM_CM_U_DEALT;
   p.graph = h->use_graph && !h->prof_on && p.nl > 0 && p.N < h->graph_max_rows && !p.packed;
   return 0;
 }
@@ -1071,7 +1104,7 @@
   if (int r = ensure(h, h->hbuf, N * p.DFF)) return r;
   if (int r = ensure(h, h->qkv, N * 3 * D)) return r;
   if (int r = ensure(h, h->ctx, N * D)) return r;
-  if (int r = ensure(h, h->ubuf, N * 2 * D)) return r;
+  if (int r = ensure(h, h->ubuf, N * D * (p.u_mode == GAM_CM_U_GLUED ? 1 : 2))) return r;
   if (int r = ensure(h, h->zbuf, N * D)) return r;
   if (int r = ensure(h, h->rsbuf, N + 64)) return r;
   if (p.packed)
@@ -1201,12 +1234,12 @@
 
 static hipError_t launch_convmod(gam_handle* h, hipStream_t s, const float* u, float* z, const float* dw_w, const float* dw_b, const float* n_scale,
                                  const float* n_shift, const int* lens, const int* cu, int B, int Ta, int Tv, int d, int ks, bool layer_norm,
-                                 int z_split) {
+                                 int z_split, int u_mode) {
   GamConvModArgs cm;
   memset(&cm, 0, sizeof cm);
   cm.u = u; cm.z = z; cm.dw_w = dw_w; cm.dw_b = dw_b; cm.n_scale = n_scale; cm.n_shift = n_shift;
   cm.lens = lens; cm.cu = cu; cm.B = B; cm.Ta = Ta; cm.Tv = Tv; cm.d = d; cm.ks = ks; cm.eps = 1e-5f;
-  cm.z_split = z_split; cm.range_flag = h->use_range ? h->range_flag : nullptr;
+  cm.z_split = z_split; cm.u_mode = u_mode; cm.range_flag = h->use_range ? h->range_flag : nullptr;
   return gam_launch_convmod(cm, layer_norm, s);
 }
 
@@ -1277,13 +1310,14 @@
   const EncPlan& p = c.p;
   const int D = p.D, NR = p.NR, ks = h->cfg.conv_kernel_size;
   if (int r = norm_to_y(h, s, c, L.ln_conv_w, L.ln_conv_b, pend)) return r;
-  GamGemmArgs g1 = gemm_args(h->y.p, D, L.pw1_w, L.pw1_b, h->ubuf.p, 2 * D, NR, 2 * D, D);
+  const bool glued = p.u_mode == GAM_CM_U_GLUED;
+  GamGemmArgs g1 = gemm_args(h->y.p, D, L.pw1_w, p.u_mode == GAM_CM_U_NATURAL ? L.pw1_b : L.pw1_bd, h->ubuf.p, glued ? D : 2 * D, NR, 2 * D, D);
   gemm_formats(g1, p.spf, c.w.rs, 0, 0);
-  if (int r = gemm(h, s, g1, GAM_ACT_NONE, GAM_PF_GEMM, &L.s_pw1)) return r;
+  if (int r = gemm(h, s, g1, glued ? GAM_ACT_GLU : GAM_ACT_NONE, GAM_PF_GEMM, &L.s_pw1)) return r;
   {
-    ProfScope ps(h, s, GAM_PF_CONVMOD, (double)NR * D * 3 * 4.0);
+    ProfScope ps(h, s, GAM_PF_CONVMOD, (double)NR * D * (glued ? 2 : 3) * 4.0);
     hipError_t e = launch_convmod(h, s, h->ubuf.p, h->zbuf.p, L.dw_w, L.dw_b, L.cn_scale, L.cn_shift, c.w.len2, c.w.cu, p.B,
-                                  p.packed ? p.Tmax : p.Ta, p.Tv, D, ks, h->cfg.conv_norm_type == GAM_NORM_LAYER, p.spf);
+                                  p.packed ? p.Tmax : p.Ta, p.Tv, D, ks, h->cfg.conv_norm_type == GAM_NORM_LAYER, p.spf, p.u_mode);
     if (e != hipSuccess) return fail(h, -2, "conv-module launch (k=%d): %s", ks, hipGetErrorString(e));
   }
   GamGemmArgs g2 = gemm_args(h->zbuf.p, D, L.pw2_w, L.pw2_b, h->x.p, D, NR, D, D);
@@ -1327,7 +1361,7 @@
   *replayed = false;
   if (!p.graph) return 0;
   const GamSpForce& frc = gam_sp_force();
-  const std::vector<int> key = {p.B, p.Ta, p.Tv, p.nl, h->gemm_mode, (int)p.sp, h->use_splitk, h->fuse_reduce, frc.mt.load(), frc.nw.load(), frc.s.load(), frc.ns.load()};
+  const std::vector<int> key = {p.B, p.Ta, p.Tv, p.nl, h->gemm_mode, (int)p.sp, h->use_splitk, h->fuse_reduce, h->glu_fuse, p.u_mode, frc.mt.load(), frc.nw.load(), frc.s.load(), frc.ns.load()};
   Entry& ge = h->graphs[key];
   if (ge.gen != h->ws_generation) {
     if (ge.exec) { hipGraphExecDestroy(ge.exec); --h->graph_count; }
@@ -2600,6 +2634,22 @@
   GamGemmArgs g = gemm_args(A, K, W, bias, C, N, M, N, K);
   g.R = R; g.ldr = N; g.alpha = alpha;
   hipStream_t s = (hipStream_t)stream;
+  if (act < GAM_ACT_NONE || act > GAM_ACT_GLU) return fail(h, -1, "gam_op_gemm: unknown activation %d", act);
+  if (act == GAM_ACT_GLU) {
+    if (!split_mode(h) || K % 32 != 0 || N % 8 != 0) return fail(h, -1, "gam_op_gemm: act 3 (GLU) needs a split-fp16 mode, K %% 32 == 0 and N %% 8 == 0 (N=%d K=%d)", N, K);
+    if (R != nullptr || alpha != 1.0f) return fail(h, -1, "gam_op_gemm: act 3 (GLU) takes no residual and no alpha");
+    const int s_plan = sp_plan(h, M, N, (h->gemm_mode == GAM_GEMM_F16 && K % 64 == 0) ? K / 2 : K, 0).s;
+    if (s_plan > 1) return fail(h, -1, "gam_op_gemm: act 3 (GLU) on a split-K plan (M=%d N=%d K=%d S=%d): nothing launched", M, N, K, s_plan);
+    g.ldc = N / 2;
+    if (int r = ensure(h, h->op_deal, (size_t)N * K + N + 64)) return r;
+    float* wd = h->op_deal.p;
+    float* bd = wd + (size_t)N * K;
+    hipLaunchKernelGGL(gam_glu_deal_rows_kernel, dim3((int)std::min<size_t>(((size_t)N * K + 255) / 256, 4096)), dim3(256), 0, s, W, wd, N / 2, K);
+    if (bias != nullptr) hipLaunchKernelGGL(gam_glu_deal_rows_kernel, dim3(gam_cdiv(N, 256)), dim3(256), 0, s, bias, bd, N / 2, 1);
+    W = wd;
+    g.W = wd;
+    if (bias != nullptr) g.bias = bd;
+  }
   if (!split_mode(h) || K % 32 != 0 || N % 4 != 0) return gemm(h, s, g, act);
   const size_t wn = (size_t)N * K, an = (size_t)M * K;
   W16 w16;
@@ -2691,8 +2741,16 @@
 int gam_op_convmod(gam_handle* h, const float* u, float* z, const float* dw_w, const float* dw_b, const float* n_scale,
                    const float* n_shift, const int32_t* lens, const int32_t* cu, int B, int Ta, int Tv, int d, int ks, int layer_norm,
                    int z_split, void* stream) {
+  return gam_op_convmod_ex(h, u, z, dw_w, dw_b, n_scale, n_shift, lens, cu, B, Ta, Tv, d, ks, layer_norm, z_split, GAM_CM_U_NATURAL, stream);
+}
+
+int gam_op_convmod_ex(gam_handle* h, const float* u, float* z, const float* dw_w, const float* dw_b, const float* n_scale,
+                      const float* n_shift, const int32_t* lens, const int32_t* cu, int B, int Ta, int Tv, int d, int ks, int layer_norm,
+                      int z_split, int u_mode, void* stream) {
   if (!h) return -1;
   if (!h->finalized) return fail(h, -1, "gam_op_convmod before gam_finalize");
+  if (u_mode < GAM_CM_U_NATURAL || u_mode > GAM_CM_U_GLUED || (u_mode != GAM_CM_U_NATURAL && layer_norm))
+    return fail(h, -1, "conv module: u_mode %d (0 [values | gates], 1 dealt quads, 2 GLU applied; 1 and 2: BatchNorm kernel only)", u_mode);
   if (!u || !z || !dw_w || !dw_b || !n_scale || !n_shift || !lens) return fail(h, -1, "conv module: null operand");
   if (B <= 0 || Ta <= 0 || Tv <= 0 || d <= 0) return fail(h, -1, "conv module: bad shape B %d Ta %d Tv %d d %d", B, Ta, Tv, d);
   if (cu == nullptr && Tv > Ta) return fail(h, -1, "conv module: Tv %d > Ta %d in the padded layout", Tv, Ta);
@@ -2702,7 +2760,7 @@
   if (d % 4 == 0 && (!al16(u) || !al16(z) || !al16(dw_b) || !al16(n_scale) || !al16(n_shift)))
     return fail(h, -1, "conv module: operands must be 16-byte aligned");
   HIPCHK(h, hipSetDevice(h->device));
-  hipError_t e = launch_convmod(h, (hipStream_t)stream, u, z, dw_w, dw_b, n_scale, n_shift, lens, cu, B, Ta, Tv, d, ks, layer_norm != 0, z_split);
+  hipError_t e = launch_convmod(h, (hipStream_t)stream, u, z, dw_w, dw_b, n_scale, n_shift, lens, cu, B, Ta, Tv, d, ks, layer_norm != 0, z_split, u_mode);
   if (e != hipSuccess) return fail(h, -2, "conv-module launch (k=%d, d=%d, %s): %s", ks, d, layer_norm ? "LayerNorm" : "BatchNorm", hipGetErrorString(e));
   return 0;
 }
diff --git a/gigaam_amd/csrc/gam_common.h b/gigaam_amd/csrc/gam_common.h
--- a/gigaam_amd/csrc/gam_common.h
+++ b/gigaam_amd/csrc/gam_common.h
@@ -203,4 +203,4 @@
   return acc;
 }
 
-enum { GAM_ACT_NONE = 0, GAM_ACT_SILU = 1, GAM_ACT_RELU = 2 };
+enum { GAM_ACT_NONE = 0, GAM_ACT_SILU = 1, GAM_ACT_RELU = 2, GAM_ACT_GLU = 3 };
diff --git a/gigaam_amd/csrc/gam_convmod.h b/gigaam_amd/csrc/gam_convmod.h
--- a/gigaam_amd/csrc/gam_convmod.h
+++ b/gigaam_amd/csrc/gam_convmod.h
@@ -16,9 +16,12 @@
   float eps;
   int z_split;
   int* range_flag;
+  int u_mode;
 };
 
-template <int KS>
+enum { GAM_CM_U_NATURAL = 0, GAM_CM_U_DEALT = 1, GAM_CM_U_GLUED = 2 };
+
+template <int KS, int UM = GAM_CM_U_NATURAL>
 __global__ __launch_bounds__(512, 4) void gam_convmod_bn_kernel(GamConvModArgs a) {
   constexpr int NRG = 32, TT = 128, PAD = (KS - 1) / 2, ROWS = (TT + KS - 1 + NRG - 1) / NRG * NRG, OUT = TT / NRG;
   __shared__ f32x4 tile[ROWS * 16];
@@ -33,14 +36,17 @@
   const size_t rowbase = ur.base;
   const int rlim = ur.lim;
   constexpr int NLD = ROWS / NRG;
-  f32x4 ua[NLD], ub[NLD];
+  constexpr bool GLUED = UM == GAM_CM_U_GLUED;
+  f32x4 ua[NLD], ub[GLUED ? 1 : NLD];
+  const int ldu = GLUED ? a.d : 2 * a.d;
+  const int ca = UM == GAM_CM_U_DEALT ? 2 * c : c, cb = UM == GAM_CM_U_DEALT ? 2 * c + 4 : a.d + c;
 #pragma unroll
   for (int u = 0; u < NLD; ++u) {
     const int t = t0 - PAD + rg + NRG * u;
     const int tc = t < 0 ? 0 : (t < rlim ? t : rlim - 1);
-    const float* up = a.u + (rowbase + tc) * (size_t)(2 * a.d);
-    ua[u] = *reinterpret_cast<const f32x4*>(up + c);
-    ub[u] = *reinterpret_cast<const f32x4*>(up + a.d + c);
+    const float* up = a.u + (rowbase + tc) * (size_t)ldu;
+    ua[u] = *reinterpret_cast<const f32x4*>(up + ca);
+    if (!GLUED) ub[u] = *reinterpret_cast<const f32x4*>(up + cb);
   }
   {
 #pragma unroll
@@ -55,8 +61,11 @@
     const int rr = rg + NRG * u;
     const int t = t0 - PAD + rr;
     const bool live = t >= 0 && t < klen;
-    const f32x4 glu = (f32x4){ua[u].x * gam_sigmoid(ub[u].x), ua[u].y * gam_sigmoid(ub[u].y),
-                              ua[u].z * gam_sigmoid(ub[u].z), ua[u].w * gam_sigmoid(ub[u].w)};
+    f32x4 glu = ua[u];
+    if (!GLUED) {
+      const f32x4 gt = ub[GLUED ? 0 : u];
+      glu = (f32x4){ua[u].x * gam_sigmoid(gt.x), ua[u].y * gam_sigmoid(gt.y), ua[u].z * gam_sigmoid(gt.z), ua[u].w * gam_sigmoid(gt.w)};
+    }
     tile[rr * 16 + q] = live ? glu : (f32x4){0.f, 0.f, 0.f, 0.f};
   }
   __syncthreads();
@@ -300,11 +309,18 @@
   if (!layer_norm) {
     if (a.d % 64 != 0) return hipErrorInvalidValue;
     dim3 grid(gam_cdiv(a.Ta, 128), a.d / 64, a.B);
-    if (a.ks == 31) hipLaunchKernelGGL(gam_convmod_bn_kernel<31>, grid, dim3(512), 0, s, a);
-    else if (a.ks == 5) hipLaunchKernelGGL(gam_convmod_bn_kernel<5>, grid, dim3(512), 0, s, a);
-    else if (a.ks == 9) hipLaunchKernelGGL(gam_convmod_bn_kernel<9>, grid, dim3(512), 0, s, a);
+#define GAM_CM_BN(KSV)                                                                                              \
+  if (a.u_mode == GAM_CM_U_GLUED) hipLaunchKernelGGL((gam_convmod_bn_kernel<KSV, GAM_CM_U_GLUED>), grid, dim3(512), 0, s, a);      \
+  else if (a.u_mode == GAM_CM_U_DEALT) hipLaunchKernelGGL((gam_convmod_bn_kernel<KSV, GAM_CM_U_DEALT>), grid, dim3(512), 0, s, a); \
+  else hipLaunchKernelGGL((gam_convmod_bn_kernel<KSV, GAM_CM_U_NATURAL>), grid, dim3(512), 0, s, a)
+    if (a.u_mode < GAM_CM_U_NATURAL || a.u_mode > GAM_CM_U_GLUED) return hipErrorInvalidValue;
+    if (a.ks == 31) { GAM_CM_BN(31); }
+    else if (a.ks == 5) { GAM_CM_BN(5); }
+    else if (a.ks == 9) { GAM_CM_BN(9); }
     else return hipErrorInvalidValue;
+#undef GAM_CM_BN
   } else {
+    if (a.u_mode != GAM_CM_U_NATURAL) return hipErrorInvalidValue;
     if (a.d > 1024) return hipErrorInvalidValue;
     dim3 grid(gam_cdiv(a.Ta, 8), a.B);
     if ((a.ks == 5 || a.ks == 9) && a.d % 4 == 0) {
diff --git a/gigaam_amd/csrc/gam_gemm_sp.h b/gigaam_amd/csrc/gam_gemm_sp.h
--- a/gigaam_amd/csrc/gam_gemm_sp.h
+++ b/gigaam_amd/csrc/gam_gemm_sp.h
@@ -357,11 +357,19 @@
           t = t * rsc + bv[pp][hf];
           if (ACT == GAM_ACT_SILU) { t.x = gam_silu(t.x); t.y = gam_silu(t.y); t.z = gam_silu(t.z); t.w = gam_silu(t.w); }
           if (ACT == GAM_ACT_RELU) { t.x = fmaxf(t.x, 0.f); t.y = fmaxf(t.y, 0.f); t.z = fmaxf(t.z, 0.f); t.w = fmaxf(t.w, 0.f); }
-          if (masked) t = (f32x4){0.f, 0.f, 0.f, 0.f};
-          t = t * g.alpha;
-          if (resid) t += rv[pp][hf];
-          if (!both && hf == 1) t = (f32x4){0.f, 0.f, 0.f, 0.f};
+          if (ACT != GAM_ACT_GLU) {
+            if (masked) t = (f32x4){0.f, 0.f, 0.f, 0.f};
+            t = t * g.alpha;
+            if (resid) t += rv[pp][hf];
+            if (!both && hf == 1) t = (f32x4){0.f, 0.f, 0.f, 0.f};
+          }
           v[hf] = t;
+        }
+        if (ACT == GAM_ACT_GLU) {
+          const f32x4 o = (f32x4){v[0].x * gam_sigmoid(v[1].x), v[0].y * gam_sigmoid(v[1].y), v[0].z * gam_sigmoid(v[1].z),
+                                  v[0].w * gam_sigmoid(v[1].w)};
+          *reinterpret_cast<f32x4*>(g.C + orow * g.ldc + (ecol >> 1)) = o;
+          continue;
         }
         if (g.c_guard) { gam_range_note(g.range_flag, v[0].x, v[0].y, v[0].z, v[0].w); gam_range_note(g.range_flag, v[1].x, v[1].y, v[1].z, v[1].w); }
         if ((GAM_SP_DBG(g) & 32) && v[0].x != 123.456f) continue;
@@ -496,6 +504,8 @@
   if (a.K <= 0 || a.K % 32 != 0 || a.Asp == nullptr || a.Wsp == nullptr) return hipErrorInvalidValue;
   if (a.a_mode == 0 ? (a.lda % 32 != 0) : (a.conv_c % 32 != 0)) return hipErrorInvalidValue;
   if (!gam_gemm_sp_epilogue_ok(a)) return hipErrorInvalidValue;
+  if (act == GAM_ACT_GLU && (a.N % 8 != 0 || a.lens != nullptr || a.R != nullptr || a.alpha != 1.0f || a.c_split || a.c_guard || a.splitk > 1))
+    return hipErrorInvalidValue;
   int mt = a.sp_mt, nw = a.sp_nw, ns = a.sp_ns;
   if (mt < 2 || mt > 4 || (nw != 2 && nw != 4) || (nw == 2 && mt == 4)) {
     const GamSpPlan p = gam_gemm_sp_plan(a.M, a.N, a.K, a.a_mode);
@@ -554,6 +564,7 @@
   switch (act) {
     case GAM_ACT_SILU: GAM_LSP(GAM_ACT_SILU); break;
     case GAM_ACT_RELU: GAM_LSP(GAM_ACT_RELU); break;
+    case GAM_ACT_GLU: GAM_LSP(GAM_ACT_GLU); break;
     default: GAM_LSP(GAM_ACT_NONE); break;
   }
 #undef GAM_LSP
@@ -613,6 +624,15 @@
   }
 }
 
+__host__ __device__ inline int gam_glu_dealt_row(int r, int D) { return (r & 4 ? D : 0) + 4 * (r >> 3) + (r & 3); }
+__global__ __launch_bounds__(256) void gam_glu_deal_rows_kernel(const float* __restrict__ x, float* __restrict__ y, int D, int K) {
+  const size_t total = (size_t)2 * D * K, stride = (size_t)gridDim.x * 256;
+  for (size_t i = (size_t)blockIdx.x * 256 + threadIdx.x; i < total; i += stride) {
+    const int r = (int)(i / K), k = (int)(i - (size_t)r * K);
+    y[i] = x[(size_t)gam_glu_dealt_row(r, D) * K + k];
+  }
+}
+
 __global__ __launch_bounds__(256) void gam_rowscale_kernel(const float* __restrict__ x, float* __restrict__ rs, int rows,
                                                            int K, long lda) {
   const int row = blockIdx.x * 4 + (threadIdx.x >> 6), lane = threadIdx.x & 63;
diff --git a/gigaam_amd/engine.py b/gigaam_amd/engine.py
--- a/gigaam_amd/engine.py
+++ b/gigaam_amd/engine.py
@@ -1084,7 +1084,7 @@
         resid = None if resid is None else self._dev(resid, torch.float32)
         m, k = a.shape
         n = w.shape[0]
-        out = torch.empty((m, n), dtype=torch.float32, device=self.device)
+        out = torch.empty((m, n // 2 if act == 3 else n), dtype=torch.float32, device=self.device)
         with torch.cuda.device(self.device):
             rc = self.lib.gam_op_gemm_ex(self._h, _ptr(a), _ptr(w), _ptr(bias), _ptr(resid), alpha, _ptr(out), m, n, k, act,
                                          self._stream())
@@ -1143,14 +1143,15 @@
         self._check(rc, "gam_op_layernorm")
 
     def op_convmod(self, u: Tensor, z: Tensor, dw_w: Tensor, dw_b: Tensor, n_scale: Tensor, n_shift: Tensor, lens: Tensor, B: int,
-                   Ta: int, Tv: int, d: int, ks: int, layer_norm: bool, z_split: int = 0, cu: Optional[Tensor] = None) -> None:
+                   Ta: int, Tv: int, d: int, ks: int, layer_norm: bool, z_split: int = 0, cu: Optional[Tensor] = None,
+                   u_mode: int = 0) -> None:
         what = "op_convmod"
         ptrs = [self._op_ptr(what, n, t) for n, t in (("u", u), ("z", z), ("dw_w", dw_w), ("dw_b", dw_b), ("n_scale", n_scale),
                                                       ("n_shift", n_shift))]
         ptrs += [self._op_ptr(what, "lens", lens, torch.int32), self._op_ptr(what, "cu", cu, torch.int32)]
         with torch.cuda.device(self.device):
-            rc = self.lib.gam_op_convmod(self._h, *ptrs, B, Ta, Tv, d, ks, int(bool(layer_norm)), z_split, self._stream())
-        self._check(rc, "gam_op_convmod")
+            rc = self.lib.gam_op_convmod_ex(self._h, *ptrs, B, Ta, Tv, d, ks, int(bool(layer_norm)), z_split, u_mode, self._stream())
+        self._check(rc, "gam_op_convmod_ex")
 
     def profile_enable(self, on=True) -> None:
         self._check(self.lib.gam_profile_enable(self._h, int(on)), "gam_profile_enable")
diff --git a/include/gigaam_hip.h b/include/gigaam_hip.h
--- a/include/gigaam_hip.h
+++ b/include/gigaam_hip.h
@@ -195,6 +195,9 @@
 int gam_op_convmod(gam_handle* h, const float* u, float* z, const float* dw_w, const float* dw_b, const float* n_scale,
                    const float* n_shift, const int32_t* lens, const int32_t* cu, int B, int Ta, int Tv, int d, int ks,
                    int layer_norm, int z_split, void* stream);
+int gam_op_convmod_ex(gam_handle* h, const float* u, float* z, const float* dw_w, const float* dw_b, const float* n_scale,
+                      const float* n_shift, const int32_t* lens, const int32_t* cu, int B, int Ta, int Tv, int d, int ks,
+                      int layer_norm, int z_split, int u_mode, void* stream);
 
 int gam_tune_sp(int mt, int nw, int splitk);
 int gam_plan_sp(int M, int N, int K, int n_cu, int* mt, int* nw, int* splitk);
```

Result: no change. 20800 (median of 2 runs) (+0.1%).
